# 3dlg-hcvc/tricolo

Measured on AMD Instinct MI355X. Metric: trimodal training samples/sec (32^3 voxel + 6-view), higher is better.
Workload: dtype f16 (f16 activation storage + f16 MFMA operands, fp32 accumulate; bf16x3 heads/GRU; within 1e-3 of the fp32 reference)

## Files before the change

include/tricolo_hip.h:

```cpp
#ifndef TRICOLO_HIP_H
#define TRICOLO_HIP_H
#include <stddef.h>
#include <stdint.h>

#ifdef __cplusplus
extern "C" {
#endif

#define TRI_FMT_F32 0
#define TRI_FMT_BF16 1
#define TRI_FMT_F16 2

int tri_version(void);
const char* tri_last_error(void);

typedef struct TriConvDesc {
    int B, ID, IH, IW, Cin;
    int OD, OH, OW, Cout;
    int KD, KH, KW, stride, pad_d, pad_h, pad_w;
} TriConvDesc;

int tri_conv_kpad(int ntaps, int cin_stored);
typedef struct TriPrepDesc {
    const float* w;
// ... 1 lines not shown
    void* lo;
    long s_row, s_tap, s_inner;
    int rows, ntaps, inner, inner_pad, kpad, fmt;
    int frag;
} TriPrepDesc;
int tri_weight_prep_multi(const TriPrepDesc* descs_dev, int n, void* stream);
int tri_weight_prep(const float* w, long s_row, long s_tap, long s_inner, int rows, int ntaps, int inner, int inner_pad,
                    void* w_hi, void* w_lo, int fmt, int frag, void* stream);

int tri_embedding_fwd(const int* tokens, const float* weight, int B, int L, int D, float* out, void* stream);
int tri_embedding_bwd(const int* tokens, const float* dout, int B, int L, int V, int D, int padding_idx, float* dweight, void* stream);

int tri_retrieval_topk(const float* text, const float* shape, const int* label, int Nq, int Ns, int D, int k, int* topk_idx ,
                       double* topk_sim , int* first_hit , void* stream);

int tri_linear_small_supported(int M, int K, int N);
int tri_linear_small_fwd(const float* x, const float* w, const float* bias, float* y, int M, int K, int N, int act, int split3, void* stream);
int tri_linear_small_dgrad(const float* dout, const float* y, const float* w, float* dx, int M, int K, int N, int act, int split3,
                           void* stream);
int tri_linear_small_wgrad(const float* x, const float* dout, const float* y, float* dw, float* db , int M, int K, int N,
                           int act, int split3, void* stream);
int tri_linear_small_bwd(const float* x, const float* dout, const float* y, const float* w, float* dx, float* dw, float* db, int M, int K,
                         int N, int act, int split3, void* stream);

int tri_conv_num_mtiles(const TriConvDesc* d, int split3);
int tri_conv_num_records(const TriConvDesc* d, int split3, int row_list);
typedef enum TriConvFamily {
    TRI_CONV_IGEMM = 0,
    TRI_CONV_DMA = 2,
    TRI_CONV_HALO2D = 3,
    TRI_CONV_STEM = 4,
    TRI_CONV_HALO_ROWS = 5,
    TRI_CONV_VOX0 = 6,
    TRI_CONV_C64 = 9,
    TRI_CONV_S2D = 10,
    TRI_CONV_PW = 12,
    TRI_CONV_VOXG = 13,
    TRI_CONV_VOXB = 14,
    TRI_CONV_S2G = 15
} TriConvFamily;
#define TRI_FAMILY_CODE_MASK 255
#define TRI_FAMILY_TILE_SHIFT 8
#define TRI_FAMILY_SPLITK_SHIFT 16
#define TRI_FAMILY_SPU_SHIFT 24
int tri_conv_kernel_family(const TriConvDesc* d, int transposed, int split3);
typedef enum TriWgradFamily {
    TRI_WGRAD_STAGED = 0,
    TRI_WGRAD_DMA = 2,
    TRI_WGRAD_STEM = 4,
    TRI_WGRAD_VOX0 = 6,
    TRI_WGRAD_KROW = 7,
    TRI_WGRAD_C64 = 9
} TriWgradFamily;
#define TRI_WGRAD_MASK 1
#define TRI_WGRAD_ROWS 2
#define TRI_WGRAD_SPLIT3 4
#define TRI_WGRAD_BNF 8
#define TRI_WGRAD_ROUTE_CODE_MASK 255
#define TRI_WGRAD_ROUTE_GROUP_SHIFT 8
#define TRI_WGRAD_ROUTE_ROWS_SHIFT 12
#define TRI_WGRAD_ROUTE_COLS_SHIFT 21
int tri_conv_wgrad_route(const TriConvDesc* d, int act_fmt, int features);
int tri_conv_wgrad_kernel_family(const TriConvDesc* d, int act_fmt);
size_t tri_conv_workspace(const TriConvDesc* d, int transposed);
int tri_conv_fwd(const TriConvDesc* d, const void* in, const void* w_hi, const void* w_lo, void* out, const uint8_t* row_mask,
                 const float* bias, int act, int accumulate, float* stats, int act_fmt, void* workspace, size_t workspace_bytes,
                 const int* row_pos , const int* row_count ,
                 void* stream);
int tri_conv_dgrad(const TriConvDesc* d, const void* dout, const void* wt_hi, const void* wt_lo, void* din, const uint8_t* row_mask,
                   int accumulate, int act_fmt, void* workspace, size_t workspace_bytes,
                   const int* row_pos ,
                   const int* row_count ,
                   void* stream);
typedef struct TriConvBnSums {
    const void* y;
    const float* relu_scale;
    const float* relu_shift;
    const void* relu_out;
    float* partial;
} TriConvBnSums;
int tri_conv_dgrad_bn_records(const TriConvDesc* d, int accumulate, int act_fmt);
int tri_conv_dgrad_bn(const TriConvDesc* d, const void* dout, const void* wt_hi, const void* wt_lo, void* din, int accumulate,
                      int act_fmt, void* workspace, size_t workspace_bytes, const int* row_pos, const TriConvBnSums* sums, void* stream);
size_t tri_conv_wgrad_workspace(const TriConvDesc* d);
size_t tri_conv_plan_bytes(const TriConvDesc* d);
int tri_conv_plan_build(const TriConvDesc* d, void* plan, void* stream);
int tri_conv_wgrad(const TriConvDesc* d, const void* in, const void* dout, const uint8_t* row_mask, const void* plan ,
                   void* workspace, size_t workspace_bytes, float* dw, long s_co, long s_tap, long s_ci, int cin_real, int split3,
                   int act_fmt, float out_scale ,
                   const int* row_pos, const int* row_count ,
                   void* stream);
#ifndef TRI_WGRAD_GROUP_MAX
#define TRI_WGRAD_GROUP_MAX 24
#endif
typedef struct TriWgradReduce {
    const float* slab;
    float* dw;
    long s_co, s_tap, s_ci;
    int splits, Cout, Kpad, ntaps, cin_stored, cin_real, zlanes, nblocks;
    float out_scale;
    int kw_real;
    int kw_shift;
} TriWgradReduce;
int tri_conv_wgrad_partial(const TriConvDesc* d, const void* in, const void* dout, const uint8_t* row_mask, const void* plan ,
                           void* workspace, size_t workspace_bytes, float* dw, long s_co, long s_tap, long s_ci, int cin_real, int split3,
                           int act_fmt, float out_scale, const int* row_pos, const int* row_count, TriWgradReduce* pending ,
                           void* stream);
int tri_wgrad_reduce_grouped(const TriWgradReduce* pending , int n, void* stream);
int tri_wgrad_reduce_grouped_noted(const TriWgradReduce* pending , int n, int* note, void* stream);
#define TRI_WGRAD_JOBS_MAX 12
typedef struct TriWgradJob {
    const TriConvDesc* d;
    const void* in;
    const void* dout;
    const void* plan;
    void* workspace;
    size_t workspace_bytes;
    float* dw;
    long s_co, s_tap, s_ci;
    int cin_real;
    float out_scale;
    const int* row_pos;
    const int* row_count;
} TriWgradJob;
int tri_conv_stem_wgrad_bn(const TriConvDesc* d, const void* in, const void* y, const uint8_t* arg, const void* dpool, const float* c1,
                           const float* c2, const float* c3, const float* relu_scale, const float* relu_shift, void* workspace,
                           size_t workspace_bytes, float* dw, long s_co, long s_tap, long s_ci, int cin_real, int act_fmt, float out_scale,
                           TriWgradReduce* pending , void* stream);
int tri_conv_wgrad_group_info(const TriConvDesc* d, int act_fmt, int* family, int* tiles, int* steps);
int tri_conv_wgrad_partial_group(const TriWgradJob* jobs , int n, int act_fmt, TriWgradReduce* pending ,
                                 void* stream);

int tri_bn_finalize(const float* partial, int ntiles, int C, const int* count_dev, int count_host, const float* gamma,
                    const float* beta, float* running_mean, float* running_var, long long* num_batches_tracked, float momentum,
                    float eps, float* mean, float* invstd, float* scale, float* shift, void* stream);
int tri_bn_eval_coeffs(int C, const float* gamma, const float* beta, const float* rm, const float* rv, float eps, float* mean,
                       float* invstd, float* scale, float* shift, void* stream);
int tri_bn_act(const void* y, const float* scale, const float* shift, const void* res, const float* rscale, const float* rshift,
               void* out, long M, int C, int relu, int act_fmt, void* stream);
int tri_relu_bwd(const void* dout, const void* out, void* g, long n, int act_fmt, void* stream);
int tri_bn_bwd_num_blocks(long M);
int tri_bn_bwd_reduce(const void* y, const void* g, long M, int C, float* partial, const float* relu_scale, const float* relu_shift,
                      const void* relu_out, const uint8_t* row_mask , int act_fmt,
                      void* stream);
int tri_bn_bwd_small(const void* y, const void* g, long M, int C, const int* count_dev, int count_host, const float* gamma,
                     const float* mean, const float* invstd, const float* relu_scale, const float* relu_shift, const void* relu_out,
                     void* g_masked, const uint8_t* row_mask, int keep_inactive, void* dy, float* dgamma, float* dbeta, float out_scale,
                     int act_fmt, void* stream);
int tri_bn_bwd_finalize(const float* partial, int nblk, int C, const int* count_dev, int count_host, const float* gamma,
                        const float* mean, const float* invstd, float* dgamma, float* dbeta, float* c1, float* c2, float* c3,
                        float out_scale ,
                        void* stream);
int tri_bn_bwd_apply(const void* y, const void* g, const float* c1, const float* c2, const float* c3, const uint8_t* row_mask,
                     void* dy, long M, int C, const float* relu_scale, const float* relu_shift, const void* relu_out,
                     void* g_masked ,
                     int keep_inactive ,
                     int act_fmt, void* stream);
int tri_bn_bwd_pair_reduce(const void* ya, const void* yb, const void* g, const void* relu_out, long M, int C, float* partial_a,
                           float* partial_b, int act_fmt, void* stream);
int tri_bn_bwd_pair_finalize(const float* partial_a, const float* partial_b, int nblk, int C, int count_host, const float* gamma_a,
                             const float* mean_a, const float* invstd_a, float* buf_a, const float* gamma_b, const float* mean_b,
                             const float* invstd_b, float* buf_b, float out_scale, void* stream);
int tri_bn_bwd_pair_apply(const void* ya, const void* yb, const void* g, const void* relu_out, const float* buf_a, const float* buf_b,
                          void* dya, void* dyb, void* g_masked, long M, int C, int act_fmt, void* stream);

int tri_bn_relu_pool3d_fwd(const void* y, const float* scale, const float* shift, const uint8_t* mask, int B, int D, int C,
// ... 131 lines not shown
```

tricolo_amd/_C.py:

```python
from __future__ import annotations

import ctypes as C
import os

import torch

_HERE = os.path.dirname(os.path.abspath(__file__))
LIB_PATH = os.path.join(_HERE, "libtricolo_hip.so")


class TriConvDesc(C.Structure):
    _fields_ = [(n, C.c_int) for n in ("B", "ID", "IH", "IW", "Cin", "OD", "OH", "OW", "Cout",
                                       "KD", "KH", "KW", "stride", "pad_d", "pad_h", "pad_w")]


class TriPrepDesc(C.Structure):
    _fields_ = [("w", C.c_void_p), ("hi", C.c_void_p), ("lo", C.c_void_p), ("s_row", C.c_long), ("s_tap", C.c_long),
                ("s_inner", C.c_long), ("rows", C.c_int), ("ntaps", C.c_int), ("inner", C.c_int), ("inner_pad", C.c_int),
                ("kpad", C.c_int), ("fmt", C.c_int), ("frag", C.c_int)]


class TriWgradReduce(C.Structure):
    _fields_ = [("slab", C.c_void_p), ("dw", C.c_void_p), ("s_co", C.c_long), ("s_tap", C.c_long), ("s_ci", C.c_long)] + \
               [(n, C.c_int) for n in ("splits", "Cout", "Kpad", "ntaps", "cin_stored", "cin_real", "zlanes", "nblocks")] + \
               [("out_scale", C.c_float), ("kw_real", C.c_int), ("kw_shift", C.c_int)]


class TriWgradJob(C.Structure):
    _fields_ = [("d", C.POINTER(TriConvDesc)), ("inp", C.c_void_p), ("dout", C.c_void_p), ("plan", C.c_void_p), ("workspace", C.c_void_p),
                ("workspace_bytes", C.c_size_t), ("dw", C.c_void_p), ("s_co", C.c_long), ("s_tap", C.c_long), ("s_ci", C.c_long),
                ("cin_real", C.c_int), ("out_scale", C.c_float), ("row_pos", C.c_void_p), ("row_count", C.c_void_p)]


class TriConvBnSums(C.Structure):
    _fields_ = [("y", C.c_void_p), ("relu_scale", C.c_void_p), ("relu_shift", C.c_void_p), ("relu_out", C.c_void_p), ("partial", C.c_void_p)]


TRI_WGRAD_JOBS_MAX = 12
TRI_ERR_ARG, TRI_ERR_UNSUPPORTED = -1, -2

P, I, L, F, Z, DBL = C.c_void_p, C.c_int, C.c_long, C.c_float, C.c_size_t, C.c_double
DP = C.POINTER(TriConvDesc)

SIGNATURES = {
    "tri_version": (I, []),
    "tri_last_error": (C.c_char_p, []),
    "tri_conv_kpad": (I, [I, I]),
    "tri_weight_prep": (I, [P, L, L, L, I, I, I, I, P, P, I, I, P]),
    "tri_weight_prep_multi": (I, [P, I, P]),
    "tri_embedding_fwd": (I, [P, P, I, I, I, P, P]),
    "tri_embedding_bwd": (I, [P, P, I, I, I, I, I, P, P]),
    "tri_retrieval_topk": (I, [P, P, P, I, I, I, I, P, P, P, P]),
    "tri_linear_small_supported": (I, [I, I, I]),
    "tri_linear_small_fwd": (I, [P, P, P, P, I, I, I, I, I, P]),
    "tri_linear_small_dgrad": (I, [P, P, P, P, I, I, I, I, I, P]),
    "tri_linear_small_wgrad": (I, [P, P, P, P, P, I, I, I, I, I, P]),
    "tri_linear_small_bwd": (I, [P, P, P, P, P, P, P, I, I, I, I, I, P]),
    "tri_conv_num_mtiles": (I, [DP, I]),
    "tri_conv_num_records": (I, [DP, I, I]),
    "tri_conv_workspace": (Z, [DP, I]),
    "tri_conv_kernel_family": (I, [DP, I, I]),
    "tri_conv_wgrad_kernel_family": (I, [DP, I]),
    "tri_conv_wgrad_route": (I, [DP, I, I]),
    "tri_conv_fwd": (I, [DP, P, P, P, P, P, P, I, I, P, I, P, Z, P, P, P]),
    "tri_conv_dgrad": (I, [DP, P, P, P, P, P, I, I, P, Z, P, P, P]),
    "tri_conv_dgrad_bn_records": (I, [DP, I, I]),
    "tri_conv_dgrad_bn": (I, [DP, P, P, P, P, I, I, P, Z, P, C.POINTER(TriConvBnSums), P]),
    "tri_conv_wgrad_workspace": (Z, [DP]),
    "tri_conv_plan_bytes": (Z, [DP]),
    "tri_conv_plan_build": (I, [DP, P, P]),
    "tri_conv_wgrad": (I, [DP, P, P, P, P, P, Z, P, L, L, L, I, I, I, F, P, P, P]),
    "tri_conv_wgrad_partial": (I, [DP, P, P, P, P, P, Z, P, L, L, L, I, I, I, F, P, P, P, P]),
    "tri_wgrad_reduce_grouped": (I, [P, I, P]),
    "tri_wgrad_reduce_grouped_noted": (I, [P, I, P, P]),
    "tri_conv_stem_wgrad_bn": (I, [DP, P, P, P, P, P, P, P, P, P, P, Z, P, L, L, L, I, I, F, P, P]),
    "tri_conv_wgrad_group_info": (I, [DP, I, P, P, P]),
    "tri_conv_wgrad_partial_group": (I, [P, I, I, P, P]),
    "tri_bn_finalize": (I, [P, I, I, P, I, P, P, P, P, P, F, F, P, P, P, P, P]),
    "tri_bn_eval_coeffs": (I, [I, P, P, P, P, F, P, P, P, P, P]),
    "tri_bn_act": (I, [P, P, P, P, P, P, P, L, I, I, I, P]),
    "tri_relu_bwd": (I, [P, P, P, L, I, P]),
    "tri_bn_bwd_num_blocks": (I, [L]),
    "tri_bn_bwd_reduce": (I, [P, P, L, I, P, P, P, P, P, I, P]),
    "tri_bn_bwd_finalize": (I, [P, I, I, P, I, P, P, P, P, P, P, P, P, F, P]),
    "tri_bn_bwd_small": (I, [P, P, L, I, P, I, P, P, P, P, P, P, P, P, I, P, P, P, F, I, P]),
    "tri_bn_bwd_apply": (I, [P, P, P, P, P, P, P, L, I, P, P, P, P, I, I, P]),
    "tri_bn_bwd_pair_reduce": (I, [P, P, P, P, L, I, P, P, I, P]),
    "tri_bn_bwd_pair_finalize": (I, [P, P, I, I, I, P, P, P, P, P, P, P, P, F, P]),
    "tri_bn_bwd_pair_apply": (I, [P, P, P, P, P, P, P, P, P, L, I, I, P]),
    "tri_bn_relu_pool3d_fwd": (I, [P, P, P, P, I, I, I, P, P, I, P]),
    "tri_pool3d_bwd_route": (I, [P, P, P, P, P, P, I, I, I, P, I, P]),
    "tri_pool3d_bwd_route_rows": (I, [P, P, P, P, P, P, I, I, I, P, P, P, I, P]),
    "tri_pool3d_bwd_route_rows_num_blocks": (I, [I, I, I]),
    "tri_pool3d_bwd_route_rows_reduce": (I, [P, P, P, P, P, P, I, I, I, P, P, P, P, I, P]),
    "tri_bn_bwd_apply_rows": (I, [P, P, P, P, P, P, I, P, P, L, I, P]),
    "tri_bn_bwd_rows_scratch": (C.c_size_t, [I]),
    "tri_bn_bwd_rows": (I, [P, P, I, P, P, L, P, P, P, P, P, P, F, P, I, P]),
    "tri_pool3d_bwd_route_reduce_num_blocks": (I, [I, I, I]),
    "tri_pool3d_bwd_route_reduce": (I, [P, P, P, P, P, P, I, I, I, P, P, I, P]),
    "tri_maxpool2d_fwd": (I, [P, I, I, I, I, P, P, P, P, I, P]),
    "tri_maxpool2d_bwd": (I, [P, P, I, I, I, I, P, I, P]),
    "tri_maxpool_bn_bwd_num_blocks": (I, [I, I, I]),
    "tri_maxpool_bn_bwd_reduce": (I, [P, P, P, I, I, I, I, P, P, P, I, P]),
    "tri_maxpool_bn_bwd_pooled_num_blocks": (I, [I, I, I]),
    "tri_maxpool_bn_bwd_reduce_pooled": (I, [P, P, P, P, I, I, I, I, P, P, P, P, I, P]),
    "tri_maxpool_bn_bwd_apply": (I, [P, P, P, I, I, I, I, P, P, P, P, P, P, I, P]),
    "tri_avgpool_viewmax_fwd": (I, [P, I, I, I, I, P, P, I, P]),
    "tri_avgpool_viewmax_bwd": (I, [P, P, I, I, I, I, P, I, F, P]),
    "tri_voxel_scatter": (I, [P, P, I, I, I, P, P, I, P]),
    "tri_voxel_from_rgba_u8": (I, [P, I, I, P, P, I, P]),
    "tri_nchw3_u8_to_nhwc4": (I, [P, I, I, I, P, P, P, I, P]),
    "tri_mask_count": (I, [P, L, P, P]),
    "tri_debug_stamp": (I, [P, P]),
    "tri_debug_buffer_b128_probe": (I, [P, P, L, I, P]),
    "tri_mask_compact_scratch": (Z, [L]),
    "tri_mask_compact": (I, [P, L, P, P, P, P]),
    "tri_mask_pyramid": (I, [P, I, I, P, P]),
    "tri_mask_compact_multi_scratch": (Z, [P, I]),
    "tri_mask_compact_multi": (I, [P, P, I, P, P, P, P]),
    "tri_nchw3_to_nhwc4": (I, [P, I, I, I, P, I, P]),
    "tri_l2norm_fwd": (I, [P, I, I, F, P, P, P]),
    "tri_l2norm_bwd": (I, [P, P, P, I, I, F, P, P]),
    "tri_colsum": (I, [P, L, I, P, P]),
    "tri_axpy": (I, [P, F, P, L, P]),
    "tri_act_bwd": (I, [P, P, P, L, I, P]),
    "tri_cast_from_f32": (I, [P, P, L, F, I, P]),
    "tri_cast_to_f32": (I, [P, P, L, I, P]),
    "tri_gru_fwd": (I, [P, P, P, I, I, P, P, P, I, P]),
    "tri_gru_bwd": (I, [P, P, P, P, I, I, P, P, P, P, I, P]),
    "tri_ntxent_workspace": (Z, [I, I]),
    "tri_ntxent_fwd_bwd": (I, [P, P, I, I, F, F, I, P, P, P, P, Z, P]),
    "tri_ntxent_bwd": (I, [P, P, I, I, F, F, I, P, P, P, P, Z, P]),
    "tri_ntxent_multi_workspace": (Z, [I, I, I]),
    "tri_ntxent_multi_fwd": (I, [P, I, I, I, F, F, I, P, P, Z, P]),
    "tri_ntxent_multi_bwd": (I, [P, I, I, I, F, F, I, P, P, P, P, Z, P]),
    "tri_triplet_workspace": (Z, [I, I]),
    "tri_triplet_fwd": (I, [P, P, I, I, DBL, P, P, P, Z, P]),
    "tri_triplet_bwd": (I, [P, P, I, I, DBL, P, P, P, P, Z, P]),
    "tri_triplet_multi_workspace": (Z, [I, I, I]),
    "tri_triplet_multi_fwd": (I, [P, I, I, I, DBL, P, P, P, Z, P]),
    "tri_triplet_multi_bwd": (I, [P, I, I, I, DBL, P, P, P, P, Z, P]),
    "tri_nn_dist2": (I, [P, P, P, P, I, I, I, I, I, P, P, P]),
    "tri_f1_counts": (I, [P, P, I, I, C.POINTER(F), I, P, P, P]),
    "tri_f1_finalize": (I, [P, P, P, P, P, P, I, I, I, I, F, P, P, P, P, P]),
    "tri_mesh_bbox": (I, [P, P, I, P, P]),
    "tri_mesh_face_cdf": (I, [P, P, P, P, P, I, L, P, P, P]),
    "tri_mesh_sample_points": (I, [P, P, P, P, P, P, P, I, I, C.c_ulonglong, P, P, P]),
    "tri_raster_workspace": (Z, [L, I, I, I, I]),
    "tri_raster_render": (I, [P, P, P, P, P, P, P, P, I, L, I, I, I, DBL, DBL, P, P, P, P]),
    "tri_voxelize_workspace": (Z, [L, I, I]),
# ... 87 lines not shown
```

tricolo_amd/csrc/bn_pool.hip:

```cpp
#include "common.h"
#include "../../include/tricolo_hip.h"

__global__ void bn_finalize_kernel(const float* __restrict__ partial, int ntiles, int C, const int* __restrict__ count_dev,
                                   int count_host, const float* __restrict__ gamma, const float* __restrict__ beta,
                                   float* running_mean, float* running_var, long long* num_batches_tracked, float momentum,
                                   float eps, float* __restrict__ mean_out, float* __restrict__ invstd_out,
                                   float* __restrict__ scale_out, float* __restrict__ shift_out) {
    __shared__ double ssum[4], ssq[4];
    const int c = blockIdx.x;
    float pg = 0.f, pb = 0.f, prm = 0.f, prv = 0.f;
    int pcount = count_host;
    if (threadIdx.x == 0) {
        pg = gamma[c]; pb = beta[c];
        if (running_mean) { prm = running_mean[c]; prv = running_var[c]; }
        if (count_dev) pcount = *count_dev;
    }
    double s = 0.0, q = 0.0;
#pragma unroll 8
    for (int tIdx = threadIdx.x; tIdx < ntiles; tIdx += 256) {
        s += (double)partial[((size_t)tIdx * 2 + 0) * C + c];
        q += (double)partial[((size_t)tIdx * 2 + 1) * C + c];
    }
#pragma unroll
    for (int o = 32; o > 0; o >>= 1) { s += __shfl_xor(s, o); q += __shfl_xor(q, o); }
    if ((threadIdx.x & 63) == 0) { ssum[threadIdx.x >> 6] = s; ssq[threadIdx.x >> 6] = q; }
    __syncthreads();
    if (threadIdx.x == 0) {
        s = (ssum[0] + ssum[1]) + (ssum[2] + ssum[3]);
        q = (ssq[0] + ssq[1]) + (ssq[2] + ssq[3]);
        double n = (double)pcount;
        if (n < 1.0) {
            mean_out[c] = 0.f; invstd_out[c] = 0.f; scale_out[c] = 0.f; shift_out[c] = 0.f;
            return;
        }
        double mean = s / n;
        double var = q / n - mean * mean;
        if (var < 0.0) var = 0.0;
        double invstd = 1.0 / sqrt(var + (double)eps);
        mean_out[c] = (float)mean;
        invstd_out[c] = (float)invstd;
        float sc = (float)((double)pg * invstd);
        scale_out[c] = sc;
        shift_out[c] = (float)((double)pb - mean * (double)pg * invstd);
        if (running_mean) {
            double unb = n > 1.0 ? var * n / (n - 1.0) : var;
            running_mean[c] = (float)((1.0 - momentum) * prm + momentum * mean);
            running_var[c] = (float)((1.0 - momentum) * prv + momentum * unb);
        }
        if (num_batches_tracked && c == 0) *num_batches_tracked += 1;
    }
}

extern "C" int tri_bn_finalize(const float* partial, int ntiles, int C, const int* count_dev, int count_host, const float* gamma,
                               const float* beta, float* running_mean, float* running_var, long long* num_batches_tracked,
                               float momentum, float eps, float* mean, float* invstd, float* scale, float* shift, void* stream) {
    bn_finalize_kernel<<<C, 256, 0, (hipStream_t)stream>>>(partial, ntiles, C, count_dev, count_host, gamma, beta,
                                                                      running_mean, running_var, num_batches_tracked, momentum,
                                                                      eps, mean, invstd, scale, shift);
    return tri_check_launch("tri_bn_finalize");
}

__global__ void bn_eval_coeffs_kernel(int C, const float* gamma, const float* beta, const float* rm, const float* rv, float eps,
                                      float* mean, float* invstd, float* scale, float* shift) {
    int c = blockIdx.x * blockDim.x + threadIdx.x;
    if (c >= C) return;
    float is = 1.0f / sqrtf(rv[c] + eps);
    mean[c] = rm[c]; invstd[c] = is; scale[c] = gamma[c] * is; shift[c] = beta[c] - rm[c] * gamma[c] * is;
}
extern "C" int tri_bn_eval_coeffs(int C, const float* gamma, const float* beta, const float* rm, const float* rv, float eps,
                                  float* mean, float* invstd, float* scale, float* shift, void* stream) {
    bn_eval_coeffs_kernel<<<(C + 255) / 256, 256, 0, (hipStream_t)stream>>>(C, gamma, beta, rm, rv, eps, mean, invstd, scale, shift);
    return tri_check_launch("tri_bn_eval_coeffs");
}

template <typename T>
__global__ void bn_act_kernel(const T* __restrict__ y, const float4* __restrict__ scale, const float4* __restrict__ shift,
                              const T* __restrict__ res, const float4* __restrict__ rscale, const float4* __restrict__ rshift,
                              T* __restrict__ out, long total4, int C4, int relu) {
    for (long i = (long)blockIdx.x * blockDim.x + threadIdx.x; i < total4; i += (long)gridDim.x * blockDim.x) {
        int c = (int)(i % C4);
        float4 v = Act<T>::ld4(y + i * 4), s = scale[c], b = shift[c];
        v.x = __fmaf_rn(v.x, s.x, b.x); v.y = __fmaf_rn(v.y, s.y, b.y); v.z = __fmaf_rn(v.z, s.z, b.z); v.w = __fmaf_rn(v.w, s.w, b.w);
        if (res) {
            float4 r = Act<T>::ld4(res + i * 4);
            if (rscale) {
                float4 rs = rscale[c], rb = rshift[c];
                r.x = r.x * rs.x + rb.x; r.y = r.y * rs.y + rb.y; r.z = r.z * rs.z + rb.z; r.w = r.w * rs.w + rb.w;
            }
            v.x += r.x; v.y += r.y; v.z += r.z; v.w += r.w;
        }
        if (relu) { v.x = fmaxf(v.x, 0.f); v.y = fmaxf(v.y, 0.f); v.z = fmaxf(v.z, 0.f); v.w = fmaxf(v.w, 0.f); }
        Act<T>::st4(out + i * 4, v);
    }
}
static inline int ew_grid(long total) {
    long b = (total + 255) / 256;
    return (int)(b < 1 ? 1 : (b > 4096 ? 4096 : b));
}
extern "C" int tri_bn_act(const void* y, const float* scale, const float* shift, const void* res, const float* rscale,
                          const float* rshift, void* out, long M, int C, int relu, int act_fmt, void* stream) {
    if (C % 4) { tri_set_error("tri_bn_act: C must be a multiple of 4"); return TRI_ERR_ARG; }
    long total4 = M * (C / 4);
    TRI_ACT_DISPATCH(act_fmt, bn_act_kernel<T><<<ew_grid(total4), 256, 0, (hipStream_t)stream>>>(
        (const T*)y, (const float4*)scale, (const float4*)shift, (const T*)res, (const float4*)rscale, (const float4*)rshift, (T*)out,
        total4, C / 4, relu));
    return tri_check_launch("tri_bn_act");
}

template <typename T>
__global__ void relu_bwd_kernel(const T* dout, const T* __restrict__ out, T* g, long total4) {
    for (long i = (long)blockIdx.x * blockDim.x + threadIdx.x; i < total4; i += (long)gridDim.x * blockDim.x) {
        float4 d = Act<T>::ld4(dout + i * 4), o = Act<T>::ld4(out + i * 4);
        d.x = o.x > 0.f ? d.x : 0.f; d.y = o.y > 0.f ? d.y : 0.f; d.z = o.z > 0.f ? d.z : 0.f; d.w = o.w > 0.f ? d.w : 0.f;
        Act<T>::st4(g + i * 4, d);
    }
}
extern "C" int tri_relu_bwd(const void* dout, const void* out, void* g, long n, int act_fmt, void* stream) {
    if (n % 4) { tri_set_error("tri_relu_bwd: n must be a multiple of 4"); return TRI_ERR_ARG; }
    TRI_ACT_DISPATCH(act_fmt, relu_bwd_kernel<T><<<ew_grid(n / 4), 256, 0, (hipStream_t)stream>>>((const T*)dout, (const T*)out, (T*)g, n / 4));
    return tri_check_launch("tri_relu_bwd");
}

static inline int bnb_rows(long M) {
    if (M <= 16384) return 16;
    if (M <= 32768) return 32;
    if (M < 65536) return 64;
    long rows = (M + 2047) / 2048;
    rows = (rows + 63) / 64 * 64;
    return (int)(rows < 256 ? 256 : rows);
}
template <typename T, int MASK, bool ROWMASK>
__global__ void bn_bwd_reduce_kernel(const T* __restrict__ y, const T* __restrict__ g, long M, int C, float* __restrict__ partial,
                                     int BNB_ROWS, const float4* __restrict__ rs, const float4* __restrict__ rb,
                                     const T* __restrict__ ro, const uint8_t* __restrict__ row_mask) {
    extern __shared__ float sh[];
    const int C4 = C >> 2;
    const int tpr = C4 < 256 ? C4 : 256;
    const int rpp = 256 / tpr;
    const int cpt = (C4 + tpr - 1) / tpr;
    const int tc = threadIdx.x % tpr, tr = threadIdx.x / tpr;
    const long r0 = (long)blockIdx.x * BNB_ROWS;
    const long r1 = r0 + BNB_ROWS < M ? r0 + BNB_ROWS : M;
    for (int cc = 0; cc < cpt; ++cc) {
        int c4 = tc + cc * tpr;
        float4 sg = make_float4(0, 0, 0, 0), sgy = make_float4(0, 0, 0, 0);
        float4 s4 = make_float4(0, 0, 0, 0), b4 = make_float4(1, 1, 1, 1);
        if (MASK == 1 && c4 < C4) { s4 = rs[c4]; b4 = rb[c4]; }
        if (c4 < C4 && tr < rpp)
#pragma unroll 4
            for (long r = r0 + tr; r < r1; r += rpp) {
                if (ROWMASK && !row_mask[r]) continue;
                float4 gv = Act<T>::ld4(g + r * C + c4 * 4), yv = Act<T>::ld4(y + r * C + c4 * 4);
                if (MASK == 1) {
                    gv.x = __fmaf_rn(yv.x, s4.x, b4.x) > 0.f ? gv.x : 0.f; gv.y = __fmaf_rn(yv.y, s4.y, b4.y) > 0.f ? gv.y : 0.f;
                    gv.z = __fmaf_rn(yv.z, s4.z, b4.z) > 0.f ? gv.z : 0.f; gv.w = __fmaf_rn(yv.w, s4.w, b4.w) > 0.f ? gv.w : 0.f;
                }
                if (MASK == 2) {
                    const float4 ov = Act<T>::ld4(ro + r * C + c4 * 4);
                    gv.x = ov.x > 0.f ? gv.x : 0.f; gv.y = ov.y > 0.f ? gv.y : 0.f; gv.z = ov.z > 0.f ? gv.z : 0.f; gv.w = ov.w > 0.f ? gv.w : 0.f;
                }
                sg.x += gv.x; sg.y += gv.y; sg.z += gv.z; sg.w += gv.w;
                sgy.x += gv.x * yv.x; sgy.y += gv.y * yv.y; sgy.z += gv.z * yv.z; sgy.w += gv.w * yv.w;
            }
        __syncthreads();
        if (c4 < C4 && tr < rpp) {
            float* p = sh + ((size_t)tr * tpr + tc) * 8;
            p[0] = sg.x; p[1] = sg.y; p[2] = sg.z; p[3] = sg.w; p[4] = sgy.x; p[5] = sgy.y; p[6] = sgy.z; p[7] = sgy.w;
        }
        __syncthreads();
        if (tr == 0 && c4 < C4) {
            float a[8] = {0, 0, 0, 0, 0, 0, 0, 0};
            for (int rr = 0; rr < rpp; ++rr) {
                const float* p = sh + ((size_t)rr * tpr + tc) * 8;
#pragma unroll
// ... 25 lines not shown
    else if (relu_scale) TRI_BNR(1);
    else TRI_BNR(0);
#undef TRI_BNR
    return tri_check_launch("tri_bn_bwd_reduce");
}

__device__ __forceinline__ void bn_bwd_finalize_body(const float* __restrict__ partial, int nblk, int C, const int* __restrict__ count_dev,
                                                     int count_host, const float* __restrict__ gamma, const float* __restrict__ mean,
                                                     const float* __restrict__ invstd, float* __restrict__ dgamma, float* __restrict__ dbeta,
                                                     float* __restrict__ c1, float* __restrict__ c2, float* __restrict__ c3, float out_scale,
                                                     int c) {
    __shared__ double ssum[4], ssq[4];
    float pmu = 0.f, pis = 0.f, pga = 0.f;
    int pcount = count_host;
    if (threadIdx.x == 0) {
        pmu = mean[c]; pis = invstd[c]; pga = gamma[c];
        if (count_dev) pcount = *count_dev;
    }
    double s = 0.0, q = 0.0;
#pragma unroll 8
    for (int b = threadIdx.x; b < nblk; b += 256) {
        s += (double)partial[((size_t)b * 2 + 0) * C + c];
        q += (double)partial[((size_t)b * 2 + 1) * C + c];
    }
#pragma unroll
    for (int o = 32; o > 0; o >>= 1) { s += __shfl_xor(s, o); q += __shfl_xor(q, o); }
    if ((threadIdx.x & 63) == 0) { ssum[threadIdx.x >> 6] = s; ssq[threadIdx.x >> 6] = q; }
    __syncthreads();
    if (threadIdx.x == 0) {
        s = (ssum[0] + ssum[1]) + (ssum[2] + ssum[3]);
        q = (ssq[0] + ssq[1]) + (ssq[2] + ssq[3]);
        double n = (double)pcount;
        if (n < 1.0) { dgamma[c] = 0.f; dbeta[c] = 0.f; c1[c] = 0.f; c2[c] = 0.f; c3[c] = 0.f; return; }
        double mu = pmu, is = pis, ga = pga;
        double dbe = s;
        double dga = is * (q - mu * s);
        dgamma[c] = (float)(dga * (double)out_scale);
        dbeta[c] = (float)(dbe * (double)out_scale);
        double k1 = ga * is;
        double k3 = -ga * is * is * dga / n;
        double k2 = -k1 * dbe / n - k3 * mu;
        c1[c] = (float)k1; c2[c] = (float)k2; c3[c] = (float)k3;
    }
}
__global__ void bn_bwd_finalize_kernel(const float* __restrict__ partial, int nblk, int C, const int* __restrict__ count_dev,
                                       int count_host, const float* __restrict__ gamma, const float* __restrict__ mean,
                                       const float* __restrict__ invstd, float* __restrict__ dgamma, float* __restrict__ dbeta,
                                       float* __restrict__ c1, float* __restrict__ c2, float* __restrict__ c3, float out_scale) {
    bn_bwd_finalize_body(partial, nblk, C, count_dev, count_host, gamma, mean, invstd, dgamma, dbeta, c1, c2, c3, out_scale, blockIdx.x);
}
__global__ void bn_bwd_finalize_pair_kernel(const float* __restrict__ pa, const float* __restrict__ pb, int nblk, int C, int count_host,
                                            const float* __restrict__ ga, const float* __restrict__ ma, const float* __restrict__ ia,
                                            float* __restrict__ buf_a, const float* __restrict__ gb, const float* __restrict__ mb,
                                            const float* __restrict__ ib, float* __restrict__ buf_b, float out_scale) {
    const bool second = (int)blockIdx.x >= C;
    const int c = second ? blockIdx.x - C : blockIdx.x;
    float* buf = second ? buf_b : buf_a;
    bn_bwd_finalize_body(second ? pb : pa, nblk, C, nullptr, count_host, second ? gb : ga, second ? mb : ma, second ? ib : ia, buf, buf + C,
                         buf + 2 * C, buf + 3 * C, buf + 4 * C, out_scale, c);
}
extern "C" int tri_bn_bwd_finalize(const float* partial, int nblk, int C, const int* count_dev, int count_host, const float* gamma,
                                   const float* mean, const float* invstd, float* dgamma, float* dbeta, float* c1, float* c2,
                                   float* c3, float out_scale, void* stream) {
    bn_bwd_finalize_kernel<<<C, 256, 0, (hipStream_t)stream>>>(partial, nblk, C, count_dev, count_host, gamma, mean,
                                                                          invstd, dgamma, dbeta, c1, c2, c3, out_scale);
    return tri_check_launch("tri_bn_bwd_finalize");
}

template <typename T, int MASK>
__global__ void bn_bwd_apply_kernel(const T* __restrict__ y, const T* g, const float4* __restrict__ c1,
                                    const float4* __restrict__ c2, const float4* __restrict__ c3,
                                    const uint8_t* __restrict__ row_mask, T* dy, long total4, int C4,
                                    const float4* __restrict__ rs, const float4* __restrict__ rb, const T* __restrict__ ro, T* gm,
                                    int keep_inactive) {
    for (long i = (long)blockIdx.x * blockDim.x + threadIdx.x; i < total4; i += (long)gridDim.x * blockDim.x) {
        long row = i / C4;
        int c = (int)(i - row * C4);
        float4 o = make_float4(0.f, 0.f, 0.f, 0.f);
        if (keep_inactive && row_mask && !row_mask[row]) continue;
        if (!row_mask || row_mask[row]) {
            float4 yv = Act<T>::ld4(y + i * 4), gv = Act<T>::ld4(g + i * 4), a = c1[c], b = c2[c], d = c3[c];
            if (MASK == 1) {
                const float4 s4 = rs[c], b4 = rb[c];
                gv.x = __fmaf_rn(yv.x, s4.x, b4.x) > 0.f ? gv.x : 0.f; gv.y = __fmaf_rn(yv.y, s4.y, b4.y) > 0.f ? gv.y : 0.f;
                gv.z = __fmaf_rn(yv.z, s4.z, b4.z) > 0.f ? gv.z : 0.f; gv.w = __fmaf_rn(yv.w, s4.w, b4.w) > 0.f ? gv.w : 0.f;
            }
            if (MASK == 2) {
                const float4 ov = Act<T>::ld4(ro + i * 4);
                gv.x = ov.x > 0.f ? gv.x : 0.f; gv.y = ov.y > 0.f ? gv.y : 0.f; gv.z = ov.z > 0.f ? gv.z : 0.f; gv.w = ov.w > 0.f ? gv.w : 0.f;
                if (gm) Act<T>::st4(gm + i * 4, gv);
            }
            o.x = a.x * gv.x + b.x + d.x * yv.x; o.y = a.y * gv.y + b.y + d.y * yv.y;
            o.z = a.z * gv.z + b.z + d.z * yv.z; o.w = a.w * gv.w + b.w + d.w * yv.w;
        }
        Act<T>::st4(dy + i * 4, o);
    }
}
extern "C" int tri_bn_bwd_apply(const void* y, const void* g, const float* c1, const float* c2, const float* c3,
                                const uint8_t* row_mask, void* dy, long M, int C, const float* relu_scale, const float* relu_shift,
                                const void* relu_out, void* g_masked, int keep_inactive, int act_fmt, void* stream) {
    long total4 = M * (C / 4);
#define TRI_BNA(MASK_)                                                                                                              \
    TRI_ACT_DISPATCH(act_fmt, bn_bwd_apply_kernel<T, MASK_><<<ew_grid(total4), 256, 0, (hipStream_t)stream>>>(                      \
        (const T*)y, (const T*)g, (const float4*)c1, (const float4*)c2, (const float4*)c3, row_mask, (T*)dy, total4, C / 4,          \
        (const float4*)relu_scale, (const float4*)relu_shift, (const T*)relu_out, (T*)g_masked, keep_inactive))
    if (relu_out) TRI_BNA(2);
    else if (relu_scale) TRI_BNA(1);
    else TRI_BNA(0);
#undef TRI_BNA
    return tri_check_launch("tri_bn_bwd_apply");
}

template <typename T>
__global__ void bn_bwd_reduce_pair_kernel(const T* __restrict__ ya, const T* __restrict__ yb, const T* __restrict__ g, long M, int C,
                                          float* __restrict__ partial_a, float* __restrict__ partial_b, int BNB_ROWS,
                                          const T* __restrict__ ro) {
    extern __shared__ float sh[];
    const int C4 = C >> 2;
    const int tpr = C4 < 256 ? C4 : 256;
    const int rpp = 256 / tpr;
    const int cpt = (C4 + tpr - 1) / tpr;
    const int tc = threadIdx.x % tpr, tr = threadIdx.x / tpr;
    const long r0 = (long)blockIdx.x * BNB_ROWS;
    const long r1 = r0 + BNB_ROWS < M ? r0 + BNB_ROWS : M;
    for (int cc = 0; cc < cpt; ++cc) {
        int c4 = tc + cc * tpr;
        float4 sg = make_float4(0, 0, 0, 0), sga = make_float4(0, 0, 0, 0), sgb = make_float4(0, 0, 0, 0);
        if (c4 < C4 && tr < rpp)
#pragma unroll 4
            for (long r = r0 + tr; r < r1; r += rpp) {
                float4 gv = Act<T>::ld4(g + r * C + c4 * 4);
                const float4 av = Act<T>::ld4(ya + r * C + c4 * 4), bv = Act<T>::ld4(yb + r * C + c4 * 4), ov = Act<T>::ld4(ro + r * C + c4 * 4);
                gv.x = ov.x > 0.f ? gv.x : 0.f; gv.y = ov.y > 0.f ? gv.y : 0.f; gv.z = ov.z > 0.f ? gv.z : 0.f; gv.w = ov.w > 0.f ? gv.w : 0.f;
                sg.x += gv.x; sg.y += gv.y; sg.z += gv.z; sg.w += gv.w;
                sga.x += gv.x * av.x; sga.y += gv.y * av.y; sga.z += gv.z * av.z; sga.w += gv.w * av.w;
                sgb.x += gv.x * bv.x; sgb.y += gv.y * bv.y; sgb.z += gv.z * bv.z; sgb.w += gv.w * bv.w;
            }
        __syncthreads();
        if (c4 < C4 && tr < rpp) {
            float* p = sh + ((size_t)tr * tpr + tc) * 12;
            p[0] = sg.x; p[1] = sg.y; p[2] = sg.z; p[3] = sg.w; p[4] = sga.x; p[5] = sga.y; p[6] = sga.z; p[7] = sga.w;
            p[8] = sgb.x; p[9] = sgb.y; p[10] = sgb.z; p[11] = sgb.w;
        }
        __syncthreads();
        if (tr == 0 && c4 < C4) {
            float a[12] = {0, 0, 0, 0, 0, 0, 0, 0, 0, 0, 0, 0};
            for (int rr = 0; rr < rpp; ++rr) {
                const float* p = sh + ((size_t)rr * tpr + tc) * 12;
#pragma unroll
                for (int k = 0; k < 12; ++k) a[k] += p[k];
            }
            float* oa = partial_a + (size_t)blockIdx.x * 2 * C;
            float* ob = partial_b + (size_t)blockIdx.x * 2 * C;
#pragma unroll
            for (int k = 0; k < 4; ++k) { oa[c4 * 4 + k] = a[k]; oa[C + c4 * 4 + k] = a[4 + k]; ob[c4 * 4 + k] = a[k]; ob[C + c4 * 4 + k] = a[8 + k]; }
        }
    }
}
template <typename T>
__global__ void bn_bwd_apply_pair_kernel(const T* __restrict__ ya, const T* __restrict__ yb, const T* g, const float4* __restrict__ ca,
                                         const float4* __restrict__ cb, T* dya, T* dyb, long total4, int C4, const T* __restrict__ ro, T* gm) {
    for (long i = (long)blockIdx.x * blockDim.x + threadIdx.x; i < total4; i += (long)gridDim.x * blockDim.x) {
        const int c = (int)(i % C4);
        float4 gv = Act<T>::ld4(g + i * 4);
        const float4 av = Act<T>::ld4(ya + i * 4), bv = Act<T>::ld4(yb + i * 4), ov = Act<T>::ld4(ro + i * 4);
        gv.x = ov.x > 0.f ? gv.x : 0.f; gv.y = ov.y > 0.f ? gv.y : 0.f; gv.z = ov.z > 0.f ? gv.z : 0.f; gv.w = ov.w > 0.f ? gv.w : 0.f;
        if (gm) Act<T>::st4(gm + i * 4, gv);
        {
            const float4 a = ca[c], b = ca[C4 + c], d = ca[2 * C4 + c];
            float4 o;
            o.x = a.x * gv.x + b.x + d.x * av.x; o.y = a.y * gv.y + b.y + d.y * av.y;
            o.z = a.z * gv.z + b.z + d.z * av.z; o.w = a.w * gv.w + b.w + d.w * av.w;
            asm volatile("" : "+v"(o.x), "+v"(o.y), "+v"(o.z), "+v"(o.w));
            Act<T>::st4(dya + i * 4, o);
        }
        {
// ... 1069 lines not shown
```

tricolo_amd/csrc/common.h:

```cpp
#pragma once
#include <hip/hip_runtime.h>
#include <stdint.h>
#include <stdlib.h>

typedef __bf16 bf16_t;
typedef __bf16 bf16x8 __attribute__((ext_vector_type(8)));
typedef __bf16 bf16x4 __attribute__((ext_vector_type(4)));
typedef float f32x4 __attribute__((ext_vector_type(4)));
typedef _Float16 f16_t;
typedef _Float16 f16x8 __attribute__((ext_vector_type(8)));
typedef _Float16 f16x4 __attribute__((ext_vector_type(4)));

#define TRI_OK 0
#define TRI_ERR_ARG (-1)
#define TRI_ERR_UNSUPPORTED (-2)

extern "C" void tri_set_error(const char* msg);
static inline int tri_probe_ablation() {
#ifdef TRI_PROBE_BUILD
    static int abl = -1;
    if (abl < 0) { const char* e = getenv("TRICOLO_HALO_ABL"); abl = e ? atoi(e) : 0; }
    return abl;
#else
    return 0;
#endif
}
int tri_check_launch(const char* what);

static inline int tri_env_read_int(const char* name, int dflt) { const char* e = getenv(name); return e ? atoi(e) : dflt; }
static inline bool tri_env_read_is(const char* name, char c) { const char* e = getenv(name); return e && e[0] == c; }
#define tri_env_int(name, dflt) ([]() -> int { static const int v = tri_env_read_int(name, dflt); return v; }())
#define tri_env_is(name, c) ([]() -> bool { static const bool v = tri_env_read_is(name, c); return v; }())

struct FastDiv {
    uint32_t mul, shift, d;
};
static inline FastDiv make_fastdiv(uint32_t d) {
    FastDiv f;
    f.d = d;
    uint32_t l = 0;
    while ((1u << l) < d) ++l;
    f.shift = l;
    f.mul = (uint32_t)((((uint64_t)1 << 32) * (((uint64_t)1 << l) - d)) / d + 1);
    return f;
}
__device__ __forceinline__ uint32_t fdiv(uint32_t n, const FastDiv& f) {
    return (__umulhi(f.mul, n) + n) >> f.shift;
}

__device__ __forceinline__ int tile_off(int row, int chunk) {
    int g = (row >> 2) & 3;
    int f = g ^ ((g & 1) << 1);
    return row * 64 + ((chunk ^ f) << 4);
}

__device__ __forceinline__ void split_bf16(const float4& v, bf16x4& hi, bf16x4& lo) {
    hi[0] = (bf16_t)v.x; hi[1] = (bf16_t)v.y; hi[2] = (bf16_t)v.z; hi[3] = (bf16_t)v.w;
    lo[0] = (bf16_t)(v.x - (float)hi[0]); lo[1] = (bf16_t)(v.y - (float)hi[1]);
    lo[2] = (bf16_t)(v.z - (float)hi[2]); lo[3] = (bf16_t)(v.w - (float)hi[3]);
}
__device__ __forceinline__ bf16x4 to_bf16x4(const float4& v) {
    bf16x4 h;
    h[0] = (bf16_t)v.x; h[1] = (bf16_t)v.y; h[2] = (bf16_t)v.z; h[3] = (bf16_t)v.w;
    return h;
}

#ifndef TRI_FMT_F32
#define TRI_FMT_F32 0
#define TRI_FMT_BF16 1
#define TRI_FMT_F16 2
#endif
__device__ __forceinline__ float fp32_rounded(float x) {
    asm volatile("" : "+v"(x));
    return x;
}
template <typename T> struct Act;
template <> struct Act<float> {
    static constexpr int BYTES = 4;
    static constexpr int SIG_BITS = 24;
    static __device__ __forceinline__ float4 ld4(const float* p) { return *(const float4*)p; }
    static __device__ __forceinline__ void st4(float* p, const float4& v) { *(float4*)p = v; }
    static __device__ __forceinline__ float rnd(float v) { return v; }
};
template <> struct Act<bf16_t> {
    static constexpr int BYTES = 2;
    static constexpr int SIG_BITS = 8;
    static __device__ __forceinline__ float4 ld4(const bf16_t* p) {
        bf16x4 r = *(const bf16x4*)p;
        return make_float4((float)r[0], (float)r[1], (float)r[2], (float)r[3]);
    }
    static __device__ __forceinline__ void st4(bf16_t* p, const float4& v) { *(bf16x4*)p = to_bf16x4(v); }
    static __device__ __forceinline__ float rnd(float v) { return (float)(bf16_t)v; }
};
template <> struct Act<f16_t> {
    static constexpr int BYTES = 2;
    static constexpr int SIG_BITS = 11;
    static __device__ __forceinline__ float4 ld4(const f16_t* p) {
        f16x4 r = *(const f16x4*)p;
        return make_float4((float)r[0], (float)r[1], (float)r[2], (float)r[3]);
    }
    static __device__ __forceinline__ void st4(f16_t* p, const float4& v) {
        f16x4 h;
        h[0] = (f16_t)v.x; h[1] = (f16_t)v.y; h[2] = (f16_t)v.z; h[3] = (f16_t)v.w;
        *(f16x4*)p = h;
    }
    static __device__ __forceinline__ float rnd(float v) { return (float)(f16_t)v; }
};
#define TRI_ACT_DISPATCH(fmt, ...)                                       \
    do {                                                                 \
        if ((fmt) == TRI_FMT_BF16) { using T = bf16_t; __VA_ARGS__; }    \
        else if ((fmt) == TRI_FMT_F16) { using T = f16_t; __VA_ARGS__; } \
        else { using T = float; __VA_ARGS__; }                           \
    } while (0)

template <typename E> struct Mma;
template <> struct Mma<bf16_t> {
    typedef bf16x8 v8;
    static __device__ __forceinline__ f32x4 mma(v8 a, v8 b, f32x4 c) { return __builtin_amdgcn_mfma_f32_16x16x32_bf16(a, b, c, 0, 0, 0); }
};
template <> struct Mma<f16_t> {
    typedef f16x8 v8;
    static __device__ __forceinline__ f32x4 mma(v8 a, v8 b, f32x4 c) { return __builtin_amdgcn_mfma_f32_16x16x32_f16(a, b, c, 0, 0, 0); }
};
template <typename AT> struct OpOf { typedef bf16_t E; };
template <> struct OpOf<f16_t> { typedef f16_t E; };

typedef int v4i __attribute__((ext_vector_type(4)));
__device__ __forceinline__ v4i make_rsrc_words(const void* base, unsigned bytes) {
    return (v4i){(int)(unsigned)(size_t)base, (int)(((size_t)base >> 32) & 0xffff), (int)bytes, 0x00020000};
}
__device__ __forceinline__ unsigned lds_addr(const void* p) {
#if defined(__HIP_DEVICE_COMPILE__)
    return (unsigned)(size_t)(__attribute__((address_space(3))) const char*)p;
#else
    return 0;
#endif
}
__device__ __forceinline__ void dma16_async(v4i rsrc, unsigned lds_dst, int voff) {
#if defined(__HIP_DEVICE_COMPILE__)
    asm volatile("s_mov_b32 m0, %0\n\ts_nop 0\n\tbuffer_load_dwordx4 %1, %2, 0 offen lds"
                 :: "s"(__builtin_amdgcn_readfirstlane(lds_dst)), "v"(voff), "s"(rsrc) : "memory", "m0");
#endif
}

__device__ __forceinline__ int xcd_remap(int orig, int nwg) {
    int q = nwg >> 3, r = nwg & 7, xcd = orig & 7;
    return (xcd < r ? xcd * (q + 1) : r * (q + 1) + (xcd - r) * q) + (orig >> 3);
}

__device__ __forceinline__ float wave_sum(float v) {
#pragma unroll
    for (int o = 32; o > 0; o >>= 1) v += __shfl_xor(v, o);
    return v;
}
__device__ __forceinline__ float wave_max(float v) {
#pragma unroll
    for (int o = 32; o > 0; o >>= 1) v = fmaxf(v, __shfl_xor(v, o));
    return v;
}
```

tricolo_amd/csrc/conv_c64.hip:

```cpp
#include "common.h"
#include <stdlib.h>
#include "../../include/tricolo_hip.h"
#include "conv_vox.h"

int tri_internal_num_cus();

template <int N>
__device__ __forceinline__ float c64_row_ror(float v) {
    return __builtin_bit_cast(float, __builtin_amdgcn_update_dpp(0, __builtin_bit_cast(int, v), 0x120 + N, 0xf, 0xf, false));
}

struct ConvC64Args {
    const void* in;
    const void* w;
    void* out;
    float* stats;
    int N, H, nbricks, transposed, accumulate;
    unsigned in_bytes;
    const void* bs_y;
    const void* bs_ro;
    const float* bs_scale;
    const float* bs_shift;
    int bs_mode;
};

template <int W, int TY>
struct C64Cfg {
    static constexpr int XOFF = 4;
    static constexpr int RPR = (W + 15) / 16;
    static constexpr int P = RPR * 16 + 16;
    static constexpr int PITCH = P * 128;
    static constexpr int SLAB = (TY + 2) * PITCH;
    static constexpr int RUNS = TY * RPR;
    static constexpr int CPR = W * 8;
    static constexpr int ITEMS = (TY + 2) * CPR;
    static constexpr int MAXC = (ITEMS + 255) / 256;
    static constexpr int WROW = 9 * 64 * 2 + 16;
    static constexpr size_t SMEM = (size_t)SLAB > (size_t)64 * WROW ? (size_t)SLAB : (size_t)64 * WROW;
    static_assert(RUNS == 8 || RUNS == 4, "a brick is 8 or 4 runs (half of them per wave pair)");
    static_assert(2 * PITCH + 4096 < 65536, "fragment-read immediates");
};

template <typename AT, int W, int TY, bool ACCUM, bool BS>
__global__ __launch_bounds__(256, 2) void conv_c64_kernel(const ConvC64Args p) {
    typedef C64Cfg<W, TY> C;
    typedef typename OpOf<AT>::E E;
    typedef Mma<E> MM;
    typedef typename MM::v8 v8;
    constexpr int KPAD = 9 * 64;
    extern __shared__ __attribute__((aligned(16))) char smem[];
    const int t = threadIdx.x, lane = t & 63, wave = __builtin_amdgcn_readfirstlane(t >> 6), fr = lane & 15, fq = lane >> 4;
    const int c = wave & 1, h = wave >> 1;
    char* const slab = smem;
    const int G = gridDim.x, wg = blockIdx.x;
    const int bpi = p.H / TY;

    v8 wf[9][2][2];
    {
        constexpr int NCH = 64 * KPAD * 2 / 16;
        uint4 wld[NCH / 256];
#pragma unroll
        for (int u = 0; u < NCH / 256; ++u) wld[u] = *(const uint4*)((const char*)p.w + (size_t)(t + u * 256) * 16);
#pragma unroll
        for (int u = 0; u < NCH / 256; ++u) {
            const int ch = t + u * 256, row = ch / 72, col = ch - row * 72;
            *(uint4*)(slab + row * C::WROW + col * 16) = wld[u];
        }
        __syncthreads();
#pragma unroll
        for (int ct = 0; ct < 2; ++ct) {
            const char* wrow = slab + (32 * c + 16 * ct + fr) * C::WROW + fq * 16;
#pragma unroll
            for (int tap = 0; tap < 9; ++tap) {
                const int tw = p.transposed ? 8 - tap : tap;
#pragma unroll
                for (int ks = 0; ks < 2; ++ks) wf[tap][ks][ct] = *(const v8*)(wrow + (tw * 64 + ks * 32) * 2);
            }
        }
        __syncthreads();
    }
    int lofs[3][2];
#pragma unroll
    for (int kx = 0; kx < 3; ++kx) {
        const int sx = C::XOFF + fr + kx - 1;
#pragma unroll
        for (int ks = 0; ks < 2; ++ks) lofs[kx][ks] = sx * 128 + (((4 * ks + fq) ^ ((sx >> 1) & 7)) << 4);
    }
    const __amdgpu_buffer_rsrc_t irs = __builtin_amdgcn_make_buffer_rsrc((void*)p.in, 0, p.in_bytes, 0x00020000);
    f32x4 cs[2], cq[2];
    cs[0] = cs[1] = cq[0] = cq[1] = (f32x4){0.f, 0.f, 0.f, 0.f};
    constexpr int bsm = BS ? (ACCUM ? 2 : 1) : 0;
    float* const bsc = (float*)(smem + C::SMEM);
    if (bsm == 1 && t < 128) bsc[t] = t < 64 ? p.bs_scale[t] : p.bs_shift[t - 64];
    constexpr int NZ = C::RPR * 16 - W + 2;
    for (int i = t; i < (TY + 2) * NZ * 8; i += 256) {
        const int row = i / (NZ * 8), rem = i - row * (NZ * 8), zp = rem >> 3, q = rem & 7;
        const int sx = zp == 0 ? C::XOFF - 1 : C::XOFF + W + zp - 1;
        *(uint4*)(slab + row * C::PITCH + sx * 128 + q * 16) = make_uint4(0u, 0u, 0u, 0u);
    }

#pragma unroll 1
    for (int j = wg; j < p.nbricks; j += G) {
        const int n = j / bpi, y0 = (j - n * bpi) * TY;
        unsigned warm = 0;
        if (bsm) {
            constexpr int LINES = TY * W;
            const size_t b0 = ((size_t)(n * p.H + y0) * W) * 64;
            if (t < LINES) warm = *(const unsigned*)((const AT*)p.bs_y + b0 + (size_t)t * 64);
            else if (bsm == 2 && t < 2 * LINES) warm = *(const unsigned*)((const AT*)p.bs_ro + b0 + (size_t)(t - LINES) * 64);
        }
        __syncthreads();
        {
            uint4 pre[C::MAXC];
            int dst[C::MAXC];
#pragma unroll
            for (int u = 0; u < C::MAXC; ++u) {
                const int i = t + u * 256;
                const int yy = i / C::CPR, cc = i % C::CPR;
                const int sx = C::XOFF + (cc >> 3), q = cc & 7;
                const int gy = y0 - 1 + yy;
                const bool inside = i < C::ITEMS;
                dst[u] = inside ? yy * C::PITCH + sx * 128 + ((q ^ ((sx >> 1) & 7)) << 4) : -1;
                const bool ok = inside && (unsigned)gy < (unsigned)p.H;
                const unsigned voff = ok ? (unsigned)(((n * p.H + gy) * W) * 128 + cc * 16) : 0x80000000u;
                pre[u] = __builtin_bit_cast(uint4, __builtin_amdgcn_raw_buffer_load_b128(irs, voff, 0, 0));
            }
#pragma unroll
            for (int u = 0; u < C::MAXC; ++u)
                if (dst[u] >= 0) *(uint4*)(slab + dst[u]) = pre[u];
        }
        if (bsm) asm volatile("" :: "v"(warm));
        __syncthreads();

#pragma unroll 1
        for (int r = h; r < C::RUNS; r += 2) {
            const int yl = r / C::RPR, xr = r % C::RPR;
            const char* sb = slab + yl * C::PITCH + xr * 2048;
            f32x4 acc[2];
            acc[0] = acc[1] = (f32x4){0.f, 0.f, 0.f, 0.f};
            typedef E e4 __attribute__((ext_vector_type(4)));
            const size_t eo = (((size_t)(n * p.H + y0 + yl) * W) + xr * 16 + fr) * 64 + 32 * c + fq * 4;
            AT* const o = (AT*)p.out + eo;
            const bool valid = !(W % 16) || xr * 16 + fr < W;
            e4 prev[2];
            if (ACCUM && valid) { prev[0] = *(const e4*)o; prev[1] = *(const e4*)(o + 16); }
            e4 bsy[2], bsr[2];
            v8 bf[2][6];
#pragma unroll
            for (int i = 0; i < 6; ++i) bf[0][i] = *(const v8*)(sb + lofs[i >> 1][i & 1]);
#pragma unroll
            for (int ky = 0; ky < 3; ++ky) {
                if (ky < 2) {
#pragma unroll
                    for (int i = 0; i < 6; ++i) bf[(ky + 1) & 1][i] = *(const v8*)(sb + lofs[i >> 1][i & 1] + (ky + 1) * C::PITCH);
                }
                if (ky == 2 && bsm && valid) {
                    bsy[0] = *(const e4*)((const AT*)p.bs_y + eo); bsy[1] = *(const e4*)((const AT*)p.bs_y + eo + 16);
                    if (bsm == 2) { bsr[0] = *(const e4*)((const AT*)p.bs_ro + eo); bsr[1] = *(const e4*)((const AT*)p.bs_ro + eo + 16); }
                }
                __builtin_amdgcn_sched_barrier(0);
#pragma unroll
                for (int i = 0; i < 6; ++i) {
                    acc[0] = MM::mma(wf[ky * 3 + (i >> 1)][i & 1][0], bf[ky & 1][i], acc[0]);
                    acc[1] = MM::mma(wf[ky * 3 + (i >> 1)][i & 1][1], bf[ky & 1][i], acc[1]);
                }
                __builtin_amdgcn_sched_barrier(0);
            }
            if (!valid) continue;
#pragma unroll
            for (int ct = 0; ct < 2; ++ct) {
                f32x4 v = acc[ct];
                if (ACCUM) {
                    const e4 e = prev[ct];
                    v[0] += (float)e[0]; v[1] += (float)e[1]; v[2] += (float)e[2]; v[3] += (float)e[3];
                }
                const e4 hh = __builtin_convertvector(v, e4);
                *(e4*)(o + 16 * ct) = hh;
                f32x4 rv = {(float)hh[0], (float)hh[1], (float)hh[2], (float)hh[3]};
                if (bsm) {
                    const f32x4 yv = {(float)bsy[ct][0], (float)bsy[ct][1], (float)bsy[ct][2], (float)bsy[ct][3]};
                    f32x4 sc = {0.f, 0.f, 0.f, 0.f}, sh = sc;
                    if (bsm == 1) { sc = *(const f32x4*)(bsc + 32 * c + 16 * ct + 4 * fq); sh = *(const f32x4*)(bsc + 64 + 32 * c + 16 * ct + 4 * fq); }
#pragma unroll
                    for (int r = 0; r < 4; ++r) {
                        const bool keep = bsm == 1 ? __fmaf_rn(yv[r], sc[r], sh[r]) > 0.f : (float)bsr[ct][r] > 0.f;
                        rv[r] = keep ? rv[r] : 0.f;
                    }
                    cs[ct] += rv;
                    cq[ct] += rv * yv;
                } else {
                    cs[ct] += rv;
                    cq[ct] += rv * rv;
                }
            }
        }
    }

    if (p.stats) {
        float* const red = (float*)slab;
        __syncthreads();
#pragma unroll
        for (int ct = 0; ct < 2; ++ct)
#pragma unroll
            for (int r = 0; r < 4; ++r) {
                float s_ = cs[ct][r], q_ = cq[ct][r];
                s_ += c64_row_ror<8>(s_); q_ += c64_row_ror<8>(q_);
                s_ += c64_row_ror<4>(s_); q_ += c64_row_ror<4>(q_);
                s_ += c64_row_ror<2>(s_); q_ += c64_row_ror<2>(q_);
                s_ += c64_row_ror<1>(s_); q_ += c64_row_ror<1>(q_);
                if (fr == 0) {
                    red[(wave * 32 + 16 * ct + 4 * fq + r) * 2 + 0] = s_;
                    red[(wave * 32 + 16 * ct + 4 * fq + r) * 2 + 1] = q_;
                }
            }
        __syncthreads();
        if (t < 64) {
            const int cw = t >> 5, i = t & 31;
            const float s_ = red[(cw * 32 + i) * 2] + red[((cw + 2) * 32 + i) * 2];
            const float q_ = red[(cw * 32 + i) * 2 + 1] + red[((cw + 2) * 32 + i) * 2 + 1];
            p.stats[(size_t)blockIdx.x * 128 + t] = s_;
            p.stats[(size_t)blockIdx.x * 128 + 64 + t] = q_;
        }
    }
}

bool tri_internal_c64_geometry(const TriConvDesc& d, TriC64Geom* g) {
    if (tri_env_is("TRICOLO_NO_C64_CONV", '1')) return false;
    if (d.ID != 1 || d.OD != 1 || d.KD != 1 || d.KH != 3 || d.KW != 3 || d.stride != 1 || d.pad_d != 0 || d.pad_h != 1 || d.pad_w != 1) return false;
    if (d.Cin != 64 || d.Cout != 64 || d.OH != d.IH || d.OW != d.IW) return false;
    int ty;
    if (d.IW == 32) ty = 4; else if (d.IW == 64 || d.IW == 56) ty = 2; else if (d.IW == 16) ty = 8; else return false;
    if ((long)d.B * d.IH * d.IW * 128 >= (1L << 31)) return false;
    const int slots = 2 * tri_internal_num_cus();
    if (d.IH % ty || (long)d.B * (d.IH / ty) < 3L * slots) ty /= 2;
    if (d.IH % ty) return false;
    g->W = d.IW; g->TY = ty;
    g->nbricks = d.B * (d.IH / ty);
    g->grid = g->nbricks < slots ? g->nbricks : slots;
    return true;
}

template <typename AT, int W, int TY, bool ACCUM, bool BS>
static int c64_launch_t(const ConvC64Args& a, int grid, hipStream_t stream) {
    typedef C64Cfg<W, TY> C;
    static bool attr = false;
    if (!attr) {
        hipFuncSetAttribute((const void*)conv_c64_kernel<AT, W, TY, ACCUM, BS>, hipFuncAttributeMaxDynamicSharedMemorySize, (int)C::SMEM + 512);
        attr = true;
    }
    conv_c64_kernel<AT, W, TY, ACCUM, BS><<<grid, 256, C::SMEM + 512, stream>>>(a);
    return tri_check_launch("tri_conv(c64)");
}

int tri_internal_c64_launch(const TriC64Geom& g, int B, int H, const void* in, const void* w, void* out, float* stats, int transposed,
                            int accumulate, int act_fmt, const TriConvBnSums* bs, hipStream_t stream) {
    ConvC64Args a{};
    a.in = in; a.w = w; a.out = out; a.stats = stats;
    if (bs) {
        a.bs_y = bs->y; a.bs_ro = bs->relu_out; a.bs_scale = bs->relu_scale; a.bs_shift = bs->relu_shift;
        a.bs_mode = accumulate ? 2 : 1;
        if (accumulate ? !bs->relu_out : !bs->relu_scale) {
            tri_set_error("conv(c64): BatchNorm-backward sums come in two forms: relu_scale / relu_shift without accumulate, relu_out with it");
            return TRI_ERR_UNSUPPORTED;
        }
    }
    a.N = B; a.H = H; a.nbricks = g.nbricks; a.transposed = transposed; a.accumulate = accumulate;
    a.in_bytes = (unsigned)((size_t)B * H * g.W * 128);
#define TRI_C64_BS(W_, TY_, BS_)                                                                                           \
    if (g.W == W_ && g.TY == TY_ && (bs != nullptr) == BS_) {                                                              \
        if (act_fmt == TRI_FMT_F16)                                                                                        \
            return accumulate ? c64_launch_t<f16_t, W_, TY_, true, BS_>(a, g.grid, stream) : c64_launch_t<f16_t, W_, TY_, false, BS_>(a, g.grid, stream);   \
        return accumulate ? c64_launch_t<bf16_t, W_, TY_, true, BS_>(a, g.grid, stream) : c64_launch_t<bf16_t, W_, TY_, false, BS_>(a, g.grid, stream);     \
    }
#define TRI_C64(W_, TY_) TRI_C64_BS(W_, TY_, false)
    TRI_C64(32, 4)
    TRI_C64(32, 2)
    TRI_C64(64, 2)
    TRI_C64(64, 1)
    TRI_C64(56, 2)
    TRI_C64(56, 1)
    TRI_C64(16, 8)
    TRI_C64(16, 4)
    TRI_C64_BS(32, 4, true)
    TRI_C64_BS(32, 2, true)
    TRI_C64_BS(16, 8, true)
    TRI_C64_BS(16, 4, true)
#undef TRI_C64_BS
#undef TRI_C64
    tri_set_error("conv(c64): brick shape not instantiated (BatchNorm-backward sums: 16- and 32-wide images only)");
    return TRI_ERR_UNSUPPORTED;
}

struct ConvS2dArgs {
    const void* in;
    const void* w;
    void* out;
    int N, H, nbricks;
    unsigned in_bytes;
};

template <int W, int TY>
struct S2dCfg {
    static constexpr int RPR = W / 16;
    static constexpr int P = RPR * 16 + 16;
    static constexpr int PITCH = P * 128;
    static constexpr int HALF = (TY + 1) * PITCH;
    static constexpr int SLAB = 2 * HALF;
    static constexpr int CPR = W * 16;
    static constexpr int ITEMS = (TY + 1) * CPR;
    static constexpr int MAXC = (ITEMS + 255) / 256;
    static constexpr int WROW = 3 * 128 * 2 + 16;
    static constexpr size_t SMEM = (size_t)SLAB > (size_t)64 * WROW ? (size_t)SLAB : (size_t)64 * WROW;
    static_assert(W % 16 == 0, "whole runs");
    static_assert(HALF + PITCH + 4096 < 65536, "fragment-read immediates");
};

template <typename AT, int W, int TY, bool ACCUM>
__global__ __launch_bounds__(256, 2) void conv_s2d_kernel(const ConvS2dArgs p) {
    typedef S2dCfg<W, TY> C;
    typedef typename OpOf<AT>::E E;
    typedef Mma<E> MM;
    typedef typename MM::v8 v8;
    constexpr int KPAD = 9 * 128;
    extern __shared__ __attribute__((aligned(16))) char smem[];
    const int t = threadIdx.x, lane = t & 63, wave = __builtin_amdgcn_readfirstlane(t >> 6), fr = lane & 15, fq = lane >> 4;
    char* const slab = smem;
    const int G = gridDim.x, wg = blockIdx.x;
    const int bpi = p.H / TY;

    v8 wf[9][4];
#pragma unroll
    for (int part = 0; part < 3; ++part) {
        constexpr int CH_ROW = 3 * 128 * 2 / 16;
        constexpr int NCH = 64 * CH_ROW;
        if (part) __syncthreads();
#pragma unroll
        for (int u = 0; u < NCH / 256; ++u) {
            const int ch = t + u * 256, row = ch / CH_ROW, col = ch - row * CH_ROW;
            *(uint4*)(slab + row * C::WROW + col * 16) = *(const uint4*)((const char*)p.w + ((size_t)row * KPAD + part * 384) * 2 + col * 16);
        }
        __syncthreads();
        const char* wrow = slab + (16 * wave + fr) * C::WROW + fq * 16;
#pragma unroll
        for (int tp = 0; tp < 3; ++tp)
#pragma unroll
            for (int ks = 0; ks < 4; ++ks) wf[part * 3 + tp][ks] = *(const v8*)(wrow + (tp * 128 + ks * 32) * 2);
    }
    __syncthreads();
    int lofs[2][2];
#pragma unroll
    for (int dj = 0; dj < 2; ++dj) {
        const int sx = fr + dj;
#pragma unroll
        for (int kk = 0; kk < 2; ++kk) lofs[dj][kk] = sx * 128 + (((4 * kk + fq) ^ ((sx >> 1) & 7)) << 4);
    }
    const __amdgpu_buffer_rsrc_t irs = __builtin_amdgcn_make_buffer_rsrc((void*)p.in, 0, p.in_bytes, 0x00020000);
    for (int i = t; i < 2 * (TY + 1) * 8; i += 256) {
        const int hf = i / ((TY + 1) * 8), rem = i - hf * ((TY + 1) * 8), row = rem >> 3, q = rem & 7;
        *(uint4*)(slab + hf * C::HALF + row * C::PITCH + W * 128 + q * 16) = make_uint4(0u, 0u, 0u, 0u);
    }

#pragma unroll 1
    for (int j = wg; j < p.nbricks; j += G) {
        const int n = j / bpi, y0 = (j - n * bpi) * TY;
        __syncthreads();
        {
            uint4 pre[C::MAXC];
            int dst[C::MAXC];
#pragma unroll
            for (int u = 0; u < C::MAXC; ++u) {
                const int i = t + u * 256;
                const int yy = i / C::CPR, cc = i % C::CPR;
// ... 125 lines not shown
```

tricolo_amd/csrc/conv_igemm.hip:

```cpp
#include "common.h"
#include <stdio.h>
#include <stdlib.h>
#include <map>
#include <mutex>
#include "../../include/tricolo_hip.h"
#include "conv_vox.h"

struct ConvArgs {
    const void* in;
    const void* w_hi;
    const void* w_lo;
    void* out;
    const uint8_t* row_mask;
    const int* row_pos;
    const int* row_count;
    const float* bias;
    float* stats;
    float* slab;
    int B, ID, IH, IW, Cin;
    int OD, OH, OW, Cout;
    int KD, KH, KW, stride, pd, ph, pw;
    int transposed, act, accumulate;
    int Kpad, M, ntaps, cin_shift, ksplit, steps_per_split;
    unsigned in_bytes;
// ... 1979 lines not shown
        do {                                                                                                                        \
            static size_t attrp = 0;                                                                                                \
            if (smem5 > attrp) {                                                                                                    \
                hipFuncSetAttribute((const void*)conv_halo_rows_kernel<AT, DRIP_, ACC_, 0, 2, true>, hipFuncAttributeMaxDynamicSharedMemorySize, \
                                    (int)smem5);                                                                                    \
                attrp = smem5;                                                                                                      \
            }                                                                                                                       \
            conv_halo_rows_kernel<AT, DRIP_, ACC_, 0, 2, true><<<pl.grid, 512, smem5, stream>>>(a);                                \
        } while (0)
            if (a.accumulate) TRI_ROWS_LAUNCH_P(false, true);
            else if (drip) TRI_ROWS_LAUNCH_P(true, false);
            else TRI_ROWS_LAUNCH_P(false, false);
#undef TRI_ROWS_LAUNCH_P
            return tri_check_launch("tri_conv(halo rows, producer waves)");
        }
        if (pl.TM == 3) {
            if (a.accumulate) TRI_ROWS_LAUNCH(false, true, 0, 3);
            else TRI_ROWS_LAUNCH(false, false, 0, 3);
        }
        else if (ntl == 0) TRI_ROWS_MODE(0);
        else if (ntl == 1) TRI_ROWS_MODE(1);
#ifdef HALO_NTL_EXPERIMENT
        else if (ntl == 2) TRI_ROWS_MODE(2);
        else TRI_ROWS_MODE(4);
#endif
#undef TRI_ROWS_MODE
#undef TRI_ROWS_LAUNCH
        return tri_check_launch("tri_conv(halo rows)");
    }
    static size_t attr = 0;
    if (smem > attr) {
        hipFuncSetAttribute((const void*)conv_halo2d_kernel<TM, false, AT>, hipFuncAttributeMaxDynamicSharedMemorySize, (int)smem);
        hipFuncSetAttribute((const void*)conv_halo2d_kernel<TM, true, AT>, hipFuncAttributeMaxDynamicSharedMemorySize, (int)smem);
        attr = smem;
    }
    if (pl.wgrec && a.stats) conv_halo2d_kernel<TM, true, AT><<<pl.grid, 256, smem, stream>>>(a);
    else conv_halo2d_kernel<TM, false, AT><<<pl.grid, 256, smem, stream>>>(a);
    return tri_check_launch("tri_conv(halo)");
}

template <typename AT>
static int launch_stem(ConvArgs& a, const StemGeom& sg, hipStream_t stream) {
    a.h_abl = tri_probe_ablation();
    a.row_pos = nullptr;
    const size_t smem = (size_t)2 * sg.slab_rows * sg.row_bytes + 4 * 64 * 2 * sizeof(float);
#define TRI_STEM(KH_)                                                                                                     \
    case KH_: {                                                                                                           \
        static bool attr = false;                                                                                         \
        if (!attr) {                                                                                                      \
            hipFuncSetAttribute((const void*)conv_stem_kernel<KH_, 2, AT>, hipFuncAttributeMaxDynamicSharedMemorySize, 80 * 1024); \
            hipFuncSetAttribute((const void*)conv_stem_kernel<KH_, 4, AT>, hipFuncAttributeMaxDynamicSharedMemorySize, 80 * 1024); \
            attr = true;                                                                                                  \
        }                                                                                                                 \
        if (sg.npt == 4) conv_stem_kernel<KH_, 4, AT><<<sg.grid, 256, smem, stream>>>(a, sg);                             \
        else conv_stem_kernel<KH_, 2, AT><<<sg.grid, 256, smem, stream>>>(a, sg);                                         \
        break;                                                                                                            \
    }
    switch (a.KH) {
        TRI_STEM(7) TRI_STEM(3) TRI_STEM(5)
        default: tri_set_error("conv(stem): kernel height not instantiated (3, 5, 7)"); return TRI_ERR_UNSUPPORTED;
    }
#undef TRI_STEM
    return tri_check_launch("tri_conv(stem)");
}

template <typename AT>
static int launch_dma_any(const ConvArgs& a, int bn, hipStream_t stream) {
    const int nst = dma_stages_for(a, bn);
    if (bn == 32) return nst == 2 ? launch_dma<32, 2, AT>(a, stream) : launch_dma<32, 3, AT>(a, stream);
    switch (nst) {
        case 4: return bn == 128 ? launch_dma<128, 4, AT>(a, stream) : launch_dma<64, 4, AT>(a, stream);
        case 3: return bn == 128 ? launch_dma<128, 3, AT>(a, stream) : launch_dma<64, 3, AT>(a, stream);
        default: return bn == 128 ? launch_dma<128, 2, AT>(a, stream) : launch_dma<64, 2, AT>(a, stream);
    }
}


enum : unsigned {
    CF_FWD = 1, CF_DGRAD = 2,
    CF_MASK = 4,
    CF_ROWS = 8,
    CF_BIAS_ACT = 16, CF_ACCUM = 32, CF_STATS = 64,
    CF_BNSUMS = 128,
    CF_EPI = CF_MASK | CF_ROWS | CF_BIAS_ACT,
};
enum ConvNeeds { ANY_MODE, MODE16, MODE16_DMA };
enum { PLAN_NO = 0, PLAN_TAKES = 1, PLAN_ALSO = 2 };

struct ConvFamily {
    TriConvFamily code;
    const char* kernel;
    ConvNeeds needs;
    int (*plan)(const TriConvDesc& v, int split_mode, int row_list, ConvPlan* pl);
    unsigned falls;
    unsigned refuses;
    unsigned fall_refuses;
    bool fall_drops_order;
    bool frag;
    bool site_mask;
    int (*records)(const ConvPlan& pl);
    int (*launch)(ConvArgs& a, const ConvPlan& pl, int act_fmt, const TriConvBnSums* bs, hipStream_t stream);
};

static int plan_generic(const TriConvDesc& v, int split_mode, int row_list, ConvPlan* pl) {
    const int cout = v.Cout, ntaps = v.KD * v.KH * v.KW, kpad = conv_kpad(v), bn = conv_bn(cout);
    const long M = (long)v.B * v.OD * v.OH * v.OW;
    int blocks = (int)((M + 127) / 128) * (cout / bn);
    const int blocks_dense = blocks;
    if (row_list) {
        const int side = v.OD > v.OH ? (v.OD > v.OW ? v.OD : v.OW) : (v.OH > v.OW ? v.OH : v.OW);
        const int occ_div = side >= 8 ? 4 : (side >= 4 ? 2 : 1);
        blocks = (blocks + occ_div - 1) / occ_div;
    }
    {
        static int narrow = -1;
        if (narrow < 0) narrow = 1024;
        if (pl->dma && bn == 128 && blocks_dense < narrow) { pl->bn = 64; blocks *= 2; }
    }
    static int lin64 = -1;
    if (lin64 < 0) lin64 = 1;
    const bool short_linear = lin64 && !pl->dma && !row_list && ntaps == 1 && kpad <= 256 && cout % 64 == 0;
    if (short_linear && bn == 128 && blocks < num_cus() && 2 * blocks >= num_cus()) { pl->bn = 64; blocks *= 2; }
    pl->nunits = pl->dma ? kpad / 64 : kpad / 32;
    int ks = 1;
    int min_per = pl->dma ? 2 : 4;
    if (blocks < 384 && pl->nunits >= 2 * min_per && cout % 64 == 0 && !(short_linear && blocks >= num_cus())) {
        const int target = conv_target_blocks() ? conv_target_blocks() : (split_mode == 2 ? 256 : 768);
        ks = (target + blocks - 1) / blocks;
        if (ks > pl->nunits / min_per) ks = pl->nunits / min_per;
        if (ks > 32) ks = 32;
        if (ks < 1) ks = 1;
    }
    if (row_list) {
        const long per_split = M * cout * (long)sizeof(float);
        while (ks > 1 && ks * per_split > (48L << 20)) --ks;
    }
    pl->per_split = (pl->nunits + ks - 1) / ks;
    pl->ksplit = (pl->nunits + pl->per_split - 1) / pl->per_split;
    return PLAN_TAKES;
}

static int plan_vox0(const TriConvDesc& v, int, int, ConvPlan* pl) { return tri_internal_vox0_geometry(v, &pl->g.vox0); }
static int plan_voxb(const TriConvDesc& v, int, int, ConvPlan* pl) { return tri_internal_voxb_geometry(v, &pl->g.voxb); }
static int plan_voxg(const TriConvDesc& v, int, int, ConvPlan* pl) {
    if (!tri_internal_voxg_geometry(v, &pl->g.voxg)) return PLAN_NO;
    pl->bn = pl->g.voxg.ct; pl->spu = pl->g.voxg.spu;
    return PLAN_TAKES;
}
static int plan_stem(const TriConvDesc& v, int, int, ConvPlan* pl) { return stem_geometry(v, &pl->g.stem); }
static int plan_pw(const TriConvDesc& v, int, int row_list, ConvPlan* pl) {
    if (row_list || !tri_internal_pw_geometry(v, &pl->g.pw)) return PLAN_NO;
    pl->bn = pl->g.pw.bn; pl->fall_also = pl->g.pw.transposed ? CF_FWD : CF_DGRAD;
    return PLAN_TAKES;
}
static int plan_c64(const TriConvDesc& v, int, int, ConvPlan* pl) {
    if (!tri_internal_c64_geometry(v, &pl->g.c64)) return PLAN_NO;
    if (pl->g.c64.W > 32) pl->fall_also = CF_BNSUMS;
    return PLAN_TAKES;
}
static int plan_s2g(const TriConvDesc& v, int, int, ConvPlan* pl) {
    if (!tri_internal_s2g_geometry(v, &pl->g.s2g)) return PLAN_NO;
    pl->bn = 64;
    return PLAN_TAKES;
}
static int plan_s2d(const TriConvDesc& v, int, int, ConvPlan* pl) { return tri_internal_s2d_geometry(v, &pl->also_g) ? PLAN_ALSO : PLAN_NO; }
static int plan_halo_rows(const TriConvDesc& v, int, int, ConvPlan* pl) {
    HaloGeom& h = pl->halo;
    if (v.Cout % 64 || tri_env_is("TRICOLO_NO_HALO", '1') || v.KD != 1 || v.KH != 3 || v.KW != 3 || v.stride != 1 || v.pad_d != 0 || v.pad_h != 1 ||
        v.pad_w != 1 || v.ID != 1 || v.OD != 1 || v.IH != v.OH || v.IW != v.OW || (long)v.B * v.IH * v.IW * v.Cin * 2 >= ((long)1 << 31))
        return PLAN_NO;
    HaloGeom t3{};
    if (!halo_geometry(v, 2, &h)) return PLAN_NO;
    if (h.v5 && !tri_env_is("TRICOLO_HALO_TM3", '0') && v.Cin != 64 && halo_geometry(v, 3, &t3) && t3.v5) {
        const int g = h.grid > t3.grid ? h.grid : t3.grid;
        const int r2 = (h.mtiles * h.nt + g - 1) / g, r3 = (t3.mtiles * h.nt + g - 1) / g;
        if (12 * r3 < 10 * r2) h = t3;
    }
    if (!h.v5) return PLAN_NO;
    pl->bn = 64; pl->tile = h.TM;
    return PLAN_TAKES;
}
static int plan_halo2d(const TriConvDesc&, int, int, ConvPlan* pl) {
    if (!pl->halo.TM) return PLAN_NO;
    pl->bn = 64; pl->tile = pl->halo.TM;
    return PLAN_TAKES;
}

static int halo_records(const ConvPlan& pl) { return pl.halo.wgrec ? pl.halo.grid / pl.halo.nt : pl.halo.mtiles; }

static int run_vox0(ConvArgs& a, const ConvPlan& pl, int fmt, const TriConvBnSums*, hipStream_t s) {
    return tri_internal_vox0_launch(pl.g.vox0, a.B, a.in, a.w_hi, a.Kpad, a.out, a.row_mask, a.stats, fmt, s);
}
static int run_voxb(ConvArgs& a, const ConvPlan& pl, int fmt, const TriConvBnSums*, hipStream_t s) {
    return tri_internal_voxb_launch(pl.g.voxb, a.B, a.in, a.w_hi, a.out, a.row_mask, a.stats, fmt, s);
}
static int run_voxg(ConvArgs& a, const ConvPlan& pl, int fmt, const TriConvBnSums*, hipStream_t s) {
    return tri_internal_voxg_launch(pl.g.voxg, a.B, a.Cin, a.Cout, a.Kpad, a.in, a.w_hi, a.out, a.row_mask, a.stats, a.transposed, fmt, s);
}
static int run_stem(ConvArgs& a, const ConvPlan& pl, int fmt, const TriConvBnSums*, hipStream_t s) {
    return fmt == TRI_FMT_F16 ? launch_stem<f16_t>(a, pl.g.stem, s) : launch_stem<bf16_t>(a, pl.g.stem, s);
}
static int run_pw(ConvArgs& a, const ConvPlan& pl, int fmt, const TriConvBnSums*, hipStream_t s) {
    return tri_internal_pw_launch(pl.g.pw, a.B, a.in, a.w_hi, a.Cin, a.Cout, a.Kpad, a.out, a.stats, a.transposed ? 1 : 0, fmt, s);
}
static int run_c64(ConvArgs& a, const ConvPlan& pl, int fmt, const TriConvBnSums* bs, hipStream_t s) {
    return tri_internal_c64_launch(pl.g.c64, a.B, a.IH, a.in, a.w_hi, a.out, bs ? bs->partial : a.stats, a.transposed, a.accumulate, fmt, bs, s);
}
static int run_s2g(ConvArgs& a, const ConvPlan& pl, int fmt, const TriConvBnSums*, hipStream_t s) {
    return tri_internal_s2g_launch(pl.g.s2g, a.B, a.IH, a.IW, a.Cin, a.Cout, a.Kpad, a.in, a.w_hi, a.out, a.stats, fmt, s);
}
static int run_s2d(ConvArgs& a, const ConvPlan& pl, int fmt, const TriConvBnSums*, hipStream_t s) {
    return tri_internal_s2d_launch(pl.also_g, a.B, a.IH, a.in, a.w_hi, a.out, a.accumulate, fmt, s);
}
static int run_halo(ConvArgs& a, const ConvPlan& pl, int fmt, const TriConvBnSums*, hipStream_t s) {
    return fmt == TRI_FMT_F16 ? launch_halo<2, f16_t>(a, pl.halo, s) : launch_halo<2, bf16_t>(a, pl.halo, s);
}

#define CONV_RECORDS(member) [](const ConvPlan& pl) -> int { return pl.g.member; }
static const ConvFamily conv_families[] = {
    {TRI_CONV_VOX0, "conv_vox0_kernel", MODE16, plan_vox0, CF_DGRAD | CF_BNSUMS, CF_ROWS | CF_BIAS_ACT | CF_ACCUM, 0, false,
     false, true, CONV_RECORDS(vox0.grid), run_vox0},
    {TRI_CONV_VOXB, "conv_voxb_kernel", MODE16, plan_voxb, CF_DGRAD | CF_BNSUMS, CF_ROWS | CF_BIAS_ACT | CF_ACCUM, 0, false,
     true, true, CONV_RECORDS(voxb.grid), run_voxb},
    {TRI_CONV_VOXG, "conv_voxg_kernel", MODE16, plan_voxg, CF_BNSUMS, CF_ROWS | CF_BIAS_ACT | CF_ACCUM, 0, false,
     true, true, CONV_RECORDS(voxg.nunits), run_voxg},
    {TRI_CONV_STEM, "conv_stem_kernel", MODE16, plan_stem, CF_DGRAD | CF_EPI | CF_ACCUM | CF_BNSUMS, 0, 0, false,
     false, false, CONV_RECORDS(stem.grid), run_stem},
    {TRI_CONV_PW, "conv_pw_kernel", MODE16_DMA, plan_pw, CF_EPI | CF_ACCUM | CF_BNSUMS, 0, 0, false,
     false, false, nullptr, run_pw},
    {TRI_CONV_C64, "conv_c64_kernel", MODE16_DMA, plan_c64, CF_EPI, 0, CF_STATS, true,
     false, false, CONV_RECORDS(c64.grid), run_c64},
    {TRI_CONV_S2G, "conv_s2g_kernel", MODE16_DMA, plan_s2g, CF_BNSUMS, CF_DGRAD | CF_EPI | CF_ACCUM, 0, false,
     true, false, CONV_RECORDS(s2g.nunits), run_s2g},
    {TRI_CONV_S2D, "conv_s2d_kernel", MODE16_DMA, plan_s2d, CF_FWD | CF_EPI | CF_STATS | CF_BNSUMS, 0, 0, false,
     false, false, nullptr, run_s2d},
    {TRI_CONV_HALO_ROWS, "conv_halo_rows_kernel", MODE16_DMA, plan_halo_rows, CF_EPI | CF_BNSUMS, 0, 0, false,
     false, false, halo_records, run_halo},
    {TRI_CONV_HALO2D, "conv_halo2d_kernel", MODE16_DMA, plan_halo2d, CF_EPI | CF_BNSUMS, 0, 0, false,
     false, false, halo_records, run_halo},
    {TRI_CONV_DMA, "conv_dma_kernel", MODE16_DMA, plan_generic, 0, 0, 0, false, false, false, nullptr, nullptr},
    {TRI_CONV_IGEMM, "conv_igemm_kernel", ANY_MODE, plan_generic, 0, 0, 0, false, false, false, nullptr, nullptr},
};
#undef CONV_RECORDS

static ConvPlan conv_make_plan(const TriConvDesc& v, int split_mode, int row_list = 0) {
    ConvPlan pl{};
    static int no32 = -1;
    if (no32 < 0) no32 = 0;
    if (split_mode == 2 && v.Cin % 64 == 0 && (v.Cout % 64 == 0 || (v.Cout % 32 == 0 && !no32)) && !tri_env_is("TRICOLO_NO_DMA", '1')) pl.dma = 1;
    pl.bn = conv_bn(v.Cout);
    for (const ConvFamily& f : conv_families) {
        if ((f.needs == MODE16 && split_mode != 2) || (f.needs == MODE16_DMA && !pl.dma)) continue;
        const int r = f.plan(v, split_mode, row_list, &pl);
        if (r == PLAN_ALSO) pl.also = &f;
        if (r == PLAN_TAKES) { pl.family = &f; break; }
    }
    if (pl.family->launch) {
        pl.nunits = conv_kpad(v) / (pl.dma ? 64 : 32); pl.ksplit = 1; pl.per_split = pl.nunits;
    }
    if (!pl.tile) pl.tile = pl.bn;
    return pl;
}

static bool conv_takes(const ConvPlan& pl, unsigned feat) {
    const ConvFamily& f = *pl.family;
    return f.launch && !(feat & (f.falls | f.refuses | pl.fall_also));
}

static int conv_refuse(const ConvFamily& f, unsigned what, unsigned wanting) {
    static const char* const names[] = {"forward", "data gradient", "row mask", "row list", "bias / activation", "accumulate", "statistics",
                                        "BatchNorm-backward sums"};
    char msg[400];
    int n = snprintf(msg, sizeof(msg), "conv: this layer runs %s (tri_conv_kernel_family == %d), which takes no", f.kernel, (int)f.code);
    for (int pass = 0; pass < 2; ++pass) {
        const unsigned bits = pass ? wanting : what;
        if (pass && bits) n += snprintf(msg + n, sizeof(msg) - n, " in a call that wants");
        const char* sep = " ";
        for (int b = 0; b < 8; ++b)
            if (bits >> b & 1) { n += snprintf(msg + n, sizeof(msg) - n, "%s%s", sep, names[b]); sep = ", "; }
    }
    if (f.site_mask) snprintf(msg + n, sizeof(msg) - n, "; pass the site mask as row_mask");
    tri_set_error(msg);
    return TRI_ERR_ARG;
}

static ConvArgs conv_args(const TriConvDesc* d, int transposed) {
    const TriConvDesc v = conv_view(*d, transposed);
    ConvArgs a{};
    a.B = v.B; a.ID = v.ID; a.IH = v.IH; a.IW = v.IW; a.Cin = v.Cin;
    a.OD = v.OD; a.OH = v.OH; a.OW = v.OW; a.Cout = v.Cout;
    a.KD = v.KD; a.KH = v.KH; a.KW = v.KW; a.stride = v.stride; a.pd = v.pad_d; a.ph = v.pad_h; a.pw = v.pad_w;
    a.transposed = transposed;
    a.ntaps = v.KD * v.KH * v.KW;
    a.M = v.B * v.OD * v.OH * v.OW;
    return a;
}

static int conv_dispatch(const TriConvDesc* d, ConvArgs& a, int act_fmt, void* workspace, size_t workspace_bytes, hipStream_t stream,
                         const TriConvBnSums* bs = nullptr) {
    if (a.Cin % 4 != 0) { tri_set_error("conv: stored input channels must be a multiple of 4"); return TRI_ERR_ARG; }
    if (a.Cout % 32 != 0) { tri_set_error("conv: output channels must be a multiple of 32"); return TRI_ERR_ARG; }
    if (a.ntaps > 64) { tri_set_error("conv: more than 64 taps unsupported"); return TRI_ERR_UNSUPPORTED; }
    if (a.stride != 1 && a.stride != 2) { tri_set_error("conv: stride must be 1 or 2"); return TRI_ERR_UNSUPPORTED; }
    if (a.KD > 8 || a.KH > 8 || a.KW > 8) { tri_set_error("conv: kernel extent > 8 unsupported"); return TRI_ERR_UNSUPPORTED; }
    if (act_fmt < 0 || act_fmt > 2) { tri_set_error("conv: act_fmt must be 0 (fp32), 1 (bf16) or 2 (f16)"); return TRI_ERR_ARG; }
    a.Kpad = (a.ntaps * a.Cin + 31) / 32 * 32;
    a.cin_shift = ilog2_exact(a.Cin);
    size_t in_bytes = (size_t)a.B * a.ID * a.IH * a.IW * a.Cin * (act_fmt ? 2 : 4);
    if (in_bytes >= ((size_t)1 << 31)) { tri_set_error("conv: input tensor >= 2 GiB (32-bit buffer offsets)"); return TRI_ERR_UNSUPPORTED; }
    a.in_bytes = (unsigned)in_bytes;
    const bool split = a.w_lo != nullptr;
    if (act_fmt && split) { tri_set_error("conv: 16-bit activation storage takes single operands (no lo part)"); return TRI_ERR_ARG; }
    const ConvPlan pl = conv_make_plan(conv_view(*d, a.transposed), act_fmt ? 2 : (split ? 1 : 0), a.row_count ? 1 : 0);
    a.ksplit = pl.ksplit;
    a.steps_per_split = pl.per_split;
    a.nunits = pl.nunits;
    if (a.ksplit > 1) {
        size_t need = (size_t)a.ksplit * a.M * a.Cout * sizeof(float);
        if (workspace == nullptr || workspace_bytes < need) {
            tri_set_error("conv: this layer runs split-K; pass tri_conv_workspace() bytes of scratch");
            return TRI_ERR_ARG;
        }
        a.slab = (float*)workspace;
    }
    a.dOW = make_fastdiv(a.OW); a.dOH = make_fastdiv(a.OH); a.dOD = make_fastdiv(a.OD); a.dCin = make_fastdiv(a.Cin);
    if (a.row_count) {
        if (!a.row_pos) { tri_set_error("conv: row_count needs row_pos"); return TRI_ERR_ARG; }
        if (a.row_mask) { tri_set_error("conv: pass either row_mask or a compact row list"); return TRI_ERR_ARG; }
        if (pl.dma && a.Kpad / 64 > 256) {
            tri_set_error("conv: more than 256 k-steps with a row list (the live-step table of conv_dma_kernel)");
            return TRI_ERR_UNSUPPORTED;
        }
    } else if (a.row_pos && !(pl.dma && pl.ksplit == 1 && !a.row_mask && !a.stats && a.Kpad / 64 <= 256)) {
        a.row_pos = nullptr;
    }
    const unsigned feat = (a.transposed ? CF_DGRAD : CF_FWD) | (a.row_mask ? CF_MASK : 0) | (a.row_count ? CF_ROWS : 0) |
                          ((a.bias || a.act != 0) ? CF_BIAS_ACT : 0) | (a.accumulate ? CF_ACCUM : 0) | (a.stats ? CF_STATS : 0) | (bs ? CF_BNSUMS : 0);
    if (pl.also && !(feat & pl.also->falls)) return pl.also->launch(a, pl, act_fmt, bs, stream);
    const ConvFamily& f = *pl.family;
    if (f.launch) {
        if (!(feat & (f.falls | pl.fall_also))) {
            if (feat & f.refuses) return conv_refuse(f, f.refuses, 0);
            return f.launch(a, pl, act_fmt, bs, stream);
        }
        if (feat & f.fall_refuses) return conv_refuse(f, f.falls & ~CF_BNSUMS, f.fall_refuses);
        if (f.fall_drops_order && !a.row_count) a.row_pos = nullptr;
    }
    if (bs) {
        tri_set_error("conv: this layer's data-gradient kernel takes no BatchNorm-backward sums (tri_conv_dgrad_bn_records == 0)");
        return TRI_ERR_UNSUPPORTED;
    }
    if (pl.dma) return act_fmt == TRI_FMT_F16 ? launch_dma_any<f16_t>(a, pl.bn, stream) : launch_dma_any<bf16_t>(a, pl.bn, stream);
#define TRI_CONV(BN_)                                                                                     \
    (act_fmt == TRI_FMT_F16 ? launch_conv<BN_, 1, f16_t>(a, stream)                                       \
     : act_fmt == TRI_FMT_BF16 ? launch_conv<BN_, 1, bf16_t>(a, stream)                                   \
     : (split ? launch_conv<BN_, 2, float>(a, stream) : launch_conv<BN_, 1, float>(a, stream)))
    if (a.Cout % 128 == 0 && pl.bn != 64) return TRI_CONV(128);
    if (a.Cout % 64 == 0) return TRI_CONV(64);
    return TRI_CONV(32);
#undef TRI_CONV
}

extern "C" int tri_conv_kpad(int ntaps, int cin_stored) { return (ntaps * cin_stored + 31) / 32 * 32; }

static int conv_records(const TriConvDesc& v, const ConvPlan& pl) {
    if (pl.family->records) return pl.family->records(pl);
    const long M = (long)v.B * v.OD * v.OH * v.OW;
    return pl.ksplit > 1 ? (int)((M + 31) / 32) : (int)((M + 127) / 128);
}
extern "C" int tri_conv_num_records(const TriConvDesc* d, int split3, int row_list) { return conv_records(*d, conv_make_plan(*d, split3, row_list)); }
extern "C" int tri_conv_num_mtiles(const TriConvDesc* d, int split3) { return tri_conv_num_records(d, split3, 0); }

static int conv_family_word(int code, int tile, int spu, bool splitk) {
    return code | (tile << TRI_FAMILY_TILE_SHIFT) | ((splitk ? 1 : 0) << TRI_FAMILY_SPLITK_SHIFT) | (spu << TRI_FAMILY_SPU_SHIFT);
}
extern "C" int tri_conv_kernel_family(const TriConvDesc* d, int transposed, int split3) {
    const TriConvDesc v = conv_view(*d, transposed);
    const ConvPlan pl = conv_make_plan(v, split3);
    const unsigned dir = transposed ? CF_DGRAD : CF_FWD;
    if (pl.also && !(dir & pl.also->falls)) return conv_family_word(pl.also->code, pl.bn, 0, false);
    if (conv_takes(pl, dir)) return conv_family_word(pl.family->code, pl.tile, pl.spu, false);
    return conv_family_word(pl.dma ? TRI_CONV_DMA : TRI_CONV_IGEMM, pl.bn, 0, pl.ksplit > 1 || (pl.dma && conv_kpad(v) / 64 > 256));
}

extern "C" size_t tri_conv_workspace(const TriConvDesc* d, int transposed) {
    const TriConvDesc v = conv_view(*d, transposed);
    const long M = (long)v.B * v.OD * v.OH * v.OW;
    size_t need = 0;
    for (int mode = 0; mode < 6; ++mode) {
        const int rl = mode / 3;
        if (rl && (d->KD != 3 || d->stride != 1)) continue;
        const ConvPlan pl = conv_make_plan(v, mode % 3, rl);
        size_t n = pl.ksplit > 1 ? (size_t)pl.ksplit * M * v.Cout * sizeof(float) : 0;
        if (n > need) need = n;
    }
    return need;
}

extern "C" int tri_conv_fwd(const TriConvDesc* d, const void* in, const void* w_hi, const void* w_lo, void* out,
                            const uint8_t* row_mask, const float* bias, int act, int accumulate, float* stats, int act_fmt,
                            void* workspace, size_t workspace_bytes, const int* row_pos, const int* row_count, void* stream) {
    ConvArgs a = conv_args(d, 0);
    a.in = in; a.w_hi = w_hi; a.w_lo = w_lo; a.out = out;
    a.row_mask = row_mask; a.bias = bias; a.stats = stats; a.row_pos = row_pos; a.row_count = row_count;
    a.act = act; a.accumulate = accumulate;
    return conv_dispatch(d, a, act_fmt, workspace, workspace_bytes, (hipStream_t)stream);
}

extern "C" int tri_conv_dgrad(const TriConvDesc* d, const void* dout, const void* wt_hi, const void* wt_lo, void* din,
                              const uint8_t* row_mask, int accumulate, int act_fmt, void* workspace, size_t workspace_bytes,
                              const int* row_pos, const int* row_count, void* stream) {
    ConvArgs a = conv_args(d, 1);
    a.in = dout; a.w_hi = wt_hi; a.w_lo = wt_lo; a.out = din;
    a.row_mask = row_mask; a.row_pos = row_pos; a.row_count = row_count;
    a.accumulate = accumulate;
    return conv_dispatch(d, a, act_fmt, workspace, workspace_bytes, (hipStream_t)stream);
}

extern "C" int tri_conv_dgrad_bn_records(const TriConvDesc* d, int accumulate, int act_fmt) {
    (void)accumulate;
    if (act_fmt != TRI_FMT_BF16 && act_fmt != TRI_FMT_F16) return 0;
    const TriConvDesc v = conv_view(*d, 1);
    const ConvPlan pl = conv_make_plan(v, 2, 0);
    return conv_takes(pl, CF_DGRAD | CF_BNSUMS) ? conv_records(v, pl) : 0;
}
extern "C" int tri_conv_dgrad_bn(const TriConvDesc* d, const void* dout, const void* wt_hi, const void* wt_lo, void* din, int accumulate,
                                 int act_fmt, void* workspace, size_t workspace_bytes, const int* row_pos, const TriConvBnSums* sums,
                                 void* stream) {
    if (!sums || !sums->y || !sums->partial || (!sums->relu_scale != !sums->relu_shift) || (sums->relu_scale && sums->relu_out)) {
        tri_set_error("tri_conv_dgrad_bn: sums needs y, partial and at most one of (relu_scale + relu_shift) / relu_out");
        return TRI_ERR_ARG;
    }
    if (tri_conv_dgrad_bn_records(d, accumulate, act_fmt) == 0) {
        tri_set_error("tri_conv_dgrad_bn: no fused form for this layer (tri_conv_dgrad_bn_records == 0)");
        return TRI_ERR_UNSUPPORTED;
    }
    ConvArgs a = conv_args(d, 1);
    a.in = dout; a.w_hi = wt_hi; a.w_lo = wt_lo; a.out = din;
    a.row_pos = row_pos;
    a.accumulate = accumulate;
    return conv_dispatch(d, a, act_fmt, workspace, workspace_bytes, (hipStream_t)stream, sums);
}
```

tricolo_amd/csrc/conv_vox.h:

```cpp
#pragma once
#include <hip/hip_runtime.h>
#include <stdint.h>
#include "../../include/tricolo_hip.h"

struct TriVox0Geom { int V, TY, grid; };
bool tri_internal_vox0_geometry(const TriConvDesc& d, TriVox0Geom* g);
int tri_internal_vox0_launch(const TriVox0Geom& g, int B, const void* in, const void* w, int kpad, void* out, const uint8_t* mask, float* stats,
                             int act_fmt, hipStream_t stream);

int tri_internal_vox0_wgrad_grid(const TriVox0Geom& g);
int tri_internal_vox0_wgrad_launch(const TriVox0Geom& g, int grid, int B, const void* in, const void* dout, const uint8_t* mask, float* slab,
                                   int act_fmt, hipStream_t stream);

struct TriVoxgGeom { int D, spu, nunits, ct, grid, smem; };
bool tri_internal_voxg_geometry(const TriConvDesc& d, TriVoxgGeom* g);
int tri_internal_voxg_launch(const TriVoxgGeom& g, int B, int cin, int cout, int kpad, const void* in, const void* w, void* out, const uint8_t* mask,
                             float* stats, int transposed, int act_fmt, hipStream_t stream);

struct TriVoxbGeom { int D, nbricks, grid; };
bool tri_internal_voxb_geometry(const TriConvDesc& d, TriVoxbGeom* g);
int tri_internal_voxb_launch(const TriVoxbGeom& g, int B, const void* in, const void* w, void* out, const uint8_t* mask, float* stats, int act_fmt,
                             hipStream_t stream);

struct TriS2gGeom { int ipu, nunits, nrt, PW, PS, NSP, HB, grid, smem; };
bool tri_internal_s2g_geometry(const TriConvDesc& d, TriS2gGeom* g);
int tri_internal_s2g_launch(const TriS2gGeom& g, int B, int IH, int IW, int cin, int cout, int kpad, const void* in, const void* w, void* out,
                            float* stats, int act_fmt, hipStream_t stream);

struct TriC64Geom { int W, TY, nbricks, grid; };
bool tri_internal_c64_geometry(const TriConvDesc& d, TriC64Geom* g);
bool tri_internal_s2d_geometry(const TriConvDesc& d, TriC64Geom* g);
int tri_internal_s2d_launch(const TriC64Geom& g, int B, int H, const void* in, const void* w, void* out, int accumulate, int act_fmt,
                            hipStream_t stream);
int tri_internal_c64_launch(const TriC64Geom& g, int B, int H, const void* in, const void* w, void* out, float* stats, int transposed,
                            int accumulate, int act_fmt, const TriConvBnSums* bs, hipStream_t stream);

struct TriPwGeom { int bn, mtiles, GH, GW, transposed; };
bool tri_internal_pw_geometry(const TriConvDesc& d, TriPwGeom* g);
int tri_internal_pw_launch(const TriPwGeom& g, int B, const void* in, const void* w, int K, int N, int Kpad, void* out, float* stats, int transposed,
                           int act_fmt, hipStream_t stream);
```

tricolo_amd/model/module/img_encoder/mv_cnn.py:

```python
from __future__ import annotations

import contextlib
import os

import torch
import torch.nn as nn

from .... import ops
from ....layers import SideStream, TriModule, linear_bwd, linear_fwd, require_gpu


_DS_FWD = int(os.environ.get("TRICOLO_DS_FWD", "2"))
_DS_BWD = int(os.environ.get("TRICOLO_DS_BWD", "2"))
_PREP_DGRAD_LATE = os.environ.get("TRICOLO_PREP_DGRAD_LATE", "1") != "0"
_BN_PAIR = True
_STEM_BESIDE_WGRAD = os.environ.get("TRICOLO_STEM_BESIDE_WGRAD", "1") != "0"
_PREP_ISSUE = int(os.environ.get("TRICOLO_PREP_ISSUE", "1"))


class _BasicBlockParams(nn.Module):
    def __init__(self, inplanes, planes, stride):
        super().__init__()
        self.conv1 = nn.Conv2d(inplanes, planes, 3, stride, 1, bias=False)
        self.bn1 = nn.BatchNorm2d(planes)
        self.relu = nn.ReLU(inplace=True)
        self.conv2 = nn.Conv2d(planes, planes, 3, 1, 1, bias=False)
        self.bn2 = nn.BatchNorm2d(planes)
        self.downsample = None
        if stride != 1 or inplanes != planes:
            self.downsample = nn.Sequential(nn.Conv2d(inplanes, planes, 1, stride, bias=False), nn.BatchNorm2d(planes))
        self.stride = stride


def _resnet18_trunk_params():
    layers = [nn.Conv2d(3, 64, 7, 2, 3, bias=False), nn.BatchNorm2d(64), nn.ReLU(inplace=True), nn.MaxPool2d(3, 2, 1)]
    inpl = 64
    for planes, stride in ((64, 1), (128, 2), (256, 2), (512, 2)):
        layers.append(nn.Sequential(_BasicBlockParams(inpl, planes, stride), _BasicBlockParams(planes, planes, 1)))
        inpl = planes
    layers.append(nn.AdaptiveAvgPool2d((1, 1)))
    net = nn.Sequential(*layers)
    for m in net.modules():
        if isinstance(m, nn.Conv2d):
            nn.init.kaiming_normal_(m.weight, mode="fan_out", nonlinearity="relu")
    return net


class MVCNNEncoder(TriModule):
    def __init__(self, z_dim, out_dim, cnn_name, num_views, precision=None, **kwargs):
        super().__init__()
        if cnn_name != "resnet18":
            raise NotImplementedError(f"cnn_name={cnn_name!r}: only the resnet18 branch (mv_cnn.py:43-45) is built")
        self.num_views = num_views
        self.precision = precision
        self.net_1 = _resnet18_trunk_params()
        self.net_2 = nn.Linear(512, z_dim)
        self.mlp = nn.Sequential(nn.Linear(z_dim, out_dim), nn.ReLU(inplace=True), nn.Linear(out_dim, out_dim))
        self._geoms = {}
        self.__dict__["_packers"] = {}
        self.__dict__["_packed"] = {}
        self.__dict__["_side"] = SideStream("img")
        self.__dict__["_side_ds"] = SideStream("imgds")
        self.__dict__["_side_prep"] = SideStream("imgprep")
        self.__dict__["split"] = None

    def _prec(self):
        return self.precision or ops.default_precision()

    def _blocks(self):
        return [blk for li in (4, 5, 6, 7) for blk in self.net_1[li]]

    def _param_list(self):
        ps = [self.net_1[0].weight, self.net_1[1].weight, self.net_1[1].bias]
        for blk in self._blocks():
            ps += [blk.conv1.weight, blk.bn1.weight, blk.bn1.bias, blk.conv2.weight, blk.bn2.weight, blk.bn2.bias]
            if blk.downsample is not None:
                ps += [blk.downsample[0].weight, blk.downsample[1].weight, blk.downsample[1].bias]
        ps += [self.net_2.weight, self.net_2.bias, self.mlp[0].weight, self.mlp[0].bias, self.mlp[2].weight, self.mlp[2].bias]
        return ps

    def _geom2d(self, N, H, W, conv: nn.Conv2d):
        key = (N, H, W, id(conv))
        g = self._geoms.get(key)
        if g is None:
            cin, cout = conv.in_channels, conv.out_channels
            k, s, p = conv.kernel_size[0], conv.stride[0], conv.padding[0]
            cs = 4 if cin == 3 else cin
            g = ops.ConvGeom(N, (1, H, W), cin, cs, cout, (1, k, k), s, (0, p, p), (cin * k * k, 1, k * k))
            self._geoms[key] = g
        return g

    def _pack_all(self, N, H, W, prec, train, device):
        key = (N, H, W, train)
        packer = self._packers.get(key)
        if packer is None:
            packer = (ops.WeightPacker(), ops.WeightPacker(), ops.WeightPacker())
            stem_g = self._geom2d(N, H, W, self.net_1[0])
            packer[0].add((id(self.net_1[0]), False), self.net_1[0].weight, stem_g)
            convs = []
            h, w = (H + 6 - 7) // 2 + 1, (W + 6 - 7) // 2 + 1
            h, w = (h + 1) // 2, (w + 1) // 2
            for blk in self._blocks():
                s = blk.conv1.stride[0]
                convs.append((blk.conv1, h, w))
                if blk.downsample is not None:
                    convs.append((blk.downsample[0], h, w))
                h, w = (h + 2 - 3) // s + 1, (w + 2 - 3) // s + 1
                convs.append((blk.conv2, h, w))
            for conv, ch, cw in convs:
                g = self._geom2d(N, ch, cw, conv)
                packer[1].add((id(conv), False), conv.weight, g)
                if train:
                    packer[2 if _PREP_DGRAD_LATE else 1].add((id(conv), True), conv.weight, g, transposed=True)
            self._packers[key] = packer
        packed = dict(packer[0].run(prec, device))
        ev = None
        if _PREP_ISSUE:
            ev = torch.cuda.Event()
            ev.record()

        def pack_rest():
            with torch.cuda.stream(self._side_prep.fork(event=ev)):
                rest = packer[1].run(prec, device)
            self._packed.update(rest)
            self.__dict__["_prep_pending"] = [t for pair in rest.values() for t in pair if t is not None]

        def pack_dgrad():
            with torch.cuda.stream(self._side_prep.fork(event=ev)):
                rest = packer[2].run(prec, device)
            self._packed.update(rest)
            self.__dict__["_prep_pending_dgrad"] = [t for pair in rest.values() for t in pair if t is not None]
        self.__dict__["_pack_dgrad"] = pack_dgrad if (train and _PREP_DGRAD_LATE and packer[2].entries) else None
        if ev is None and self.__dict__["_pack_dgrad"] is not None:
            ev = torch.cuda.Event()
            ev.record()
        self.__dict__["_pack_rest"] = pack_rest
        self._packed = packed
        if not _PREP_ISSUE:
            self._run_pack_rest()
        return packed

    def _run_pack_rest(self):
        fn = self.__dict__.get("_pack_rest")
        if fn is not None:
            self.__dict__["_pack_rest"] = None
            fn()

    def _run_pack_dgrad(self):
        fn = self.__dict__.get("_pack_dgrad")
        if fn is not None:
            self.__dict__["_pack_dgrad"] = None
            fn()

    def _join_packing_dgrad(self):
        self._run_pack_dgrad()
        pend = self.__dict__.get("_prep_pending_dgrad")
        if pend:
            self._side_prep.join(*pend)
            self.__dict__["_prep_pending_dgrad"] = None

    def _join_packing(self):
        pend = self.__dict__.get("_prep_pending")
        if pend:
            self._side_prep.join(*pend)
            self.__dict__["_prep_pending"] = None

    def _conv_bn(self, x, conv, bn, prec, train, after_conv=None):
        N, _, H, W, _ = x.shape
        g = self._geom2d(N, H, W, conv)
        packed = self._packed[(id(conv), False)]
        if train:
            y, stats = ops.conv_fwd(x, g, packed, want_stats=True)
            if after_conv is not None:
                after_conv()
            co = ops.bn_finalize(stats, g.cout, bn.weight, bn.bias, bn.running_mean, bn.running_var, bn.num_batches_tracked,
                                 count_host=g.M, momentum=bn.momentum, eps=bn.eps)
        else:
            y = ops.conv_fwd(x, g, packed)
            co = ops.bn_eval_coeffs(g.cout, bn.weight, bn.bias, bn.running_mean, bn.running_var, bn.eps)
        return y, co, g

    N_LOWER_BLOCKS = 4

    def _lower_params(self):
        return self._param_list()[:3 + sum(9 if b.downsample is not None else 6 for b in self._blocks()[:self.N_LOWER_BLOCKS])]

    def _upper_params(self):
        return self._param_list()[len(self._lower_params()):]

    def _run_block(self, blk, x, prec, train, save, store):
        ds = blk.downsample is not None
        mode = _DS_FWD if (ds and train) else 0
        shortcut = []
        ev = None
        if mode == 2:
            ev = torch.cuda.Event()
            ev.record()

        def run_shortcut():
            with torch.cuda.stream(self._side_ds.fork(x, event=ev)):
                shortcut.extend(self._conv_bn(x, blk.downsample[0], blk.downsample[1], prec, train))
        if ds and not mode:
            run_shortcut()
        fine = ops.TIMELINE is not None and ops.TIMELINE.get("fine")
        y1, co1, g1 = self._conv_bn(x, blk.conv1, blk.bn1, prec, train, after_conv=run_shortcut if mode else None)
        if ds:
            yd, cod, gd = shortcut
        if fine:
            ops.stamp(f"image.fwd.c{y1.shape[-1]}.conv1+fin")
        a1 = ops.bn_act(y1, co1, relu=True)
        if fine:
            ops.stamp(f"image.fwd.c{y1.shape[-1]}.act1")
        y2, co2, g2 = self._conv_bn(a1, blk.conv2, blk.bn2, prec, train)
        if fine:
            ops.stamp(f"image.fwd.c{y1.shape[-1]}.conv2+fin")
        if ds:
            self._side_ds.join(yd, cod.scale, cod.shift)
            out = ops.bn_act(y2, co2, relu=True, res=yd, res_co=cod)
        else:
            yd = cod = gd = None
            out = ops.bn_act(y2, co2, relu=True, res=x)
        if fine:
            ops.stamp(f"image.fwd.c{y1.shape[-1]}.act2")
        if save:
            store.append((x, y1, co1, g1, a1, y2, co2, g2, yd, cod, gd, out))
        return out

    def _forward_lower(self, images, save: bool):
        prec, train = self._prec(), self.training
        N = images.shape[0]
        if N % self.num_views:
            raise RuntimeError("mat shape: number of images is not a multiple of num_views")
        self._packed = self._pack_all(N, images.shape[2], images.shape[3], prec, train and save, images.device)
        if images.dtype == torch.uint8:
            x0 = ops.nchw3_u8_to_nhwc4(images, dtype=ops.act_dtype(prec))
        else:
            x0 = ops.nchw3_to_nhwc4(images, dtype=ops.act_dtype(prec))
        def after_stem_conv():
            if _PREP_ISSUE == 1:
                self._run_pack_rest()
        y, co, g = self._conv_bn(x0, self.net_1[0], self.net_1[1], prec, train, after_conv=after_stem_conv)
        x, parg = ops.maxpool2d_fwd(y, want_arg=save, bn=co)
        self._run_pack_rest()
        ops.stamp("image.fwd.stem.end")
        saved = {"stem": (x0, y, co, g, parg), "blocks": [], "N": N}
        self._join_packing()
        for blk in self._blocks()[:self.N_LOWER_BLOCKS]:
            x = self._run_block(blk, x, prec, train, save, saved["blocks"])
        ops.stamp("image.fwd.layer2.end")
        return x, saved

    def _forward_upper(self, x, save: bool):
        prec, train = self._prec(), self.training
        N = x.shape[0]
        B = N // self.num_views
        saved = {"blocks": [], "B": B, "N": N}
        for blk in self._blocks()[self.N_LOWER_BLOCKS:]:
            x = self._run_block(blk, x, prec, train, save, saved["blocks"])
        ops.stamp("image.fwd.layer4.end")
        if save:
            self._run_pack_dgrad()
        pooled, arg = ops.avgpool_viewmax_fwd(x, B, self.num_views)
        f = linear_fwd(pooled, self.net_2.weight, self.net_2.bias, 0, prec)
        h = linear_fwd(f, self.mlp[0].weight, self.mlp[0].bias, 1, prec)
        o = linear_fwd(h, self.mlp[2].weight, self.mlp[2].bias, 0, prec)
        zz, norm = ops.l2norm_fwd(o)
        if save:
            self._join_packing_dgrad()
            saved.update(feat_shape=tuple(x.shape), pooled=pooled, arg=arg, f=f, h=h, o=o, z=zz, norm=norm)
        return zz, saved

    def _forward_impl(self, images, save: bool):
        x2, lo = self._forward_lower(images, save)
        zz, hi = self._forward_upper(x2, save)
        return zz, {"lower": lo, "upper": hi}

    def _backward_blocks(self, blocks, saved_blocks, dout, gr, prec, ugs, batch=None):
        side = self._side
        pattern = "m"
        turn = [0]

        def wgrad_async(x, dy, g, w):
            ch = pattern[turn[0] % len(pattern)]
            turn[0] += 1
            if ch == "m":
                gr[w] = ops.conv_wgrad(x, dy, g, w, prec, out_scale=ugs, batch=batch)
                return
            with torch.cuda.stream(side.fork(x, dy)):
                gr[w] = ops.conv_wgrad(x, dy, g, w, prec, out_scale=ugs)

        dout_sums = None
        for bi in range(len(blocks) - 1, -1, -1):
            blk, sv = blocks[bi], saved_blocks[bi]
            x, y1, co1, g1, a1, y2, co2, g2, yd, cod, gd, out = sv
            pair = (_BN_PAIR and blk.downsample is not None and batch is not None and dout_sums is None and yd is not None
                    and yd.shape == y2.shape and ops._sync_world() == 1)
            dyd_pair = None
            if pair:
                (dy2, gr[blk.bn2.weight], gr[blk.bn2.bias], dyd_pair, gr[blk.downsample[1].weight],
                 gr[blk.downsample[1].bias]) = ops.bn_bwd_pair(y2, co2, blk.bn2.weight, yd, cod, blk.downsample[1].weight, dout, out, g2.M,
                                                               g_masked=dout, out_scale=ugs)
            else:
                dy2, gr[blk.bn2.weight], gr[blk.bn2.bias] = ops.bn_bwd(y2, dout, co2, blk.bn2.weight, count_host=g2.M, inplace=False,
                                                                       relu_out=out, g_masked=dout, out_scale=ugs, partial=dout_sums)
            g = dout
            fine = ops.TIMELINE is not None and ops.TIMELINE.get("fine")
            tag = f"image.bwd.c{y2.shape[-1]}.b{bi}"
            if fine:
                ops.stamp(tag + ".bn2")
            mode = _DS_BWD if (blk.downsample is not None and batch is not None) else 0
            ev = None
            if mode == 2:
                ev = torch.cuda.Event()
                ev.record()

            def shortcut_bwd():
                with torch.cuda.stream(self._side_ds.fork(g, yd, event=ev)):
                    if dyd_pair is not None:
                        return dyd_pair, ops.conv_dgrad(dyd_pair, gd, self._packed[(id(blk.downsample[0]), True)])
                    dyd_, gr[blk.downsample[1].weight], gr[blk.downsample[1].bias] = ops.bn_bwd(
                        yd, g, cod, blk.downsample[1].weight, count_host=gd.M, inplace=False, out_scale=ugs)
                    if batch is None:
                        gr[blk.downsample[0].weight] = ops.conv_wgrad(x, dyd_, gd, blk.downsample[0].weight, prec, out_scale=ugs)
                    return dyd_, ops.conv_dgrad(dyd_, gd, self._packed[(id(blk.downsample[0]), True)])
            if blk.downsample is not None and not mode:
                dyd, dx = shortcut_bwd()
            wgrad_async(a1, dy2, g2, blk.conv2.weight)
            da1, sums1 = ops.conv_dgrad(dy2, g2, self._packed[(id(blk.conv2), True)], bn_sums=(y1, co1, None))
            if mode:
                dyd, dx = shortcut_bwd()
            if fine:
                ops.stamp(tag + ".dgrad2")
            dy1, gr[blk.bn1.weight], gr[blk.bn1.bias] = ops.bn_bwd(y1, da1, co1, blk.bn1.weight, count_host=g1.M, relu=True, out_scale=ugs,
                                                                   partial=sums1)
            if fine:
                ops.stamp(tag + ".bn1")
            wgrad_async(x, dy1, g1, blk.conv1.weight)
            if blk.downsample is not None:
                if batch is None:
                    self._side_ds.join(dx, gr[blk.downsample[0].weight], gr[blk.downsample[1].weight], gr[blk.downsample[1].bias])
                else:
                    self._side_ds.join(dx, dyd, gr[blk.downsample[1].weight], gr[blk.downsample[1].bias])
                    gr[blk.downsample[0].weight] = ops.conv_wgrad(x, dyd, gd, blk.downsample[0].weight, prec, out_scale=ugs, batch=batch)
            else:
                dx = g
            if bi > 0:
                prev = saved_blocks[bi - 1]
                dx, dout_sums = ops.conv_dgrad(dy1, g1, self._packed[(id(blk.conv1), True)], out=dx, accumulate=True,
                                               bn_sums=(prev[5], None, prev[11]))
            else:
                dx, dout_sums = ops.conv_dgrad(dy1, g1, self._packed[(id(blk.conv1), True)], out=dx, accumulate=True), None
            if fine:
                ops.stamp(tag + ".dgrad1")
            dout = dx
        side.join(*[v for v in gr.values() if v.dim() == 4])
        return dout

    def _backward_upper(self, saved, dz, batch=None):
        prec, B = self._prec(), saved["B"]
        gr = {}
        ops.stamp("image.bwd.start")
        self._join_packing_dgrad()
        own = batch is None
        if own:
            batch = ops.wgrad_batch(dz.device)
        do = ops.l2norm_bwd(saved["z"], saved["norm"], dz)
        dh, gr[self.mlp[2].weight], gr[self.mlp[2].bias] = linear_bwd(saved["h"], self.mlp[2].weight, saved["o"], do, 0, prec)
        df, gr[self.mlp[0].weight], gr[self.mlp[0].bias] = linear_bwd(saved["f"], self.mlp[0].weight, saved["h"], dh, 1, prec)
        dp, gr[self.net_2.weight], gr[self.net_2.bias] = linear_bwd(saved["pooled"], self.net_2.weight, saved["f"], df, 0, prec)
        gs = ops.grad_scale(prec)
        dout = ops.avgpool_viewmax_bwd(dp, saved["arg"], saved["feat_shape"], B, self.num_views, dtype=ops.act_dtype(prec), scale=gs)
        ops.stamp("image.bwd.heads.end")
        dx2 = self._backward_blocks(self._blocks()[self.N_LOWER_BLOCKS:], saved["blocks"], dout, gr, prec, 1.0 / gs, batch)
        ops.stamp("image.bwd.layer3.end")
        if own and batch is not None:
            batch.flush()
        return dx2, [gr[p] for p in self._upper_params()]

    def _backward_lower(self, saved, dout, batch=None, stem_side=None):
        prec = self._prec()
        ugs = 1.0 / ops.grad_scale(prec)
        gr = {}
        self._join_packing_dgrad()
        own = batch is None
        if own:
            batch = ops.wgrad_batch(dout.device)
        dout = self._backward_blocks(self._blocks()[:self.N_LOWER_BLOCKS], saved["blocks"], dout, gr, prec, ugs, batch)
        x0, y, co, g0, parg = saved["stem"]
        ops.stamp("image.bwd.layer1.end")
        side = None
        if y.shape[2] % 2 == 0 and y.shape[3] % 2 == 0 and stem_side is not None and _STEM_BESIDE_WGRAD and batch is not None:
            ev = torch.cuda.Event()
            ev.record()
            if batch.prelaunch():
                side = stem_side.fork(dout, event=ev)
        with (torch.cuda.stream(side) if side is not None else contextlib.nullcontext()):
            stem = ops.maxpool_bn_bwd_wgrad(x0, y, parg, dout, co, self.net_1[1].weight, g0, self.net_1[0].weight, prec, out_scale=ugs, batch=batch,
                                            pooled=saved["blocks"][0][0])
        if side is not None and not torch.cuda.is_current_stream_capturing():
            for t_ in stem:
                t_.record_stream(torch.cuda.current_stream())
        gr[self.net_1[0].weight], gr[self.net_1[1].weight], gr[self.net_1[1].bias] = stem
        if own and batch is not None:
            batch.flush()
        return [gr[p] for p in self._lower_params()]

    def _backward_impl(self, saved, dz):
        batch = ops.wgrad_batch(dz.device)
        dx2, up = self._backward_upper(saved["upper"], dz, batch)
        lo = self._backward_lower(saved["lower"], dx2, batch, stem_side=self._side)
        if batch is not None:
            batch.flush(side=self._side)
        ops.stamp("image.bwd.end")
        return lo + up

    def forward(self, x, data_dict=None):
        require_gpu(x, "MVCNNEncoder")
        if torch.is_grad_enabled() and any(p.requires_grad for p in self.parameters()):
            if self.split is not None:
                x2 = _MVCNNLowerFn.apply(self, x, *self._lower_params())
                return _MVCNNUpperFn.apply(self, self.split.gate(x2), *self._upper_params())
            return _MVCNNTowerFn.apply(self, x, *self._param_list())
        z, _ = self._forward_impl(x, save=False)
        return z


class _MVCNNTowerFn(torch.autograd.Function):
    @staticmethod
    def forward(ctx, module, images, *params):
        z, saved = module._forward_impl(images, save=True)
        ctx.module, ctx.saved = module, saved
        return z

    @staticmethod
# ... 37 lines not shown
```

tricolo_amd/ops.py:

```python
from __future__ import annotations

import collections
import math
import os

import torch

from . import _C
from ._C import check, lib, make_desc, ptr, stream

_PRECISIONS = ("bf16", "bf16x3", "f16")
_FMT = {torch.float32: 0, torch.bfloat16: 1, torch.float16: 2}
F16_GRAD_SCALE = float(os.environ.get("TRICOLO_F16_GRAD_SCALE", "4096"))
if not (F16_GRAD_SCALE >= 1.0 and math.frexp(F16_GRAD_SCALE)[0] == 0.5):
    raise ValueError(f"TRICOLO_F16_GRAD_SCALE={F16_GRAD_SCALE!r}: must be a power of two >= 1 (the kernels divide it out exactly)")
_default_precision = os.environ.get("TRICOLO_PRECISION", "bf16x3")


def set_default_precision(p: str):
    global _default_precision
    if p not in _PRECISIONS:
        raise ValueError(f"precision must be one of {_PRECISIONS}")
    _default_precision = p

# ... 156 lines not shown

def _conv_mode(x, lo) -> int:
    return 1 if lo is not None else (2 if x.dtype != torch.float32 else 0)


class ConvGeom:

    def __init__(self, B, in_grid, cin, cin_stored, cout, kernel, stride, pad, weight_strides):
        ID, IH, IW = in_grid
        KD, KH, KW = kernel
        pd, ph, pw = pad
        OD = (ID + 2 * pd - KD) // stride + 1
        OH = (IH + 2 * ph - KH) // stride + 1
        OW = (IW + 2 * pw - KW) // stride + 1
        self.B, self.in_grid, self.out_grid = B, (ID, IH, IW), (OD, OH, OW)
        self.cin, self.cin_stored, self.cout = cin, cin_stored, cout
        self.kernel, self.stride, self.pad = kernel, stride, pad
        self.ntaps = KD * KH * KW
        self.strides = weight_strides
        self.desc = make_desc(B, ID, IH, IW, cin_stored, OD, OH, OW, cout, KD, KH, KW, stride, pd, ph, pw)
        self.kpad = lib().tri_conv_kpad(self.ntaps, cin_stored)
        self.kpad_t = lib().tri_conv_kpad(self.ntaps, cout)
        self.M = B * OD * OH * OW
        self.M_in = B * ID * IH * IW
        self.num_mtiles = {m: lib().tri_conv_num_mtiles(_C.C.byref(self.desc), m) for m in (0, 1, 2)}
        self.num_records_rows = {m: lib().tri_conv_num_records(_C.C.byref(self.desc), m, 1) for m in (0, 1, 2)}
        self.kernel_family = {(tr, m): lib().tri_conv_kernel_family(_C.C.byref(self.desc), 1 if tr else 0, m)
                              for tr in (False, True) for m in (0, 1, 2)}
        self.wgrad_ws = lib().tri_conv_wgrad_workspace(_C.C.byref(self.desc))
        routes = [lib().tri_conv_wgrad_route(_C.C.byref(self.desc), 1, feat) for feat in (0, WGRAD_MASK)]
        self.wgrad_krow = routes[0] >= 0 and routes[0] & FAMILY_CODE_MASK == 7
        self.wgrad_brick = routes[1] >= 0 and routes[1] & FAMILY_CODE_MASK == 6
        self._plans = {}
        self.fwd_ws = lib().tri_conv_workspace(_C.C.byref(self.desc), 0)
        self.dgrad_ws = lib().tri_conv_workspace(_C.C.byref(self.desc), 1) if cin == cin_stored and cin % 32 == 0 else 0

    def dgrad_row_order(self, device):
        if self.stride != 2 or self.ntaps == 1:
            return None
        t = self._plans.get(("rowpos", device))
        if t is None:
            ID, IH, IW = self.in_grid
            pd, ph, pw = self.pad
            pos = torch.arange(self.M_in, dtype=torch.int64)
            x, r = pos % IW, pos // IW
            y, r = r % IH, r // IH
            z = r % ID
            cls = (((z + pd) & 1) << 2) | (((y + ph) & 1) << 1) | ((x + pw) & 1)
            order = torch.sort(cls * self.M_in + pos).indices
            t = order.to(torch.int32).to(device)
            self._plans[("rowpos", device)] = t
        return t

    def family(self, transposed: bool, mode: int) -> ConvFamily:
        return CONV_FAMILIES[self.kernel_family[(transposed, mode)] & FAMILY_CODE_MASK]

    def brick(self, transposed: bool, mode: int) -> bool:
        return self.family(transposed, mode).site_mask

    def packed_frag(self, transposed: bool, precision: str, storage=None) -> int:
        storage = storage or act_dtype(precision)
        mode = 1 if precision == "bf16x3" else (2 if storage != torch.float32 else 0)
        return int(self.family(transposed, mode).frag)

    def check_packed(self, packed, transposed: bool, x):
        need = int(self.family(transposed, _conv_mode(x, packed[1])).frag)
        if getattr(packed[0], "tri_frag", 0) != need:
            raise RuntimeError("conv: the packed operand was ordered for another plan (row-major vs fragment-major): pack it with "
                               "pack_weight(..., storage=<dtype of the activations>)")

    def voxg_spu(self, transposed: bool, mode: int) -> int:
        return (self.kernel_family[(transposed, mode)] >> FAMILY_SPU_SHIFT) & 127

    def splitk(self, transposed: bool, mode: int) -> bool:
        return bool(self.kernel_family[(transposed, mode)] >> FAMILY_SPLITK_SHIFT & 1)

    def dgrad_bn_records(self, accumulate: bool, fmt: int) -> int:
        c = self.__dict__.setdefault("_dgrad_bn", {})
        k = (bool(accumulate), fmt)
        if k not in c:
            c[k] = int(lib().tri_conv_dgrad_bn_records(_C.C.byref(self.desc), 1 if accumulate else 0, fmt))
        return c[k]

    def wgrad_group(self, fmt: int):
        c = self.__dict__.setdefault("_wgrad_group", {})
        if fmt not in c:
            fam, tiles, steps = _C.C.c_int(), _C.C.c_int(), _C.C.c_int()
            check(lib().tri_conv_wgrad_group_info(_C.C.byref(self.desc), fmt, _C.C.byref(fam), _C.C.byref(tiles), _C.C.byref(steps)),
                  "tri_conv_wgrad_group_info")
            c[fmt] = (fam.value, tiles.value, steps.value)
        return c[fmt]

    def wgrad_route(self, fmt: int, features: int) -> int:
        c = self.__dict__.setdefault("_wgrad_route", {})
        if (fmt, features) not in c:
            word = lib().tri_conv_wgrad_route(_C.C.byref(self.desc), fmt, features)
            if word < 0:
                check(word, "tri_conv_wgrad_route")
            c[(fmt, features)] = word
        return c[(fmt, features)]

    def plan(self, device):
        pl = self._plans.get(device)
        if pl is None:
            pl = torch.empty((lib().tri_conv_plan_bytes(_C.C.byref(self.desc)),), dtype=torch.uint8, device=device)
            check(lib().tri_conv_plan_build(_C.C.byref(self.desc), ptr(pl), stream()), "tri_conv_plan_build")
            self._plans[device] = pl
        return pl

    @property
    def flops(self):
        return 2 * self.M * self.ntaps * self.cin * self.cout


def pack_weight(w: torch.Tensor, g: ConvGeom, precision: str, transposed: bool = False, storage=None):
    s_co, s_tap, s_ci = g.strides
    if not transposed:
        rows, inner, inner_pad, kpad, s_row, s_inner = g.cout, g.cin, g.cin_stored, g.kpad, s_co, s_ci
    else:
        rows, inner, inner_pad, kpad, s_row, s_inner = g.cin_stored, g.cout, g.cout, g.kpad_t, s_ci, s_co
        if g.cin != g.cin_stored:
            raise RuntimeError("dgrad operand requested for a layer with padded input channels")
    hi = torch.empty((rows, kpad), dtype=torch.float16 if precision == "f16" else torch.bfloat16, device=w.device)
    lo = torch.empty_like(hi) if precision == "bf16x3" else None
    frag = g.packed_frag(transposed, precision, storage)
    check(lib().tri_weight_prep(ptr(_f32(w)), s_row, s_tap, s_inner, rows, g.ntaps, inner, inner_pad, ptr(hi), ptr(lo), _abf(hi),
                                frag, stream()), "tri_weight_prep")
    hi.tri_frag = frag
    return hi, lo


class WeightPacker:

    def __init__(self):
        self.entries = {}
        self._tables = {}

    def add(self, key, param, g: "ConvGeom", transposed: bool = False):
        if key not in self.entries:
            self.entries[key] = (param, g, transposed)
            self._tables.clear()

    def _build(self, precision, device):
        descs = (_C.TriPrepDesc * len(self.entries))()
        bufs = {}
        for i, (key, (w, g, tr)) in enumerate(self.entries.items()):
            s_co, s_tap, s_ci = g.strides
            if not tr:
                rows, inner, inner_pad, kpad, s_row, s_inner = g.cout, g.cin, g.cin_stored, g.kpad, s_co, s_ci
            else:
                rows, inner, inner_pad, kpad, s_row, s_inner = g.cin_stored, g.cout, g.cout, g.kpad_t, s_ci, s_co
            hi = torch.empty((rows, kpad), dtype=torch.float16 if precision == "f16" else torch.bfloat16, device=device)
            lo = torch.empty_like(hi) if precision == "bf16x3" else None
            bufs[key] = (hi, lo)
            d = descs[i]
            d.fmt = _abf(hi)
            d.w, d.hi, d.lo = w.data_ptr(), hi.data_ptr(), (lo.data_ptr() if lo is not None else None)
            d.s_row, d.s_tap, d.s_inner = s_row, s_tap, s_inner
            d.rows, d.ntaps, d.inner, d.inner_pad, d.kpad = rows, g.ntaps, inner, inner_pad, kpad
            d.frag = hi.tri_frag = g.packed_frag(tr, precision)
        raw = torch.frombuffer(bytearray(bytes(descs)), dtype=torch.uint8).to(device)
        snap = tuple(w.data_ptr() for (w, _, _) in self.entries.values())
        return raw, len(self.entries), bufs, snap

    def run(self, precision, device):
        tab = self._tables.get(precision)
        if tab is None or tab[3] != tuple(w.data_ptr() for (w, _, _) in self.entries.values()):
            tab = self._build(precision, device)
            self._tables[precision] = tab
        raw, n, bufs, _ = tab
        check(lib().tri_weight_prep_multi(ptr(raw), n, stream()), "tri_weight_prep_multi")
        return bufs


def conv_fwd(x, g: ConvGeom, packed, row_mask=None, bias=None, act=0, want_stats=False, out=None, accumulate=False, rows=None):
    hi, lo = packed
    g.check_packed(packed, False, x)
    OD, OH, OW = g.out_grid
    if out is None:
        out = torch.empty((g.B, OD, OH, OW, g.cout), dtype=x.dtype, device=x.device)
    assert out.dtype == x.dtype
    nrec = (g.num_records_rows if rows else g.num_mtiles)[_conv_mode(x, lo)]
    stats = torch.empty((nrec, 2, g.cout), dtype=torch.float32, device=x.device) if want_stats else None
    ws = _workspace(g.fwd_ws, x.device) if g.fwd_ws else None
    check(_timed(_igemm_symbol(g, False, lo is not None, x), _flops(g, rows, row_mask),
                 lambda: lib().tri_conv_fwd(_C.C.byref(g.desc), ptr(_act(x)), ptr(hi), ptr(lo), ptr(out), ptr(row_mask), ptr(bias),
                                            act, 1 if accumulate else 0, ptr(stats), _abf(x), ptr(ws),
                                            ws.numel() if ws is not None else 0, ptr(rows[0]) if rows else None,
                                            ptr(rows[1]) if rows else None, stream())), "tri_conv_fwd")
    return (out, stats) if want_stats else out


_ROW_ORDER = True


_DGRAD_BN_MODE = os.environ.get("TRICOLO_DGRAD_BN", "2")
_DGRAD_BN = _DGRAD_BN_MODE != "0"


def conv_dgrad(dout, g: ConvGeom, packed_t, row_mask=None, out=None, accumulate=False, rows=None, bn_sums=None):
    hi, lo = packed_t
    g.check_packed(packed_t, True, dout)
    ID, IH, IW = g.in_grid
    if out is None:
        out = torch.empty((g.B, ID, IH, IW, g.cin_stored), dtype=dout.dtype, device=dout.device)
    assert out.dtype == dout.dtype
    ws = _workspace(g.dgrad_ws, dout.device) if g.dgrad_ws else None
    rowpos = g.dgrad_row_order(dout.device) if (row_mask is None and rows is None and _ROW_ORDER) else None
    if rows is not None:
        rowpos = rows[0]
    if bn_sums is not None:
        y, co, relu_out = bn_sums
        nrec = g.dgrad_bn_records(accumulate, _abf(dout)) if (_DGRAD_BN and not (accumulate and _DGRAD_BN_MODE == "2") and row_mask is None and rows is None and lo is None
                                                               and (relu_out is not None) == bool(accumulate)
                                                               and (co is not None) != (relu_out is not None)) else 0
        if nrec == 0:
            return conv_dgrad(dout, g, packed_t, row_mask=row_mask, out=out, accumulate=accumulate, rows=rows), None
        assert y.dtype == out.dtype and y.numel() == out.numel()
        partial = torch.empty((nrec, 2, g.cin_stored), dtype=torch.float32, device=dout.device)
        sums = _C.TriConvBnSums(ptr(y), ptr(co.scale) if co is not None else None, ptr(co.shift) if co is not None else None,
                                ptr(relu_out), ptr(partial))
        check(_timed(_igemm_symbol(g, True, False, dout), g.flops,
                     lambda: lib().tri_conv_dgrad_bn(_C.C.byref(g.desc), ptr(_act(dout)), ptr(hi), None, ptr(out), 1 if accumulate else 0,
                                                     _abf(dout), ptr(ws), ws.numel() if ws is not None else 0, ptr(rowpos),
                                                     _C.C.byref(sums), stream())), "tri_conv_dgrad_bn")
        return out, partial
    check(_timed(_igemm_symbol(g, True, lo is not None, dout), _flops(g, rows, row_mask),
                 lambda: lib().tri_conv_dgrad(_C.C.byref(g.desc), ptr(_act(dout)), ptr(hi), ptr(lo), ptr(out), ptr(row_mask),
                                              1 if accumulate else 0, _abf(dout), ptr(ws), ws.numel() if ws is not None else 0,
                                              ptr(rowpos), ptr(rows[1]) if rows else None, stream())), "tri_conv_dgrad")
    return out


_wgrad_ws = {}


def _workspace(nbytes: int, device) -> torch.Tensor:
    key = (device, torch.cuda.current_stream().cuda_stream)
    ws = _wgrad_ws.get(key)
    if ws is None or ws.numel() < nbytes:
        ws = torch.empty(max(nbytes, 1 << 20), dtype=torch.uint8, device=device)
        _wgrad_ws[key] = ws
    return ws


_WGRAD_GROUPED = os.environ.get("TRICOLO_WGRAD_GROUPED", "1") != "0"
_WGRAD_JOBS = os.environ.get("TRICOLO_WGRAD_JOBS", "1") != "0"
_WGRAD_JOB_TILES = {1: 512, 2: 448, 3: 256, 4: 512, 5: 512, 7: 512}


_WGRAD_REDUCE_OVERLAP = os.environ.get("TRICOLO_WGRAD_REDUCE_OVERLAP", "1") != "0"


_GUARD_NOTE = None


def set_guard_note(note):
    global _GUARD_NOTE
    _GUARD_NOTE = note


def guard_noted(g, note) -> bool:
    tag = g.__dict__.pop("_tri_noted", None)
    return tag is not None and tag == (note.data_ptr(), g._version)


class WgradBatch:
    _arenas = {}

    def __init__(self, device, group_jobs: bool | None = None):
        self.device = device
        self.group_jobs = _WGRAD_JOBS if group_jobs is None else bool(group_jobs)
        self.chunks = WgradBatch._arenas.setdefault((device, torch.cuda.current_stream().cuda_stream, torch.cuda.is_current_stream_capturing()), [])
        self.ci, self.off, self.descs = 0, 0, []
        self.queues = {}
        self._pre = None
        self.dws = {}

    @property
    def jobs(self):
        return [j for q in self.queues.values() for j in q[0]]

    def add_job(self, family, tiles, job, keep, flops, sym):
        q = self.queues.setdefault(family, [[], 0])
        if q[0] and (q[1] + tiles > _WGRAD_JOB_TILES[family] or len(q[0]) == _C.TRI_WGRAD_JOBS_MAX):
            self.launch_jobs(family)
            q = self.queues.setdefault(family, [[], 0])
        q[0].append((job, keep, flops, sym))
        q[1] += tiles

    def launch_jobs(self, family=None):
        for fam in ([family] if family is not None else sorted(self.queues)):
            pending = self.queues.pop(fam, [[], 0])[0]
            n = len(pending)
            if not n:
                continue
            arr = (_C.TriWgradJob * n)(*[j[0] for j in pending])
            pend = (_C.TriWgradReduce * n)()
# ... 139 lines not shown
    global _SYNC_BN
    _SYNC_BN = bool(flag)


def _sync_world() -> int:
    if not _SYNC_BN:
        return 1
    import torch.distributed as dist
    return dist.get_world_size() if (dist.is_available() and dist.is_initialized()) else 1


def _sync_sum(t: torch.Tensor) -> torch.Tensor:
    from .parallel import all_reduce_sum
    if t.dtype == torch.int32:
        u = t.to(torch.int64)
        all_reduce_sum(u)
        return u.to(torch.int32)
    all_reduce_sum(t)
    return t


def bn_finalize(stats, C, gamma, beta, running_mean, running_var, nbt, count_dev=None, count_host=0, momentum=0.1, eps=1e-5):
    world = _sync_world()
    if world > 1:
        if torch.cuda.is_current_stream_capturing():
            raise RuntimeError("sync_bn: the BatchNorm collectives cannot be captured into a HIP graph - run the step eagerly")
        stats = _sync_sum(stats.sum(0, keepdim=True).contiguous())
        if count_dev is not None:
            count_dev = _sync_sum(count_dev.clone())
        else:
            count_host = int(count_host) * world
    co = BNCoeffs(C, stats.device)
    check(lib().tri_bn_finalize(ptr(stats), stats.shape[0], C, ptr(count_dev), int(count_host), ptr(gamma), ptr(beta),
                                ptr(running_mean), ptr(running_var), ptr(nbt), momentum, eps, ptr(co.mean), ptr(co.invstd),
                                ptr(co.scale), ptr(co.shift), stream()), "tri_bn_finalize")
    return co


def bn_eval_coeffs(C, gamma, beta, running_mean, running_var, eps=1e-5):
    co = BNCoeffs(C, gamma.device)
    check(lib().tri_bn_eval_coeffs(C, ptr(gamma), ptr(beta), ptr(running_mean), ptr(running_var), eps, ptr(co.mean),
                                   ptr(co.invstd), ptr(co.scale), ptr(co.shift), stream()), "tri_bn_eval_coeffs")
    return co


def bn_act(y, co: BNCoeffs, relu=True, res=None, res_co: BNCoeffs | None = None):
    C = y.shape[-1]
    out = torch.empty_like(y)
    check(lib().tri_bn_act(ptr(_act(y)), ptr(co.scale), ptr(co.shift), ptr(res), ptr(res_co.scale) if res_co else None,
                           ptr(res_co.shift) if res_co else None, ptr(out), y.numel() // C, C, 1 if relu else 0, _abf(y), stream()),
          "tri_bn_act")
    return out


def relu_bwd(dout, out, inplace=True):
    g = dout if inplace else torch.empty_like(dout)
    check(lib().tri_relu_bwd(ptr(_act(dout)), ptr(out), ptr(g), dout.numel(), _abf(dout), stream()), "tri_relu_bwd")
    return g


def _bn_bwd_finalize(partial, nblk, C, count_dev, count_host, gamma, co: "BNCoeffs", out_scale):
    buf = torch.empty((5, C), dtype=torch.float32, device=partial.device)
    check(lib().tri_bn_bwd_finalize(ptr(partial), nblk, C, ptr(count_dev), int(count_host), ptr(gamma), ptr(co.mean),
                                    ptr(co.invstd), ptr(buf[0]), ptr(buf[1]), ptr(buf[2]), ptr(buf[3]), ptr(buf[4]), float(out_scale), stream()),
          "tri_bn_bwd_finalize")
    world = _sync_world()
    if world > 1:
        tot = _sync_sum(partial.sum(0, keepdim=True).contiguous())
        if count_dev is not None:
            count_dev = _sync_sum(count_dev.clone())
        else:
            count_host = int(count_host) * world
        gbuf = torch.empty((5, C), dtype=torch.float32, device=partial.device)
        check(lib().tri_bn_bwd_finalize(ptr(tot), 1, C, ptr(count_dev), int(count_host), ptr(gamma), ptr(co.mean), ptr(co.invstd), ptr(gbuf[0]),
                                        ptr(gbuf[1]), ptr(gbuf[2]), ptr(gbuf[3]), ptr(gbuf[4]), float(out_scale), stream()), "tri_bn_bwd_finalize")
        buf = torch.stack([buf[0], buf[1], gbuf[2], gbuf[3], gbuf[4]])
    return buf


_BN_SMALL = True


def _bn_bwd_finish(y, g, partial, co: BNCoeffs, gamma, count_dev, count_host, out_scale, dy, row_mask=None, keep_inactive=False, rows=None,
                   rs=None, rb=None, relu_out=None, g_masked=None):
    C = y.shape[-1]
    buf = _bn_bwd_finalize(partial, partial.shape[0], C, count_dev, count_host, gamma, co, out_scale)
    if rows is not None:
        check(lib().tri_bn_bwd_apply_rows(ptr(y), ptr(g), ptr(buf[2]), ptr(buf[3]), ptr(buf[4]), ptr(dy), C, ptr(rows[0]), ptr(rows[1]),
                                          rows[0].numel(), _abf(y), stream()), "tri_bn_bwd_apply_rows")
    else:
        check(lib().tri_bn_bwd_apply(ptr(y), ptr(g), ptr(buf[2]), ptr(buf[3]), ptr(buf[4]), ptr(row_mask), ptr(dy), y.numel() // C, C, ptr(rs), ptr(rb),
                                     ptr(relu_out), ptr(g_masked), 1 if keep_inactive else 0, _abf(y), stream()), "tri_bn_bwd_apply")
    return dy, buf[0], buf[1]


def bn_bwd(y, g, co: BNCoeffs, gamma, count_dev=None, count_host=0, row_mask=None, inplace=True, relu=False, relu_out=None,
           g_masked=None, out_scale: float = 1.0, keep_inactive: bool = False, partial=None):
    rs, rb = (co.scale, co.shift) if relu else (None, None)
    C = y.shape[-1]
    M = y.numel() // C
    assert y.dtype == g.dtype
    dy = g if inplace else torch.empty_like(g)
    if partial is None and _BN_SMALL and M <= 512 and C % 8 == 0 and C >= 64 and _sync_world() == 1:
        buf = torch.empty((2, C), dtype=torch.float32, device=y.device)
        check(lib().tri_bn_bwd_small(ptr(_act(y)), ptr(_act(g)), M, C, ptr(count_dev), int(count_host), ptr(gamma), ptr(co.mean), ptr(co.invstd),
                                     ptr(rs), ptr(rb), ptr(relu_out), ptr(g_masked), ptr(row_mask), 1 if keep_inactive else 0, ptr(dy), ptr(buf[0]),
                                     ptr(buf[1]), float(out_scale), _abf(y), stream()), "tri_bn_bwd_small")
        return dy, buf[0], buf[1]
    if partial is None:
        partial = torch.empty((lib().tri_bn_bwd_num_blocks(M), 2, C), dtype=torch.float32, device=y.device)
        check(lib().tri_bn_bwd_reduce(ptr(_act(y)), ptr(_act(g)), M, C, ptr(partial), ptr(rs), ptr(rb), ptr(relu_out), ptr(row_mask), _abf(y), stream()),
              "tri_bn_bwd_reduce")
    assert partial.shape[1:] == (2, C)
    return _bn_bwd_finish(y, g, partial, co, gamma, count_dev, count_host, out_scale, dy, row_mask=row_mask, keep_inactive=keep_inactive,
                          rs=rs, rb=rb, relu_out=relu_out, g_masked=g_masked)


def bn_bwd_pair(ya, coa: BNCoeffs, gamma_a, yb, cob: BNCoeffs, gamma_b, g, relu_out, count_host, g_masked=None, out_scale: float = 1.0):
    C = ya.shape[-1]
    M = ya.numel() // C
    assert ya.dtype == g.dtype == yb.dtype == relu_out.dtype and ya.shape == yb.shape and _sync_world() == 1
    nblk = lib().tri_bn_bwd_num_blocks(M)
    partial = torch.empty((2, nblk, 2, C), dtype=torch.float32, device=ya.device)
    check(lib().tri_bn_bwd_pair_reduce(ptr(_act(ya)), ptr(_act(yb)), ptr(_act(g)), ptr(relu_out), M, C, ptr(partial[0]), ptr(partial[1]), _abf(ya),
                                       stream()), "tri_bn_bwd_pair_reduce")
    buf = torch.empty((2, 5, C), dtype=torch.float32, device=ya.device)
    check(lib().tri_bn_bwd_pair_finalize(ptr(partial[0]), ptr(partial[1]), nblk, C, int(count_host), ptr(gamma_a), ptr(coa.mean), ptr(coa.invstd),
                                         ptr(buf[0]), ptr(gamma_b), ptr(cob.mean), ptr(cob.invstd), ptr(buf[1]), float(out_scale), stream()),
          "tri_bn_bwd_pair_finalize")
    dya, dyb = torch.empty_like(ya), torch.empty_like(yb)
    check(lib().tri_bn_bwd_pair_apply(ptr(ya), ptr(yb), ptr(g), ptr(relu_out), ptr(buf[0]), ptr(buf[1]), ptr(dya), ptr(dyb), ptr(g_masked), M, C,
                                      _abf(ya), stream()), "tri_bn_bwd_pair_apply")
    return dya, buf[0, 0], buf[0, 1], dyb, buf[1, 0], buf[1, 1]


def bn_relu_pool3d_fwd(y, co: BNCoeffs, mask, B, D, C, want_mask: bool = True):
    Do = D // 2
    pooled = torch.empty((B, Do, Do, Do, C), dtype=y.dtype, device=y.device)
    mask_out = torch.empty(((B * Do ** 3 + 31) // 32 * 32,), dtype=torch.uint8, device=y.device) if want_mask else None
    check(lib().tri_bn_relu_pool3d_fwd(ptr(_act(y)), ptr(co.scale), ptr(co.shift), ptr(mask), B, D, C, ptr(pooled), ptr(mask_out),
                                       _abf(y), stream()), "tri_bn_relu_pool3d_fwd")
    return pooled, mask_out


_VOX_ROWS = True
_ROUTE_RED = True
_POOL3D_ROUTES = {(False, False): "tri_pool3d_bwd_route", (True, False): "tri_pool3d_bwd_route_rows",
                  (False, True): "tri_pool3d_bwd_route_reduce", (True, True): "tri_pool3d_bwd_route_rows_reduce"}


def _pool3d_bwd_route(y, co: BNCoeffs, mask, pooled, dpooled, B, D, C, rows_out=None, sums=False):
    assert dpooled.dtype == y.dtype and pooled.dtype == y.dtype
    g, partial = torch.empty_like(y), None
    args = (ptr(_act(y)), ptr(co.scale), ptr(co.shift), ptr(mask), ptr(pooled), ptr(_act(dpooled)), B, D, C, ptr(g))
    args += (ptr(rows_out[0]), ptr(rows_out[1])) if rows_out is not None else ()
    if sums:
        nblk = (lib().tri_pool3d_bwd_route_reduce_num_blocks if rows_out is None else lib().tri_pool3d_bwd_route_rows_num_blocks)(B, D, C)
        partial = torch.empty((nblk, 2, C), dtype=torch.float32, device=y.device)
        args += (ptr(partial),)
    name = _POOL3D_ROUTES[(rows_out is not None, sums)]
    check(getattr(lib(), name)(*args, _abf(y), stream()), name)
    return g, partial


def pool3d_bwd_route(y, co: BNCoeffs, mask, pooled, dpooled, B, D, C):
    return _pool3d_bwd_route(y, co, mask, pooled, dpooled, B, D, C)[0]


def pool3d_bwd_route_rows(y, co: BNCoeffs, mask, pooled, dpooled, B, D, C, rows_out):
    return _pool3d_bwd_route(y, co, mask, pooled, dpooled, B, D, C, rows_out)[0]


def bn_bwd_rows(y, g, co: BNCoeffs, gamma, rows, out_scale: float = 1.0):
    C = y.shape[-1]
    scratch = torch.empty((lib().tri_bn_bwd_rows_scratch(C),), dtype=torch.uint8, device=y.device)
    buf = torch.empty((2, C), dtype=torch.float32, device=y.device)
    check(lib().tri_bn_bwd_rows(ptr(_act(y)), ptr(_act(g)), C, ptr(rows[0]), ptr(rows[1]), rows[0].numel(), ptr(gamma), ptr(co.mean),
                                ptr(co.invstd), ptr(g), ptr(buf[0]), ptr(buf[1]), float(out_scale), ptr(scratch), _abf(y), stream()),
          "tri_bn_bwd_rows")
    return g, buf[0], buf[1]


def pool3d_bn_bwd(y, co: BNCoeffs, mask, pooled, dpooled, B, D, C, gamma, count_dev, out_scale: float = 1.0, fused: bool = True,
                  keep_inactive: bool = False, rows=None, rows_out=None):
    c4 = C % 4 == 0
    sums = fused and c4 and 256 % (C // 4) == 0
    lists = _VOX_ROWS and c4 and y.numel() // C > 16384
    own = rows is not None and keep_inactive
    if lists and sums and _ROUTE_RED and rows_out is not None:
        g, partial = _pool3d_bwd_route(y, co, mask, pooled, dpooled, B, D, C, rows_out, sums=True)
    elif lists and (rows_out is not None or own) and _sync_world() == 1:
        g, partial = _pool3d_bwd_route(y, co, mask, pooled, dpooled, B, D, C, rows_out)
    else:
        own = False
        g, partial = _pool3d_bwd_route(y, co, mask, pooled, dpooled, B, D, C, sums=sums)
    if partial is not None:
        return _bn_bwd_finish(y, g, partial, co, gamma, count_dev, 0, out_scale, g, row_mask=None if own else mask, keep_inactive=keep_inactive,
                              rows=rows if own else None)
# ... 721 lines not shown
```

Measured before the change: 13380.

## Fuse BN apply/activation prologues into c64 conv forward and data-gradient kernels

Adds a pre-pass mode to the 64-channel conv kernel. While the input slab is staged into shared memory, it applies a BN affine, optional residual add and ReLU on forward, or the BN backward apply with ReLU masking on the data gradient. The transformed tile is also written out as a by-product, so the separate elementwise bn_act / bn_bwd_apply passes and one read of the tensor can be dropped. In exchange it uses extra loads, shared-memory tables and register pressure in the conv prologue, and it needs new Python plumbing so callers can route through the fused path.

New measurement: 13610, median of 6. 1.7% higher.

```diff
diff --git a/include/tricolo_hip.h b/include/tricolo_hip.h
--- a/include/tricolo_hip.h
+++ b/include/tricolo_hip.h
@@ -107,6 +107,29 @@
 int tri_conv_dgrad_bn_records(const TriConvDesc* d, int accumulate, int act_fmt);
 int tri_conv_dgrad_bn(const TriConvDesc* d, const void* dout, const void* wt_hi, const void* wt_lo, void* din, int accumulate,
                       int act_fmt, void* workspace, size_t workspace_bytes, const int* row_pos, const TriConvBnSums* sums, void* stream);
+typedef struct TriConvPreAct {
+    const float* scale;
+    const float* shift;
+    const void* res;
+    void* act_out;
+} TriConvPreAct;
+int tri_conv_fwd_preact_supported(const TriConvDesc* d, int want_stats, int act_fmt);
+int tri_conv_fwd_preact(const TriConvDesc* d, const void* y, const void* w_hi, void* out, float* stats ,
+                        int act_fmt, const TriConvPreAct* pre, void* stream);
+typedef struct TriConvPreBn {
+    const void* y;
+    const float* c1;
+    const float* c2;
+    const float* c3;
+    const float* relu_scale;
+    const float* relu_shift;
+    const void* relu_out;
+    void* dy;
+    void* g_masked;
+} TriConvPreBn;
+int tri_conv_dgrad_prebn_supported(const TriConvDesc* d, int accumulate, int with_sums, int act_fmt);
+int tri_conv_dgrad_prebn(const TriConvDesc* d, const void* g, const void* wt_hi, void* din, int accumulate, int act_fmt,
+                         const TriConvPreBn* pre, const TriConvBnSums* sums , void* stream);
 size_t tri_conv_wgrad_workspace(const TriConvDesc* d);
 size_t tri_conv_plan_bytes(const TriConvDesc* d);
 int tri_conv_plan_build(const TriConvDesc* d, void* plan, void* stream);
diff --git a/tricolo_amd/_C.py b/tricolo_amd/_C.py
--- a/tricolo_amd/_C.py
+++ b/tricolo_amd/_C.py
@@ -34,6 +34,14 @@
 
 class TriConvBnSums(C.Structure):
     _fields_ = [("y", C.c_void_p), ("relu_scale", C.c_void_p), ("relu_shift", C.c_void_p), ("relu_out", C.c_void_p), ("partial", C.c_void_p)]
+
+
+class TriConvPreAct(C.Structure):
+    _fields_ = [("scale", C.c_void_p), ("shift", C.c_void_p), ("res", C.c_void_p), ("act_out", C.c_void_p)]
+
+
+class TriConvPreBn(C.Structure):
+    _fields_ = [(n, C.c_void_p) for n in ("y", "c1", "c2", "c3", "relu_scale", "relu_shift", "relu_out", "dy", "g_masked")]
 
 
 TRI_WGRAD_JOBS_MAX = 12
@@ -66,6 +74,10 @@
     "tri_conv_dgrad": (I, [DP, P, P, P, P, P, I, I, P, Z, P, P, P]),
     "tri_conv_dgrad_bn_records": (I, [DP, I, I]),
     "tri_conv_dgrad_bn": (I, [DP, P, P, P, P, I, I, P, Z, P, C.POINTER(TriConvBnSums), P]),
+    "tri_conv_fwd_preact_supported": (I, [DP, I, I]),
+    "tri_conv_fwd_preact": (I, [DP, P, P, P, P, I, C.POINTER(TriConvPreAct), P]),
+    "tri_conv_dgrad_prebn_supported": (I, [DP, I, I, I]),
+    "tri_conv_dgrad_prebn": (I, [DP, P, P, P, I, I, C.POINTER(TriConvPreBn), C.POINTER(TriConvBnSums), P]),
     "tri_conv_wgrad_workspace": (Z, [DP]),
     "tri_conv_plan_bytes": (Z, [DP]),
     "tri_conv_plan_build": (I, [DP, P, P]),
diff --git a/tricolo_amd/csrc/bn_pool.hip b/tricolo_amd/csrc/bn_pool.hip
--- a/tricolo_amd/csrc/bn_pool.hip
+++ b/tricolo_amd/csrc/bn_pool.hip
@@ -80,16 +80,16 @@
     for (long i = (long)blockIdx.x * blockDim.x + threadIdx.x; i < total4; i += (long)gridDim.x * blockDim.x) {
         int c = (int)(i % C4);
         float4 v = Act<T>::ld4(y + i * 4), s = scale[c], b = shift[c];
-        v.x = __fmaf_rn(v.x, s.x, b.x); v.y = __fmaf_rn(v.y, s.y, b.y); v.z = __fmaf_rn(v.z, s.z, b.z); v.w = __fmaf_rn(v.w, s.w, b.w);
+        bn_act_affine(v, s, b);
         if (res) {
             float4 r = Act<T>::ld4(res + i * 4);
             if (rscale) {
                 float4 rs = rscale[c], rb = rshift[c];
                 r.x = r.x * rs.x + rb.x; r.y = r.y * rs.y + rb.y; r.z = r.z * rs.z + rb.z; r.w = r.w * rs.w + rb.w;
             }
-            v.x += r.x; v.y += r.y; v.z += r.z; v.w += r.w;
-        }
-        if (relu) { v.x = fmaxf(v.x, 0.f); v.y = fmaxf(v.y, 0.f); v.z = fmaxf(v.z, 0.f); v.w = fmaxf(v.w, 0.f); }
+            bn_act_add(v, r);
+        }
+        if (relu) bn_act_relu(v);
         Act<T>::st4(out + i * 4, v);
     }
 }
@@ -281,16 +281,16 @@
             float4 yv = Act<T>::ld4(y + i * 4), gv = Act<T>::ld4(g + i * 4), a = c1[c], b = c2[c], d = c3[c];
             if (MASK == 1) {
                 const float4 s4 = rs[c], b4 = rb[c];
-                gv.x = __fmaf_rn(yv.x, s4.x, b4.x) > 0.f ? gv.x : 0.f; gv.y = __fmaf_rn(yv.y, s4.y, b4.y) > 0.f ? gv.y : 0.f;
-                gv.z = __fmaf_rn(yv.z, s4.z, b4.z) > 0.f ? gv.z : 0.f; gv.w = __fmaf_rn(yv.w, s4.w, b4.w) > 0.f ? gv.w : 0.f;
+                gv.x = bn_bwd_mask_affine(gv.x, yv.x, s4.x, b4.x); gv.y = bn_bwd_mask_affine(gv.y, yv.y, s4.y, b4.y);
+                gv.z = bn_bwd_mask_affine(gv.z, yv.z, s4.z, b4.z); gv.w = bn_bwd_mask_affine(gv.w, yv.w, s4.w, b4.w);
             }
             if (MASK == 2) {
                 const float4 ov = Act<T>::ld4(ro + i * 4);
-                gv.x = ov.x > 0.f ? gv.x : 0.f; gv.y = ov.y > 0.f ? gv.y : 0.f; gv.z = ov.z > 0.f ? gv.z : 0.f; gv.w = ov.w > 0.f ? gv.w : 0.f;
+                gv.x = bn_bwd_mask_out(gv.x, ov.x); gv.y = bn_bwd_mask_out(gv.y, ov.y); gv.z = bn_bwd_mask_out(gv.z, ov.z); gv.w = bn_bwd_mask_out(gv.w, ov.w);
                 if (gm) Act<T>::st4(gm + i * 4, gv);
             }
-            o.x = a.x * gv.x + b.x + d.x * yv.x; o.y = a.y * gv.y + b.y + d.y * yv.y;
-            o.z = a.z * gv.z + b.z + d.z * yv.z; o.w = a.w * gv.w + b.w + d.w * yv.w;
+            o.x = bn_bwd_apply1(a.x, b.x, d.x, gv.x, yv.x); o.y = bn_bwd_apply1(a.y, b.y, d.y, gv.y, yv.y);
+            o.z = bn_bwd_apply1(a.z, b.z, d.z, gv.z, yv.z); o.w = bn_bwd_apply1(a.w, b.w, d.w, gv.w, yv.w);
         }
         Act<T>::st4(dy + i * 4, o);
     }
diff --git a/tricolo_amd/csrc/common.h b/tricolo_amd/csrc/common.h
--- a/tricolo_amd/csrc/common.h
+++ b/tricolo_amd/csrc/common.h
@@ -106,6 +106,15 @@
     }
     static __device__ __forceinline__ float rnd(float v) { return (float)(f16_t)v; }
 };
+__device__ __forceinline__ void bn_act_affine(float4& v, const float4& s, const float4& b) {
+    v.x = __fmaf_rn(v.x, s.x, b.x); v.y = __fmaf_rn(v.y, s.y, b.y); v.z = __fmaf_rn(v.z, s.z, b.z); v.w = __fmaf_rn(v.w, s.w, b.w);
+}
+__device__ __forceinline__ void bn_act_add(float4& v, const float4& r) { v.x += r.x; v.y += r.y; v.z += r.z; v.w += r.w; }
+__device__ __forceinline__ void bn_act_relu(float4& v) { v.x = fmaxf(v.x, 0.f); v.y = fmaxf(v.y, 0.f); v.z = fmaxf(v.z, 0.f); v.w = fmaxf(v.w, 0.f); }
+__device__ __forceinline__ float bn_bwd_mask_affine(float g, float y, float s, float b) { return __fmaf_rn(y, s, b) > 0.f ? g : 0.f; }
+__device__ __forceinline__ float bn_bwd_mask_out(float g, float o) { return o > 0.f ? g : 0.f; }
+__device__ __forceinline__ float bn_bwd_apply1(float a, float b, float d, float g, float y) { return a * g + b + d * y; }
+
 #define TRI_ACT_DISPATCH(fmt, ...)                                       \
     do {                                                                 \
         if ((fmt) == TRI_FMT_BF16) { using T = bf16_t; __VA_ARGS__; }    \
diff --git a/tricolo_amd/csrc/conv_c64.hip b/tricolo_amd/csrc/conv_c64.hip
--- a/tricolo_amd/csrc/conv_c64.hip
+++ b/tricolo_amd/csrc/conv_c64.hip
@@ -22,7 +22,50 @@
     const float* bs_scale;
     const float* bs_shift;
     int bs_mode;
+    const void* pre_y;
+    const void* pre_aux;
+    const float* pre_tab[5];
+    void* pre_out;
+    void* pre_out2;
 };
+
+enum { C64_PRE_NONE = 0, C64_PRE_F = 1, C64_PRE_A = 2, C64_PRE_B = 3 };
+
+template <typename AT, int PRE>
+__device__ __forceinline__ void c64_pre_chunk(uint4& v, const uint4& yraw, const uint4& araw, const float* tab, bool has_aux, uint4& g2) {
+    AT* const pv = (AT*)&v;
+    const AT* const py = (const AT*)&yraw;
+    const AT* const pa = (const AT*)&araw;
+    AT* const p2 = (AT*)&g2;
+#pragma unroll
+    for (int hf = 0; hf < 2; ++hf) {
+        const float* tb = tab + 4 * hf;
+        if (PRE == C64_PRE_F) {
+            float4 x = Act<AT>::ld4(pv + 4 * hf);
+            bn_act_affine(x, *(const float4*)tb, *(const float4*)(tb + 64));
+            if (has_aux) bn_act_add(x, Act<AT>::ld4(pa + 4 * hf));
+            bn_act_relu(x);
+            Act<AT>::st4(pv + 4 * hf, x);
+        } else {
+            float4 gv = Act<AT>::ld4(pv + 4 * hf);
+            const float4 yv = Act<AT>::ld4(py + 4 * hf);
+            const float4 a = *(const float4*)tb, b = *(const float4*)(tb + 64), d = *(const float4*)(tb + 128);
+            if (PRE == C64_PRE_A) {
+                const float4 s4 = *(const float4*)(tb + 192), b4 = *(const float4*)(tb + 256);
+                gv.x = bn_bwd_mask_affine(gv.x, yv.x, s4.x, b4.x); gv.y = bn_bwd_mask_affine(gv.y, yv.y, s4.y, b4.y);
+                gv.z = bn_bwd_mask_affine(gv.z, yv.z, s4.z, b4.z); gv.w = bn_bwd_mask_affine(gv.w, yv.w, s4.w, b4.w);
+            } else {
+                const float4 ov = Act<AT>::ld4(pa + 4 * hf);
+                gv.x = bn_bwd_mask_out(gv.x, ov.x); gv.y = bn_bwd_mask_out(gv.y, ov.y); gv.z = bn_bwd_mask_out(gv.z, ov.z); gv.w = bn_bwd_mask_out(gv.w, ov.w);
+                Act<AT>::st4(p2 + 4 * hf, gv);
+            }
+            float4 o;
+            o.x = fp32_rounded(bn_bwd_apply1(a.x, b.x, d.x, gv.x, yv.x)); o.y = fp32_rounded(bn_bwd_apply1(a.y, b.y, d.y, gv.y, yv.y));
+            o.z = fp32_rounded(bn_bwd_apply1(a.z, b.z, d.z, gv.z, yv.z)); o.w = fp32_rounded(bn_bwd_apply1(a.w, b.w, d.w, gv.w, yv.w));
+            Act<AT>::st4(pv + 4 * hf, o);
+        }
+    }
+}
 
 template <int W, int TY>
 struct C64Cfg {
@@ -37,11 +80,14 @@
     static constexpr int MAXC = (ITEMS + 255) / 256;
     static constexpr int WROW = 9 * 64 * 2 + 16;
     static constexpr size_t SMEM = (size_t)SLAB > (size_t)64 * WROW ? (size_t)SLAB : (size_t)64 * WROW;
+    static constexpr size_t TABS = 512;
+    static constexpr size_t PRE_TABS = 5 * 64 * sizeof(float);
+    static_assert(2 * (SMEM + TABS + PRE_TABS) <= 160 * 1024, "two workgroups per CU");
     static_assert(RUNS == 8 || RUNS == 4, "a brick is 8 or 4 runs (half of them per wave pair)");
     static_assert(2 * PITCH + 4096 < 65536, "fragment-read immediates");
 };
 
-template <typename AT, int W, int TY, bool ACCUM, bool BS>
+template <typename AT, int W, int TY, bool ACCUM, bool BS, int PRE>
 __global__ __launch_bounds__(256, 2) void conv_c64_kernel(const ConvC64Args p) {
     typedef C64Cfg<W, TY> C;
     typedef typename OpOf<AT>::E E;
@@ -92,6 +138,15 @@
     constexpr int bsm = BS ? (ACCUM ? 2 : 1) : 0;
     float* const bsc = (float*)(smem + C::SMEM);
     if (bsm == 1 && t < 128) bsc[t] = t < 64 ? p.bs_scale[t] : p.bs_shift[t - 64];
+    constexpr int NTAB = PRE == C64_PRE_F ? 2 : (PRE == C64_PRE_A ? 5 : (PRE == C64_PRE_B ? 3 : 0));
+    float* const pco = bsc + 128;
+    if (PRE && t < 64) {
+#pragma unroll
+        for (int k = 0; k < NTAB; ++k) pco[k * 64 + t] = p.pre_tab[k][t];
+    }
+    const bool pre_aux = PRE == C64_PRE_B || (PRE == C64_PRE_F && p.pre_aux != nullptr);
+    const __amdgpu_buffer_rsrc_t yrs = __builtin_amdgcn_make_buffer_rsrc((void*)(PRE >= C64_PRE_A ? p.pre_y : p.in), 0, p.in_bytes, 0x00020000);
+    const __amdgpu_buffer_rsrc_t ars = __builtin_amdgcn_make_buffer_rsrc((void*)(pre_aux ? p.pre_aux : p.in), 0, p.in_bytes, 0x00020000);
     constexpr int NZ = C::RPR * 16 - W + 2;
     for (int i = t; i < (TY + 2) * NZ * 8; i += 256) {
         const int row = i / (NZ * 8), rem = i - row * (NZ * 8), zp = rem >> 3, q = rem & 7;
@@ -110,7 +165,7 @@
             else if (bsm == 2 && t < 2 * LINES) warm = *(const unsigned*)((const AT*)p.bs_ro + b0 + (size_t)(t - LINES) * 64);
         }
         __syncthreads();
-        {
+        if (!PRE) {
             uint4 pre[C::MAXC];
             int dst[C::MAXC];
 #pragma unroll
@@ -128,6 +183,43 @@
 #pragma unroll
             for (int u = 0; u < C::MAXC; ++u)
                 if (dst[u] >= 0) *(uint4*)(slab + dst[u]) = pre[u];
+        } else {
+            constexpr int NT = PRE == C64_PRE_B ? 3 : 2, BSZ = 6 / NT;
+            const float* const tab = pco + 8 * (t & 7);
+#pragma unroll
+            for (int u0 = 0; u0 < C::MAXC; u0 += BSZ) {
+                uint4 pre[BSZ], py[BSZ], pa[BSZ];
+                int dst[BSZ];
+                unsigned vo[BSZ];
+#pragma unroll
+                for (int k = 0; k < BSZ; ++k) {
+                    if (u0 + k >= C::MAXC) continue;
+                    const int i = t + (u0 + k) * 256;
+                    const int yy = i / C::CPR, cc = i % C::CPR;
+                    const int sx = C::XOFF + (cc >> 3), q = cc & 7;
+                    const int gy = y0 - 1 + yy;
+                    const bool inside = i < C::ITEMS;
+                    dst[k] = inside ? (yy * C::PITCH + sx * 128 + ((q ^ ((sx >> 1) & 7)) << 4)) | (yy >= 1 && yy <= TY ? 1 : 0) : -1;
+                    const bool ok = inside && (unsigned)gy < (unsigned)p.H;
+                    vo[k] = ok ? (unsigned)(((n * p.H + gy) * W) * 128 + cc * 16) : 0x80000000u;
+                    pre[k] = __builtin_bit_cast(uint4, __builtin_amdgcn_raw_buffer_load_b128(irs, vo[k], 0, 0));
+                    if (PRE >= C64_PRE_A) py[k] = __builtin_bit_cast(uint4, __builtin_amdgcn_raw_buffer_load_b128(yrs, vo[k], 0, 0));
+                    if (pre_aux) pa[k] = __builtin_bit_cast(uint4, __builtin_amdgcn_raw_buffer_load_b128(ars, vo[k], 0, 0));
+                }
+#pragma unroll
+                for (int k = 0; k < BSZ; ++k) {
+                    if (u0 + k >= C::MAXC) continue;
+                    if (dst[k] < 0) continue;
+                    uint4 v = pre[k], g2 = make_uint4(0u, 0u, 0u, 0u);
+                    if ((int)vo[k] >= 0) c64_pre_chunk<AT, PRE>(v, py[k], pa[k], tab, pre_aux, g2);
+                    *(uint4*)(slab + (dst[k] & ~1)) = v;
+                    if (dst[k] & 1) {
+                        *(uint4*)((char*)p.pre_out + vo[k]) = v;
+                        if (PRE == C64_PRE_B) *(uint4*)((char*)p.pre_out2 + vo[k]) = g2;
+                    }
+                }
+                __builtin_amdgcn_sched_barrier(0);
+            }
         }
         if (bsm) asm volatile("" :: "v"(warm));
         __syncthreads();
@@ -240,20 +332,28 @@
     return true;
 }
 
-template <typename AT, int W, int TY, bool ACCUM, bool BS>
+template <typename AT, int W, int TY, bool ACCUM, bool BS, int PRE>
 static int c64_launch_t(const ConvC64Args& a, int grid, hipStream_t stream) {
     typedef C64Cfg<W, TY> C;
+    constexpr size_t smem = C::SMEM + C::TABS + (PRE ? C::PRE_TABS : 0);
     static bool attr = false;
     if (!attr) {
-        hipFuncSetAttribute((const void*)conv_c64_kernel<AT, W, TY, ACCUM, BS>, hipFuncAttributeMaxDynamicSharedMemorySize, (int)C::SMEM + 512);
+        hipFuncSetAttribute((const void*)conv_c64_kernel<AT, W, TY, ACCUM, BS, PRE>, hipFuncAttributeMaxDynamicSharedMemorySize, (int)smem);
         attr = true;
     }
-    conv_c64_kernel<AT, W, TY, ACCUM, BS><<<grid, 256, C::SMEM + 512, stream>>>(a);
+    conv_c64_kernel<AT, W, TY, ACCUM, BS, PRE><<<grid, 256, smem, stream>>>(a);
     return tri_check_launch("tri_conv(c64)");
 }
 
+bool tri_internal_c64_pre_form(int form, int transposed, int accumulate, int sums) {
+    if (form == C64_PRE_F) return !transposed && !accumulate && !sums;
+    if (form == C64_PRE_A) return transposed && accumulate;
+    if (form == C64_PRE_B) return transposed && !accumulate && sums;
+    return false;
+}
+
 int tri_internal_c64_launch(const TriC64Geom& g, int B, int H, const void* in, const void* w, void* out, float* stats, int transposed,
-                            int accumulate, int act_fmt, const TriConvBnSums* bs, hipStream_t stream) {
+                            int accumulate, int act_fmt, const TriConvBnSums* bs, const TriConvPre* pre, hipStream_t stream) {
     ConvC64Args a{};
     a.in = in; a.w = w; a.out = out; a.stats = stats;
     if (bs) {
@@ -264,30 +364,59 @@
             return TRI_ERR_UNSUPPORTED;
         }
     }
+    const int form = pre ? pre->form : C64_PRE_NONE;
+    if (pre) {
+        if (!tri_internal_c64_pre_form(form, transposed, accumulate, bs != nullptr)) {
+            tri_set_error("conv(c64): pre-pass forms: activation on a forward, bn1's apply on an accumulated data gradient, bn2's on a plain one with sums");
+            return TRI_ERR_UNSUPPORTED;
+        }
+        const int ntab = form == C64_PRE_F ? 2 : (form == C64_PRE_A ? 5 : 3);
+        bool ok = pre->out != nullptr && (form == C64_PRE_F || pre->y) && (form != C64_PRE_B || (pre->aux && pre->out2));
+        for (int k = 0; k < ntab; ++k) ok = ok && pre->tab[k];
+        const void* const ins[3] = {in, pre->y, pre->aux};
+        for (const void* q : ins) ok = ok && (!q || (q != pre->out && q != pre->out2 && q != out));
+        ok = ok && pre->out != pre->out2 && pre->out != out && pre->out2 != out;
+        if (!ok) { tri_set_error("conv(c64): pre-pass descriptor incomplete, or a by-product / the result aliases an input"); return TRI_ERR_ARG; }
+        a.pre_y = pre->y; a.pre_aux = pre->aux; a.pre_out = pre->out; a.pre_out2 = pre->out2;
+        for (int k = 0; k < ntab; ++k) a.pre_tab[k] = pre->tab[k];
+    }
     a.N = B; a.H = H; a.nbricks = g.nbricks; a.transposed = transposed; a.accumulate = accumulate;
     a.in_bytes = (unsigned)((size_t)B * H * g.W * 128);
+#define TRI_C64_T(AT_, W_, TY_)                                                                                            \
+    switch (form * 4 + (accumulate ? 2 : 0) + (bs ? 1 : 0)) {                                                              \
+        case C64_PRE_F * 4 + 0: return c64_launch_t<AT_, W_, TY_, false, false, C64_PRE_F>(a, g.grid, stream);            \
+        case C64_PRE_A * 4 + 2: return c64_launch_t<AT_, W_, TY_, true, false, C64_PRE_A>(a, g.grid, stream);             \
+        case C64_PRE_A * 4 + 3: return c64_launch_t<AT_, W_, TY_, true, true, C64_PRE_A>(a, g.grid, stream);              \
+        case C64_PRE_B * 4 + 1: return c64_launch_t<AT_, W_, TY_, false, true, C64_PRE_B>(a, g.grid, stream);             \
+        case 0: return c64_launch_t<AT_, W_, TY_, false, false, 0>(a, g.grid, stream);                                     \
+        case 1: return c64_launch_t<AT_, W_, TY_, false, true, 0>(a, g.grid, stream);                                      \
+        case 2: return c64_launch_t<AT_, W_, TY_, true, false, 0>(a, g.grid, stream);                                      \
+        case 3: return c64_launch_t<AT_, W_, TY_, true, true, 0>(a, g.grid, stream);                                       \
+    }
 #define TRI_C64_BS(W_, TY_, BS_)                                                                                           \
-    if (g.W == W_ && g.TY == TY_ && (bs != nullptr) == BS_) {                                                              \
+    if (g.W == W_ && g.TY == TY_ && !pre && (bs != nullptr) == BS_) {                                                      \
         if (act_fmt == TRI_FMT_F16)                                                                                        \
-            return accumulate ? c64_launch_t<f16_t, W_, TY_, true, BS_>(a, g.grid, stream) : c64_launch_t<f16_t, W_, TY_, false, BS_>(a, g.grid, stream);   \
-        return accumulate ? c64_launch_t<bf16_t, W_, TY_, true, BS_>(a, g.grid, stream) : c64_launch_t<bf16_t, W_, TY_, false, BS_>(a, g.grid, stream);     \
+            return accumulate ? c64_launch_t<f16_t, W_, TY_, true, BS_, 0>(a, g.grid, stream) : c64_launch_t<f16_t, W_, TY_, false, BS_, 0>(a, g.grid, stream);   \
+        return accumulate ? c64_launch_t<bf16_t, W_, TY_, true, BS_, 0>(a, g.grid, stream) : c64_launch_t<bf16_t, W_, TY_, false, BS_, 0>(a, g.grid, stream);     \
     }
 #define TRI_C64(W_, TY_) TRI_C64_BS(W_, TY_, false)
-    TRI_C64(32, 4)
-    TRI_C64(32, 2)
+#define TRI_C64_ALL(W_, TY_)                                                                                               \
+    if (g.W == W_ && g.TY == TY_) {                                                                                        \
+        if (act_fmt == TRI_FMT_F16) { TRI_C64_T(f16_t, W_, TY_) } else { TRI_C64_T(bf16_t, W_, TY_) }                      \
+    }
     TRI_C64(64, 2)
     TRI_C64(64, 1)
     TRI_C64(56, 2)
     TRI_C64(56, 1)
-    TRI_C64(16, 8)
-    TRI_C64(16, 4)
-    TRI_C64_BS(32, 4, true)
-    TRI_C64_BS(32, 2, true)
-    TRI_C64_BS(16, 8, true)
-    TRI_C64_BS(16, 4, true)
+    TRI_C64_ALL(32, 4)
+    TRI_C64_ALL(32, 2)
+    TRI_C64_ALL(16, 8)
+    TRI_C64_ALL(16, 4)
+#undef TRI_C64_ALL
+#undef TRI_C64_T
 #undef TRI_C64_BS
 #undef TRI_C64
-    tri_set_error("conv(c64): brick shape not instantiated (BatchNorm-backward sums: 16- and 32-wide images only)");
+    tri_set_error("conv(c64): brick shape not instantiated (BatchNorm-backward sums and pre-pass forms: 16- and 32-wide images only)");
     return TRI_ERR_UNSUPPORTED;
 }
 
diff --git a/tricolo_amd/csrc/conv_igemm.hip b/tricolo_amd/csrc/conv_igemm.hip
--- a/tricolo_amd/csrc/conv_igemm.hip
+++ b/tricolo_amd/csrc/conv_igemm.hip
@@ -2085,6 +2085,7 @@
     CF_ROWS = 8,
     CF_BIAS_ACT = 16, CF_ACCUM = 32, CF_STATS = 64,
     CF_BNSUMS = 128,
+    CF_PRE = 256,
     CF_EPI = CF_MASK | CF_ROWS | CF_BIAS_ACT,
 };
 enum ConvNeeds { ANY_MODE, MODE16, MODE16_DMA };
@@ -2102,7 +2103,7 @@
     bool frag;
     bool site_mask;
     int (*records)(const ConvPlan& pl);
-    int (*launch)(ConvArgs& a, const ConvPlan& pl, int act_fmt, const TriConvBnSums* bs, hipStream_t stream);
+    int (*launch)(ConvArgs& a, const ConvPlan& pl, int act_fmt, const TriConvBnSums* bs, const TriConvPre* pre, hipStream_t stream);
 };
 
 static int plan_generic(const TriConvDesc& v, int split_mode, int row_list, ConvPlan* pl) {
@@ -2158,7 +2159,7 @@
 }
 static int plan_c64(const TriConvDesc& v, int, int, ConvPlan* pl) {
     if (!tri_internal_c64_geometry(v, &pl->g.c64)) return PLAN_NO;
-    if (pl->g.c64.W > 32) pl->fall_also = CF_BNSUMS;
+    if (pl->g.c64.W > 32) pl->fall_also = CF_BNSUMS | CF_PRE;
     return PLAN_TAKES;
 }
 static int plan_s2g(const TriConvDesc& v, int, int, ConvPlan* pl) {
@@ -2191,55 +2192,55 @@
 
 static int halo_records(const ConvPlan& pl) { return pl.halo.wgrec ? pl.halo.grid / pl.halo.nt : pl.halo.mtiles; }
 
-static int run_vox0(ConvArgs& a, const ConvPlan& pl, int fmt, const TriConvBnSums*, hipStream_t s) {
+static int run_vox0(ConvArgs& a, const ConvPlan& pl, int fmt, const TriConvBnSums*, const TriConvPre*, hipStream_t s) {
     return tri_internal_vox0_launch(pl.g.vox0, a.B, a.in, a.w_hi, a.Kpad, a.out, a.row_mask, a.stats, fmt, s);
 }
-static int run_voxb(ConvArgs& a, const ConvPlan& pl, int fmt, const TriConvBnSums*, hipStream_t s) {
+static int run_voxb(ConvArgs& a, const ConvPlan& pl, int fmt, const TriConvBnSums*, const TriConvPre*, hipStream_t s) {
     return tri_internal_voxb_launch(pl.g.voxb, a.B, a.in, a.w_hi, a.out, a.row_mask, a.stats, fmt, s);
 }
-static int run_voxg(ConvArgs& a, const ConvPlan& pl, int fmt, const TriConvBnSums*, hipStream_t s) {
+static int run_voxg(ConvArgs& a, const ConvPlan& pl, int fmt, const TriConvBnSums*, const TriConvPre*, hipStream_t s) {
     return tri_internal_voxg_launch(pl.g.voxg, a.B, a.Cin, a.Cout, a.Kpad, a.in, a.w_hi, a.out, a.row_mask, a.stats, a.transposed, fmt, s);
 }
-static int run_stem(ConvArgs& a, const ConvPlan& pl, int fmt, const TriConvBnSums*, hipStream_t s) {
+static int run_stem(ConvArgs& a, const ConvPlan& pl, int fmt, const TriConvBnSums*, const TriConvPre*, hipStream_t s) {
     return fmt == TRI_FMT_F16 ? launch_stem<f16_t>(a, pl.g.stem, s) : launch_stem<bf16_t>(a, pl.g.stem, s);
 }
-static int run_pw(ConvArgs& a, const ConvPlan& pl, int fmt, const TriConvBnSums*, hipStream_t s) {
+static int run_pw(ConvArgs& a, const ConvPlan& pl, int fmt, const TriConvBnSums*, const TriConvPre*, hipStream_t s) {
     return tri_internal_pw_launch(pl.g.pw, a.B, a.in, a.w_hi, a.Cin, a.Cout, a.Kpad, a.out, a.stats, a.transposed ? 1 : 0, fmt, s);
 }
-static int run_c64(ConvArgs& a, const ConvPlan& pl, int fmt, const TriConvBnSums* bs, hipStream_t s) {
-    return tri_internal_c64_launch(pl.g.c64, a.B, a.IH, a.in, a.w_hi, a.out, bs ? bs->partial : a.stats, a.transposed, a.accumulate, fmt, bs, s);
-}
-static int run_s2g(ConvArgs& a, const ConvPlan& pl, int fmt, const TriConvBnSums*, hipStream_t s) {
+static int run_c64(ConvArgs& a, const ConvPlan& pl, int fmt, const TriConvBnSums* bs, const TriConvPre* pre, hipStream_t s) {
+    return tri_internal_c64_launch(pl.g.c64, a.B, a.IH, a.in, a.w_hi, a.out, bs ? bs->partial : a.stats, a.transposed, a.accumulate, fmt, bs, pre, s);
+}
+static int run_s2g(ConvArgs& a, const ConvPlan& pl, int fmt, const TriConvBnSums*, const TriConvPre*, hipStream_t s) {
     return tri_internal_s2g_launch(pl.g.s2g, a.B, a.IH, a.IW, a.Cin, a.Cout, a.Kpad, a.in, a.w_hi, a.out, a.stats, fmt, s);
 }
-static int run_s2d(ConvArgs& a, const ConvPlan& pl, int fmt, const TriConvBnSums*, hipStream_t s) {
+static int run_s2d(ConvArgs& a, const ConvPlan& pl, int fmt, const TriConvBnSums*, const TriConvPre*, hipStream_t s) {
     return tri_internal_s2d_launch(pl.also_g, a.B, a.IH, a.in, a.w_hi, a.out, a.accumulate, fmt, s);
 }
-static int run_halo(ConvArgs& a, const ConvPlan& pl, int fmt, const TriConvBnSums*, hipStream_t s) {
+static int run_halo(ConvArgs& a, const ConvPlan& pl, int fmt, const TriConvBnSums*, const TriConvPre*, hipStream_t s) {
     return fmt == TRI_FMT_F16 ? launch_halo<2, f16_t>(a, pl.halo, s) : launch_halo<2, bf16_t>(a, pl.halo, s);
 }
 
 #define CONV_RECORDS(member) [](const ConvPlan& pl) -> int { return pl.g.member; }
 static const ConvFamily conv_families[] = {
-    {TRI_CONV_VOX0, "conv_vox0_kernel", MODE16, plan_vox0, CF_DGRAD | CF_BNSUMS, CF_ROWS | CF_BIAS_ACT | CF_ACCUM, 0, false,
+    {TRI_CONV_VOX0, "conv_vox0_kernel", MODE16, plan_vox0, CF_DGRAD | CF_BNSUMS | CF_PRE, CF_ROWS | CF_BIAS_ACT | CF_ACCUM, 0, false,
      false, true, CONV_RECORDS(vox0.grid), run_vox0},
-    {TRI_CONV_VOXB, "conv_voxb_kernel", MODE16, plan_voxb, CF_DGRAD | CF_BNSUMS, CF_ROWS | CF_BIAS_ACT | CF_ACCUM, 0, false,
+    {TRI_CONV_VOXB, "conv_voxb_kernel", MODE16, plan_voxb, CF_DGRAD | CF_BNSUMS | CF_PRE, CF_ROWS | CF_BIAS_ACT | CF_ACCUM, 0, false,
      true, true, CONV_RECORDS(voxb.grid), run_voxb},
-    {TRI_CONV_VOXG, "conv_voxg_kernel", MODE16, plan_voxg, CF_BNSUMS, CF_ROWS | CF_BIAS_ACT | CF_ACCUM, 0, false,
+    {TRI_CONV_VOXG, "conv_voxg_kernel", MODE16, plan_voxg, CF_BNSUMS | CF_PRE, CF_ROWS | CF_BIAS_ACT | CF_ACCUM, 0, false,
      true, true, CONV_RECORDS(voxg.nunits), run_voxg},
-    {TRI_CONV_STEM, "conv_stem_kernel", MODE16, plan_stem, CF_DGRAD | CF_EPI | CF_ACCUM | CF_BNSUMS, 0, 0, false,
+    {TRI_CONV_STEM, "conv_stem_kernel", MODE16, plan_stem, CF_DGRAD | CF_EPI | CF_ACCUM | CF_BNSUMS | CF_PRE, 0, 0, false,
      false, false, CONV_RECORDS(stem.grid), run_stem},
-    {TRI_CONV_PW, "conv_pw_kernel", MODE16_DMA, plan_pw, CF_EPI | CF_ACCUM | CF_BNSUMS, 0, 0, false,
+    {TRI_CONV_PW, "conv_pw_kernel", MODE16_DMA, plan_pw, CF_EPI | CF_ACCUM | CF_BNSUMS | CF_PRE, 0, 0, false,
      false, false, nullptr, run_pw},
     {TRI_CONV_C64, "conv_c64_kernel", MODE16_DMA, plan_c64, CF_EPI, 0, CF_STATS, true,
      false, false, CONV_RECORDS(c64.grid), run_c64},
-    {TRI_CONV_S2G, "conv_s2g_kernel", MODE16_DMA, plan_s2g, CF_BNSUMS, CF_DGRAD | CF_EPI | CF_ACCUM, 0, false,
+    {TRI_CONV_S2G, "conv_s2g_kernel", MODE16_DMA, plan_s2g, CF_BNSUMS | CF_PRE, CF_DGRAD | CF_EPI | CF_ACCUM, 0, false,
      true, false, CONV_RECORDS(s2g.nunits), run_s2g},
-    {TRI_CONV_S2D, "conv_s2d_kernel", MODE16_DMA, plan_s2d, CF_FWD | CF_EPI | CF_STATS | CF_BNSUMS, 0, 0, false,
+    {TRI_CONV_S2D, "conv_s2d_kernel", MODE16_DMA, plan_s2d, CF_FWD | CF_EPI | CF_STATS | CF_BNSUMS | CF_PRE, 0, 0, false,
      false, false, nullptr, run_s2d},
-    {TRI_CONV_HALO_ROWS, "conv_halo_rows_kernel", MODE16_DMA, plan_halo_rows, CF_EPI | CF_BNSUMS, 0, 0, false,
+    {TRI_CONV_HALO_ROWS, "conv_halo_rows_kernel", MODE16_DMA, plan_halo_rows, CF_EPI | CF_BNSUMS | CF_PRE, 0, 0, false,
      false, false, halo_records, run_halo},
-    {TRI_CONV_HALO2D, "conv_halo2d_kernel", MODE16_DMA, plan_halo2d, CF_EPI | CF_BNSUMS, 0, 0, false,
+    {TRI_CONV_HALO2D, "conv_halo2d_kernel", MODE16_DMA, plan_halo2d, CF_EPI | CF_BNSUMS | CF_PRE, 0, 0, false,
      false, false, halo_records, run_halo},
     {TRI_CONV_DMA, "conv_dma_kernel", MODE16_DMA, plan_generic, 0, 0, 0, false, false, false, nullptr, nullptr},
     {TRI_CONV_IGEMM, "conv_igemm_kernel", ANY_MODE, plan_generic, 0, 0, 0, false, false, false, nullptr, nullptr},
@@ -2300,7 +2301,7 @@
 }
 
 static int conv_dispatch(const TriConvDesc* d, ConvArgs& a, int act_fmt, void* workspace, size_t workspace_bytes, hipStream_t stream,
-                         const TriConvBnSums* bs = nullptr) {
+                         const TriConvBnSums* bs = nullptr, const TriConvPre* pre = nullptr) {
     if (a.Cin % 4 != 0) { tri_set_error("conv: stored input channels must be a multiple of 4"); return TRI_ERR_ARG; }
     if (a.Cout % 32 != 0) { tri_set_error("conv: output channels must be a multiple of 32"); return TRI_ERR_ARG; }
     if (a.ntaps > 64) { tri_set_error("conv: more than 64 taps unsupported"); return TRI_ERR_UNSUPPORTED; }
@@ -2338,13 +2339,18 @@
         a.row_pos = nullptr;
     }
     const unsigned feat = (a.transposed ? CF_DGRAD : CF_FWD) | (a.row_mask ? CF_MASK : 0) | (a.row_count ? CF_ROWS : 0) |
-                          ((a.bias || a.act != 0) ? CF_BIAS_ACT : 0) | (a.accumulate ? CF_ACCUM : 0) | (a.stats ? CF_STATS : 0) | (bs ? CF_BNSUMS : 0);
-    if (pl.also && !(feat & pl.also->falls)) return pl.also->launch(a, pl, act_fmt, bs, stream);
+                          ((a.bias || a.act != 0) ? CF_BIAS_ACT : 0) | (a.accumulate ? CF_ACCUM : 0) | (a.stats ? CF_STATS : 0) | (bs ? CF_BNSUMS : 0) |
+                          (pre ? CF_PRE : 0);
+    if (pl.also && !(feat & pl.also->falls)) return pl.also->launch(a, pl, act_fmt, bs, pre, stream);
+    if (pre && !conv_takes(pl, feat)) {
+        tri_set_error("conv: this layer's kernel applies no BatchNorm pass to its input (tri_conv_fwd_preact_supported / tri_conv_dgrad_prebn_supported == 0)");
+        return TRI_ERR_UNSUPPORTED;
+    }
     const ConvFamily& f = *pl.family;
     if (f.launch) {
         if (!(feat & (f.falls | pl.fall_also))) {
             if (feat & f.refuses) return conv_refuse(f, f.refuses, 0);
-            return f.launch(a, pl, act_fmt, bs, stream);
+            return f.launch(a, pl, act_fmt, bs, pre, stream);
         }
         if (feat & f.fall_refuses) return conv_refuse(f, f.falls & ~CF_BNSUMS, f.fall_refuses);
         if (f.fall_drops_order && !a.row_count) a.row_pos = nullptr;
@@ -2444,3 +2450,58 @@
     a.accumulate = accumulate;
     return conv_dispatch(d, a, act_fmt, workspace, workspace_bytes, (hipStream_t)stream, sums);
 }
+
+static bool conv_pre_takes(const TriConvDesc* d, int transposed, int accumulate, int sums, int stats, int form, int act_fmt) {
+    if (act_fmt != TRI_FMT_BF16 && act_fmt != TRI_FMT_F16) return false;
+    const ConvPlan pl = conv_make_plan(conv_view(*d, transposed), 2, 0);
+    const unsigned feat = (transposed ? CF_DGRAD : CF_FWD) | (accumulate ? CF_ACCUM : 0) | (sums ? CF_BNSUMS : 0) | (stats ? CF_STATS : 0) | CF_PRE;
+    if (pl.also && !(feat & pl.also->falls)) return false;
+    return conv_takes(pl, feat) && tri_internal_c64_pre_form(form, transposed, accumulate, sums);
+}
+extern "C" int tri_conv_fwd_preact_supported(const TriConvDesc* d, int want_stats, int act_fmt) {
+    return conv_pre_takes(d, 0, 0, 0, want_stats, 1, act_fmt) ? 1 : 0;
+}
+extern "C" int tri_conv_fwd_preact(const TriConvDesc* d, const void* y, const void* w_hi, void* out, float* stats, int act_fmt,
+                                   const TriConvPreAct* pre, void* stream) {
+    if (!pre || !pre->scale || !pre->shift || !pre->act_out) {
+        tri_set_error("tri_conv_fwd_preact: pre needs scale, shift and act_out");
+        return TRI_ERR_ARG;
+    }
+    if (!tri_conv_fwd_preact_supported(d, stats != nullptr, act_fmt)) {
+        tri_set_error("tri_conv_fwd_preact: no fused form for this layer (tri_conv_fwd_preact_supported == 0)");
+        return TRI_ERR_UNSUPPORTED;
+    }
+    TriConvPre ip{};
+    ip.form = 1; ip.aux = pre->res; ip.tab[0] = pre->scale; ip.tab[1] = pre->shift; ip.out = pre->act_out;
+    ConvArgs a = conv_args(d, 0);
+    a.in = y; a.w_hi = w_hi; a.out = out; a.stats = stats;
+    return conv_dispatch(d, a, act_fmt, nullptr, 0, (hipStream_t)stream, nullptr, &ip);
+}
+extern "C" int tri_conv_dgrad_prebn_supported(const TriConvDesc* d, int accumulate, int with_sums, int act_fmt) {
+    return conv_pre_takes(d, 1, accumulate, with_sums, 0, accumulate ? 2 : 3, act_fmt) ? 1 : 0;
+}
+extern "C" int tri_conv_dgrad_prebn(const TriConvDesc* d, const void* g, const void* wt_hi, void* din, int accumulate, int act_fmt,
+                                    const TriConvPreBn* pre, const TriConvBnSums* sums, void* stream) {
+    if (!pre || !pre->y || !pre->c1 || !pre->c2 || !pre->c3 || !pre->dy || (!pre->relu_scale != !pre->relu_shift) ||
+        (pre->relu_scale != nullptr) == (pre->relu_out != nullptr) || (pre->relu_out && !pre->g_masked)) {
+        tri_set_error("tri_conv_dgrad_prebn: pre needs y, c1, c2, c3, dy and either relu_scale + relu_shift or relu_out + g_masked");
+        return TRI_ERR_ARG;
+    }
+    if (sums && (!sums->y || !sums->partial || (!sums->relu_scale != !sums->relu_shift) || (sums->relu_scale && sums->relu_out))) {
+        tri_set_error("tri_conv_dgrad_prebn: sums needs y, partial and at most one of (relu_scale + relu_shift) / relu_out");
+        return TRI_ERR_ARG;
+    }
+    if ((pre->relu_out != nullptr) == (accumulate != 0) || !tri_conv_dgrad_prebn_supported(d, accumulate, sums != nullptr, act_fmt)) {
+        tri_set_error("tri_conv_dgrad_prebn: no fused form for this call (tri_conv_dgrad_prebn_supported == 0; relu_scale form: accumulate, "
+                      "relu_out form: no accumulate, with sums)");
+        return TRI_ERR_UNSUPPORTED;
+    }
+    TriConvPre ip{};
+    ip.form = accumulate ? 2 : 3; ip.y = pre->y; ip.aux = pre->relu_out;
+    ip.tab[0] = pre->c1; ip.tab[1] = pre->c2; ip.tab[2] = pre->c3; ip.tab[3] = pre->relu_scale; ip.tab[4] = pre->relu_shift;
+    ip.out = pre->dy; ip.out2 = pre->g_masked;
+    ConvArgs a = conv_args(d, 1);
+    a.in = g; a.w_hi = wt_hi; a.out = din;
+    a.accumulate = accumulate;
+    return conv_dispatch(d, a, act_fmt, nullptr, 0, (hipStream_t)stream, sums, &ip);
+}
diff --git a/tricolo_amd/csrc/conv_vox.h b/tricolo_amd/csrc/conv_vox.h
--- a/tricolo_amd/csrc/conv_vox.h
+++ b/tricolo_amd/csrc/conv_vox.h
@@ -32,8 +32,17 @@
 bool tri_internal_s2d_geometry(const TriConvDesc& d, TriC64Geom* g);
 int tri_internal_s2d_launch(const TriC64Geom& g, int B, int H, const void* in, const void* w, void* out, int accumulate, int act_fmt,
                             hipStream_t stream);
+struct TriConvPre {
+    int form;
+    const void* y;
+    const void* aux;
+    const float* tab[5];
+    void* out;
+    void* out2;
+};
+bool tri_internal_c64_pre_form(int form, int transposed, int accumulate, int sums);
 int tri_internal_c64_launch(const TriC64Geom& g, int B, int H, const void* in, const void* w, void* out, float* stats, int transposed,
-                            int accumulate, int act_fmt, const TriConvBnSums* bs, hipStream_t stream);
+                            int accumulate, int act_fmt, const TriConvBnSums* bs, const TriConvPre* pre, hipStream_t stream);
 
 struct TriPwGeom { int bn, mtiles, GH, GW, transposed; };
 bool tri_internal_pw_geometry(const TriConvDesc& d, TriPwGeom* g);
diff --git a/tricolo_amd/model/module/img_encoder/mv_cnn.py b/tricolo_amd/model/module/img_encoder/mv_cnn.py
--- a/tricolo_amd/model/module/img_encoder/mv_cnn.py
+++ b/tricolo_amd/model/module/img_encoder/mv_cnn.py
@@ -15,6 +15,7 @@
 _PREP_DGRAD_LATE = os.environ.get("TRICOLO_PREP_DGRAD_LATE", "1") != "0"
 _BN_PAIR = True
 _STEM_BESIDE_WGRAD = os.environ.get("TRICOLO_STEM_BESIDE_WGRAD", "1") != "0"
+_C64_FUSE = int(os.environ.get("TRICOLO_C64_FUSE", "3"))
 _PREP_ISSUE = int(os.environ.get("TRICOLO_PREP_ISSUE", "1"))
 
 
@@ -165,10 +166,19 @@
             self._side_prep.join(*pend)
             self.__dict__["_prep_pending"] = None
 
-    def _conv_bn(self, x, conv, bn, prec, train, after_conv=None):
+    def _conv_bn(self, x, conv, bn, prec, train, after_conv=None, pre_act=None):
         N, _, H, W, _ = x.shape
         g = self._geom2d(N, H, W, conv)
         packed = self._packed[(id(conv), False)]
+        if pre_act is not None:
+            if train:
+                y, stats, a = ops.conv_fwd(x, g, packed, want_stats=True, pre_act=pre_act)
+                co = ops.bn_finalize(stats, g.cout, bn.weight, bn.bias, bn.running_mean, bn.running_var, bn.num_batches_tracked,
+                                     count_host=g.M, momentum=bn.momentum, eps=bn.eps)
+            else:
+                y, a = ops.conv_fwd(x, g, packed, pre_act=pre_act)
+                co = ops.bn_eval_coeffs(g.cout, bn.weight, bn.bias, bn.running_mean, bn.running_var, bn.eps)
+            return y, co, g, a
         if train:
             y, stats = ops.conv_fwd(x, g, packed, want_stats=True)
             if after_conv is not None:
@@ -188,8 +198,15 @@
     def _upper_params(self):
         return self._param_list()[len(self._lower_params()):]
 
-    def _run_block(self, blk, x, prec, train, save, store):
+    def _fwd_fused(self, y, conv, train):
+        if not (_C64_FUSE & 2):
+            return False
+        N, _, H, W, _ = y.shape
+        return ops.conv_fwd_pre_supported(y, self._geom2d(N, H, W, conv), self._packed[(id(conv), False)], want_stats=train)
+
+    def _run_block(self, blk, x, prec, train, save, store, next_blk=None):
         ds = blk.downsample is not None
+        lazy = x if isinstance(x, tuple) else None
         mode = _DS_FWD if (ds and train) else 0
         shortcut = []
         ev = None
@@ -203,15 +220,24 @@
         if ds and not mode:
             run_shortcut()
         fine = ops.TIMELINE is not None and ops.TIMELINE.get("fine")
-        y1, co1, g1 = self._conv_bn(x, blk.conv1, blk.bn1, prec, train, after_conv=run_shortcut if mode else None)
+        if lazy is not None:
+            py, pco, pres, slot = lazy
+            y1, co1, g1, x = self._conv_bn(py, blk.conv1, blk.bn1, prec, train, pre_act=(pco, pres))
+            if slot is not None:
+                store[slot] = store[slot][:11] + (x,)
+        else:
+            y1, co1, g1 = self._conv_bn(x, blk.conv1, blk.bn1, prec, train, after_conv=run_shortcut if mode else None)
         if ds:
             yd, cod, gd = shortcut
         if fine:
             ops.stamp(f"image.fwd.c{y1.shape[-1]}.conv1+fin")
-        a1 = ops.bn_act(y1, co1, relu=True)
-        if fine:
-            ops.stamp(f"image.fwd.c{y1.shape[-1]}.act1")
-        y2, co2, g2 = self._conv_bn(a1, blk.conv2, blk.bn2, prec, train)
+        if self._fwd_fused(y1, blk.conv2, train):
+            y2, co2, g2, a1 = self._conv_bn(y1, blk.conv2, blk.bn2, prec, train, pre_act=(co1, None))
+        else:
+            a1 = ops.bn_act(y1, co1, relu=True)
+            if fine:
+                ops.stamp(f"image.fwd.c{y1.shape[-1]}.act1")
+            y2, co2, g2 = self._conv_bn(a1, blk.conv2, blk.bn2, prec, train)
         if fine:
             ops.stamp(f"image.fwd.c{y1.shape[-1]}.conv2+fin")
         if ds:
@@ -219,6 +245,11 @@
             out = ops.bn_act(y2, co2, relu=True, res=yd, res_co=cod)
         else:
             yd = cod = gd = None
+            if (next_blk is not None and next_blk.downsample is None and next_blk.conv1.in_channels == y2.shape[-1]
+                    and self._fwd_fused(y2, next_blk.conv1, train)):
+                if save:
+                    store.append((x, y1, co1, g1, a1, y2, co2, g2, yd, cod, gd, None))
+                return (y2, co2, x, len(store) - 1 if save else None)
             out = ops.bn_act(y2, co2, relu=True, res=x)
         if fine:
             ops.stamp(f"image.fwd.c{y1.shape[-1]}.act2")
@@ -245,8 +276,9 @@
         ops.stamp("image.fwd.stem.end")
         saved = {"stem": (x0, y, co, g, parg), "blocks": [], "N": N}
         self._join_packing()
-        for blk in self._blocks()[:self.N_LOWER_BLOCKS]:
-            x = self._run_block(blk, x, prec, train, save, saved["blocks"])
+        lower = self._blocks()[:self.N_LOWER_BLOCKS]
+        for i, blk in enumerate(lower):
+            x = self._run_block(blk, x, prec, train, save, saved["blocks"], next_blk=lower[i + 1] if i + 1 < len(lower) else None)
         ops.stamp("image.fwd.layer2.end")
         return x, saved
 
@@ -296,7 +328,14 @@
             pair = (_BN_PAIR and blk.downsample is not None and batch is not None and dout_sums is None and yd is not None
                     and yd.shape == y2.shape and ops._sync_world() == 1)
             dyd_pair = None
-            if pair:
+            fuse = bool(_C64_FUSE & 1) and blk.downsample is None and batch is not None and not pair
+            packed2, packed1 = self._packed[(id(blk.conv2), True)], self._packed[(id(blk.conv1), True)]
+            fuse2 = (fuse and ops.bn_bwd_has_finalize(y2, dout_sums)
+                     and ops.conv_dgrad_pre_supported(dout, g2, packed2, bn_sums=(y1, co1, None)))
+            if fuse2:
+                buf2, gr[blk.bn2.weight], gr[blk.bn2.bias] = ops.bn_bwd(y2, dout, co2, blk.bn2.weight, count_host=g2.M, inplace=False,
+                                                                        relu_out=out, out_scale=ugs, partial=dout_sums, apply=False)
+            elif pair:
                 (dy2, gr[blk.bn2.weight], gr[blk.bn2.bias], dyd_pair, gr[blk.downsample[1].weight],
                  gr[blk.downsample[1].bias]) = ops.bn_bwd_pair(y2, co2, blk.bn2.weight, yd, cod, blk.downsample[1].weight, dout, out, g2.M,
                                                                g_masked=dout, out_scale=ugs)
@@ -325,17 +364,28 @@
                     return dyd_, ops.conv_dgrad(dyd_, gd, self._packed[(id(blk.downsample[0]), True)])
             if blk.downsample is not None and not mode:
                 dyd, dx = shortcut_bwd()
-            wgrad_async(a1, dy2, g2, blk.conv2.weight)
-            da1, sums1 = ops.conv_dgrad(dy2, g2, self._packed[(id(blk.conv2), True)], bn_sums=(y1, co1, None))
+            if fuse2:
+                da1, sums1, dy2, g = ops.conv_dgrad(dout, g2, packed2, bn_sums=(y1, co1, None), pre_bn=(y2, buf2, None, out))
+                wgrad_async(a1, dy2, g2, blk.conv2.weight)
+            else:
+                wgrad_async(a1, dy2, g2, blk.conv2.weight)
+                da1, sums1 = ops.conv_dgrad(dy2, g2, packed2, bn_sums=(y1, co1, None))
             if mode:
                 dyd, dx = shortcut_bwd()
             if fine:
                 ops.stamp(tag + ".dgrad2")
-            dy1, gr[blk.bn1.weight], gr[blk.bn1.bias] = ops.bn_bwd(y1, da1, co1, blk.bn1.weight, count_host=g1.M, relu=True, out_scale=ugs,
-                                                                   partial=sums1)
+            prev_sums = (saved_blocks[bi - 1][5], None, saved_blocks[bi - 1][11]) if bi > 0 else None
+            fuse1 = (fuse and ops.bn_bwd_has_finalize(y1, sums1)
+                     and ops.conv_dgrad_pre_supported(da1, g1, packed1, accumulate=True, bn_sums=prev_sums))
+            if fuse1:
+                buf1, gr[blk.bn1.weight], gr[blk.bn1.bias] = ops.bn_bwd(y1, da1, co1, blk.bn1.weight, count_host=g1.M, relu=True, out_scale=ugs,
+                                                                        partial=sums1, apply=False)
+            else:
+                dy1, gr[blk.bn1.weight], gr[blk.bn1.bias] = ops.bn_bwd(y1, da1, co1, blk.bn1.weight, count_host=g1.M, relu=True, out_scale=ugs,
+                                                                       partial=sums1)
+                wgrad_async(x, dy1, g1, blk.conv1.weight)
             if fine:
                 ops.stamp(tag + ".bn1")
-            wgrad_async(x, dy1, g1, blk.conv1.weight)
             if blk.downsample is not None:
                 if batch is None:
                     self._side_ds.join(dx, gr[blk.downsample[0].weight], gr[blk.downsample[1].weight], gr[blk.downsample[1].bias])
@@ -344,12 +394,13 @@
                     gr[blk.downsample[0].weight] = ops.conv_wgrad(x, dyd, gd, blk.downsample[0].weight, prec, out_scale=ugs, batch=batch)
             else:
                 dx = g
-            if bi > 0:
-                prev = saved_blocks[bi - 1]
-                dx, dout_sums = ops.conv_dgrad(dy1, g1, self._packed[(id(blk.conv1), True)], out=dx, accumulate=True,
-                                               bn_sums=(prev[5], None, prev[11]))
+            if fuse1:
+                dx, dout_sums, dy1 = ops.conv_dgrad(da1, g1, packed1, out=dx, accumulate=True, bn_sums=prev_sums, pre_bn=(y1, buf1, co1, None))
+                wgrad_async(x, dy1, g1, blk.conv1.weight)
+            elif bi > 0:
+                dx, dout_sums = ops.conv_dgrad(dy1, g1, packed1, out=dx, accumulate=True, bn_sums=prev_sums)
             else:
-                dx, dout_sums = ops.conv_dgrad(dy1, g1, self._packed[(id(blk.conv1), True)], out=dx, accumulate=True), None
+                dx, dout_sums = ops.conv_dgrad(dy1, g1, packed1, out=dx, accumulate=True), None
             if fine:
                 ops.stamp(tag + ".dgrad1")
             dout = dx
diff --git a/tricolo_amd/ops.py b/tricolo_amd/ops.py
--- a/tricolo_amd/ops.py
+++ b/tricolo_amd/ops.py
@@ -262,6 +262,16 @@
             c[k] = int(lib().tri_conv_dgrad_bn_records(_C.C.byref(self.desc), 1 if accumulate else 0, fmt))
         return c[k]
 
+    def pre_supported(self, transposed: bool, fmt: int, accumulate: bool = False, sums: bool = False, stats: bool = False) -> bool:
+        c = self.__dict__.setdefault("_pre_supported", {})
+        k = (bool(transposed), fmt, bool(accumulate), bool(sums), bool(stats))
+        if k not in c:
+            if transposed:
+                c[k] = bool(lib().tri_conv_dgrad_prebn_supported(_C.C.byref(self.desc), int(k[2]), int(k[3]), fmt))
+            else:
+                c[k] = bool(lib().tri_conv_fwd_preact_supported(_C.C.byref(self.desc), int(k[4]), fmt))
+        return c[k]
+
     def wgrad_group(self, fmt: int):
         c = self.__dict__.setdefault("_wgrad_group", {})
         if fmt not in c:
@@ -353,7 +363,11 @@
         return bufs
 
 
-def conv_fwd(x, g: ConvGeom, packed, row_mask=None, bias=None, act=0, want_stats=False, out=None, accumulate=False, rows=None):
+def conv_fwd_pre_supported(x, g: ConvGeom, packed, want_stats=False) -> bool:
+    return packed[1] is None and x.dtype != torch.float32 and g.pre_supported(False, _abf(x), stats=want_stats)
+
+
+def conv_fwd(x, g: ConvGeom, packed, row_mask=None, bias=None, act=0, want_stats=False, out=None, accumulate=False, rows=None, pre_act=None):
     hi, lo = packed
     g.check_packed(packed, False, x)
     OD, OH, OW = g.out_grid
@@ -362,6 +376,16 @@
     assert out.dtype == x.dtype
     nrec = (g.num_records_rows if rows else g.num_mtiles)[_conv_mode(x, lo)]
     stats = torch.empty((nrec, 2, g.cout), dtype=torch.float32, device=x.device) if want_stats else None
+    if pre_act is not None:
+        co, res = pre_act
+        assert row_mask is None and bias is None and act == 0 and not accumulate and rows is None and lo is None
+        assert res is None or (res.dtype == x.dtype and res.shape == x.shape)
+        a = torch.empty_like(x)
+        pre = _C.TriConvPreAct(ptr(co.scale), ptr(co.shift), ptr(res), ptr(a))
+        check(_timed(_igemm_symbol(g, False, False, x), g.flops,
+                     lambda: lib().tri_conv_fwd_preact(_C.C.byref(g.desc), ptr(_act(x)), ptr(hi), ptr(out), ptr(stats), _abf(x),
+                                                       _C.C.byref(pre), stream())), "tri_conv_fwd_preact")
+        return (out, stats, a) if want_stats else (out, a)
     ws = _workspace(g.fwd_ws, x.device) if g.fwd_ws else None
     check(_timed(_igemm_symbol(g, False, lo is not None, x), _flops(g, rows, row_mask),
                  lambda: lib().tri_conv_fwd(_C.C.byref(g.desc), ptr(_act(x)), ptr(hi), ptr(lo), ptr(out), ptr(row_mask), ptr(bias),
@@ -378,22 +402,57 @@
 _DGRAD_BN = _DGRAD_BN_MODE != "0"
 
 
-def conv_dgrad(dout, g: ConvGeom, packed_t, row_mask=None, out=None, accumulate=False, rows=None, bn_sums=None):
+def _dgrad_bn_nrec(dout, g: ConvGeom, lo, row_mask, accumulate, rows, bn_sums) -> int:
+    if bn_sums is None:
+        return 0
+    _, co, relu_out = bn_sums
+    if not (_DGRAD_BN and not (accumulate and _DGRAD_BN_MODE == "2") and row_mask is None and rows is None and lo is None
+            and (relu_out is not None) == bool(accumulate) and (co is not None) != (relu_out is not None)):
+        return 0
+    return g.dgrad_bn_records(accumulate, _abf(dout))
+
+
+def conv_dgrad_pre_supported(dout, g: ConvGeom, packed_t, accumulate=False, bn_sums=None) -> bool:
+    if packed_t[1] is not None or dout.dtype == torch.float32:
+        return False
+    sums = _dgrad_bn_nrec(dout, g, None, None, accumulate, None, bn_sums) > 0
+    return g.pre_supported(True, _abf(dout), accumulate=accumulate, sums=sums)
+
+
+def conv_dgrad(dout, g: ConvGeom, packed_t, row_mask=None, out=None, accumulate=False, rows=None, bn_sums=None, pre_bn=None):
     hi, lo = packed_t
     g.check_packed(packed_t, True, dout)
     ID, IH, IW = g.in_grid
     if out is None:
         out = torch.empty((g.B, ID, IH, IW, g.cin_stored), dtype=dout.dtype, device=dout.device)
     assert out.dtype == dout.dtype
+    if pre_bn is not None:
+        py, buf, pco, pro = pre_bn
+        assert row_mask is None and rows is None and lo is None and py.dtype == dout.dtype and py.shape == dout.shape
+        nrec = _dgrad_bn_nrec(dout, g, lo, None, accumulate, None, bn_sums)
+        partial = sums = None
+        if nrec:
+            y, co, relu_out = bn_sums
+            assert y.dtype == out.dtype and y.numel() == out.numel()
+            partial = torch.empty((nrec, 2, g.cin_stored), dtype=torch.float32, device=dout.device)
+            sums = _C.TriConvBnSums(ptr(y), ptr(co.scale) if co is not None else None, ptr(co.shift) if co is not None else None,
+                                    ptr(relu_out), ptr(partial))
+        dy = torch.empty_like(dout)
+        gm = torch.empty_like(dout) if pro is not None else None
+        pre = _C.TriConvPreBn(ptr(py), ptr(buf[2]), ptr(buf[3]), ptr(buf[4]), ptr(pco.scale) if pco is not None else None,
+                              ptr(pco.shift) if pco is not None else None, ptr(pro), ptr(dy), ptr(gm))
+        check(_timed(_igemm_symbol(g, True, False, dout), g.flops,
+                     lambda: lib().tri_conv_dgrad_prebn(_C.C.byref(g.desc), ptr(_act(dout)), ptr(hi), ptr(out), 1 if accumulate else 0,
+                                                        _abf(dout), _C.C.byref(pre), _C.C.byref(sums) if sums is not None else None,
+                                                        stream())), "tri_conv_dgrad_prebn")
+        return (out, partial, dy) if gm is None else (out, partial, dy, gm)
     ws = _workspace(g.dgrad_ws, dout.device) if g.dgrad_ws else None
     rowpos = g.dgrad_row_order(dout.device) if (row_mask is None and rows is None and _ROW_ORDER) else None
     if rows is not None:
         rowpos = rows[0]
     if bn_sums is not None:
         y, co, relu_out = bn_sums
-        nrec = g.dgrad_bn_records(accumulate, _abf(dout)) if (_DGRAD_BN and not (accumulate and _DGRAD_BN_MODE == "2") and row_mask is None and rows is None and lo is None
-                                                               and (relu_out is not None) == bool(accumulate)
-                                                               and (co is not None) != (relu_out is not None)) else 0
+        nrec = _dgrad_bn_nrec(dout, g, lo, row_mask, accumulate, rows, bn_sums)
         if nrec == 0:
             return conv_dgrad(dout, g, packed_t, row_mask=row_mask, out=out, accumulate=accumulate, rows=rows), None
         assert y.dtype == out.dtype and y.numel() == out.numel()
@@ -699,9 +758,11 @@
 
 
 def _bn_bwd_finish(y, g, partial, co: BNCoeffs, gamma, count_dev, count_host, out_scale, dy, row_mask=None, keep_inactive=False, rows=None,
-                   rs=None, rb=None, relu_out=None, g_masked=None):
+                   rs=None, rb=None, relu_out=None, g_masked=None, apply=True):
     C = y.shape[-1]
     buf = _bn_bwd_finalize(partial, partial.shape[0], C, count_dev, count_host, gamma, co, out_scale)
+    if not apply:
+        return buf, buf[0], buf[1]
     if rows is not None:
         check(lib().tri_bn_bwd_apply_rows(ptr(y), ptr(g), ptr(buf[2]), ptr(buf[3]), ptr(buf[4]), ptr(dy), C, ptr(rows[0]), ptr(rows[1]),
                                           rows[0].numel(), _abf(y), stream()), "tri_bn_bwd_apply_rows")
@@ -711,13 +772,19 @@
     return dy, buf[0], buf[1]
 
 
+def bn_bwd_has_finalize(y, partial=None) -> bool:
+    C = y.shape[-1]
+    return not (partial is None and _BN_SMALL and y.numel() // C <= 512 and C % 8 == 0 and C >= 64 and _sync_world() == 1)
+
+
 def bn_bwd(y, g, co: BNCoeffs, gamma, count_dev=None, count_host=0, row_mask=None, inplace=True, relu=False, relu_out=None,
-           g_masked=None, out_scale: float = 1.0, keep_inactive: bool = False, partial=None):
+           g_masked=None, out_scale: float = 1.0, keep_inactive: bool = False, partial=None, apply=True):
     rs, rb = (co.scale, co.shift) if relu else (None, None)
     C = y.shape[-1]
     M = y.numel() // C
     assert y.dtype == g.dtype
-    dy = g if inplace else torch.empty_like(g)
+    assert apply or (bn_bwd_has_finalize(y, partial) and row_mask is None)
+    dy = None if not apply else (g if inplace else torch.empty_like(g))
     if partial is None and _BN_SMALL and M <= 512 and C % 8 == 0 and C >= 64 and _sync_world() == 1:
         buf = torch.empty((2, C), dtype=torch.float32, device=y.device)
         check(lib().tri_bn_bwd_small(ptr(_act(y)), ptr(_act(g)), M, C, ptr(count_dev), int(count_host), ptr(gamma), ptr(co.mean), ptr(co.invstd),
@@ -730,7 +797,7 @@
               "tri_bn_bwd_reduce")
     assert partial.shape[1:] == (2, C)
     return _bn_bwd_finish(y, g, partial, co, gamma, count_dev, count_host, out_scale, dy, row_mask=row_mask, keep_inactive=keep_inactive,
-                          rs=rs, rb=rb, relu_out=relu_out, g_masked=g_masked)
+                          rs=rs, rb=rb, relu_out=relu_out, g_masked=g_masked, apply=apply)
 
 
 def bn_bwd_pair(ya, coa: BNCoeffs, gamma_a, yb, cob: BNCoeffs, gamma_b, g, relu_out, count_host, g_masked=None, out_scale: float = 1.0):
```
